# jseppanen/azalea

Hardware: AMD Instinct MI355X
Metric: mcts_sims_per_sec (higher is better)
Workload: dtype f16x3 (fp32 operands split hi+lo f16, fp32 accumulate)

## Files before the change

azalea_amd/csrc/azx_capi.cpp:

```cpp
#include <hip/hip_runtime.h>

#include <algorithm>
#include <cmath>
#include <cstdarg>
#include <cstdio>
#include <cstdlib>
#include <cstring>
#include <map>
#include <mutex>
#include <string>
#include <vector>

#include "../../include/azx.h"
#include "azx_dev.h"
#include "mcts_kernels.h"
#include "net.h"
#include "train.h"
#include "replay_kernels.h"
#include "ext_kernels.h"
#include "match_kernels.h"

#ifndef AZX_SRC_SHA
#define AZX_SRC_SHA "unknown"
#endif

static thread_local std::string g_err;

static int fail(int code, const char *fmt, ...) {
    char buf[1024];
    va_list ap;
    va_start(ap, fmt);
    vsnprintf(buf, sizeof buf, fmt, ap);
    va_end(ap);
    g_err = buf;
    return code;
}

#define HIPCHECK(expr)                                                                    \
    do {                                                                                  \
        hipError_t _e = (expr);                                                           \
        if (_e != hipSuccess)                                                             \
            return fail(AZX_EHIP, "%s failed: %s (%s:%d)", #expr, hipGetErrorString(_e),  \
                        __FILE__, __LINE__);                                              \
    } while (0)

struct azx_engine {
    azx_config cfg;
    DevEngine d;
    hipStream_t stream = nullptr;
    int reserved_cus = 0;
    std::mutex alloc_mu;
    int num_batches = 0;
    int selects_per_search = 0;
    std::vector<void *> allocs;
    int32_t *g_k = nullptr, *g_legal = nullptr, *g_nn = nullptr;
    float *g_cv = nullptr, *g_cw = nullptr, *g_cp = nullptr, *g_rv = nullptr, *g_rw = nullptr,
          *g_sv = nullptr;
    double *noise_dev = nullptr;
    size_t noise_cap = 0;
    float *prior_table_dev = nullptr;
    int32_t *moveids_dev = nullptr;
    int32_t *slots_dev = nullptr, *moves_dev = nullptr, *nmoves_dev = nullptr;
    size_t moves_cap = 0;
    bool ext_active = false;
    int ext_batches_done = 0;
    std::vector<int> ext_order;
    std::vector<std::vector<int>> ext_cells;
    azx_eval_fn ext_fn = nullptr;
    void *ext_user = nullptr;
    ExtBufs ext = {nullptr, nullptr, nullptr, nullptr, nullptr, nullptr, nullptr};
    int32_t ext_info[4] = {0, 0, AZX_EXT_NO_ERROR, 0};
    int32_t *ext_info_host = nullptr;
    std::vector<char> ext_dirty;
    bool ext_failed = false;
    bool play_ready = false;
    int64_t q_alloc = 0;
    int64_t q_rows_valid = 0;
    std::vector<void *> q_allocs;
    int32_t *export_board = nullptr;
    float *export_prob = nullptr;
    size_t export_cap = 0;
    ReplayRows ring = {nullptr, nullptr, nullptr, nullptr, nullptr};
    int64_t ring_cap = 0, ring_size = 0, ring_write = 0;
    long long *ring_idx = nullptr;
    int64_t ring_idx_cap = 0;
    int32_t *ring_maxk = nullptr;
    bool ring_mover_view = false;
    std::vector<void *> ring_allocs;
    long long *cidx_host[8] = {nullptr}, *cidx_dev[8] = {nullptr};
    hipEvent_t cidx_ev[8] = {nullptr};
    int64_t cidx_cap = 0;
    uint64_t cidx_next = 0;
    int32_t *cidx_maxk = nullptr;
    std::vector<hipEvent_t> ev_pool;
    std::vector<char> ev_tag;
    std::vector<int> ev_weight;
    std::vector<int> ev_group, ev_ref;
    int ev_groups = 0;
    size_t ev_used = 0;
    AzxNet *net = nullptr;
    bool force_generic = false;
    bool no_persistent = false;
    bool pipeline = true;
    bool stagger = true;
    hipStream_t stream_b = nullptr;
    std::vector<uint32_t> cu_mask;
    hipEvent_t ev_fork = nullptr, ev_join = nullptr, ev_stagger = nullptr;
    int32_t *stagger_ctr = nullptr;
    int64_t dbg_qcap = 0;
};

template <typename T>
static int dev_alloc(azx_engine *e, T **p, size_t count, bool zero = true) {
    void *q = nullptr;
    const size_t bytes = std::max<size_t>(count * sizeof(T), 16);
    hipError_t err = hipMalloc(&q, bytes);
    if (err != hipSuccess)
        return fail(AZX_ENOMEM, "hipMalloc(%zu bytes) failed: %s", bytes, hipGetErrorString(err));
    if (zero) {
        err = hipMemsetAsync(q, 0, bytes, e->stream);
        if (err != hipSuccess) return fail(AZX_EHIP, "hipMemset failed: %s", hipGetErrorString(err));
    }
    std::lock_guard<std::mutex> lock(e->alloc_mu);
    e->allocs.push_back(q);
    *p = reinterpret_cast<T *>(q);
    return AZX_OK;
}

struct DevGuard {
    int prev = -1;
    bool changed = false;
    explicit DevGuard(int dev) {
        if (hipGetDevice(&prev) == hipSuccess && prev != dev) changed = hipSetDevice(dev) == hipSuccess;
    }
    ~DevGuard() { if (changed) (void)hipSetDevice(prev); }
    DevGuard(const DevGuard &) = delete;
    DevGuard &operator=(const DevGuard &) = delete;
};
#define ENGINE_GUARD(e) DevGuard _dev_guard((e)->cfg.device)

#define TRY(expr)            \
    do {                     \
        int _rc = (expr);    \
        if (_rc) return _rc; \
    } while (0)

extern "C" const char *azx_last_error(void) { return g_err.c_str(); }
extern "C" int azx_version(void) { return 7; }

extern "C" int azx_create(const azx_config *cfg, azx_engine **out) {
    if (!cfg || !out) return fail(AZX_EINVAL, "null argument");
    int ndev = 0;
    if (hipGetDeviceCount(&ndev) != hipSuccess || ndev <= 0)
        return fail(AZX_ENODEV, "no HIP device visible: the engine has no CPU fallback");
    if (cfg->board_size < 2 || cfg->board_size > AZX_MAX_BOARD)
        return fail(AZX_EINVAL, "board_size %d outside [2, %d]", cfg->board_size, AZX_MAX_BOARD);
    if (cfg->n_games < 1) return fail(AZX_EINVAL, "n_games must be >= 1");
    if (cfg->search_batch_size < 1 || cfg->search_batch_size > AZX_MAX_BATCH)
        return fail(AZX_EINVAL, "search_batch_size %d outside [1, %d]", cfg->search_batch_size,
                    AZX_MAX_BATCH);
    if (cfg->simulations < 0) return fail(AZX_EINVAL, "simulations must be >= 0");
    if (cfg->evaluator < AZX_EVAL_RESNET || cfg->evaluator > AZX_EVAL_EXTERNAL)
        return fail(AZX_EINVAL, "unknown evaluator %d", cfg->evaluator);
    if (cfg->device < 0 || cfg->device >= ndev)
        return fail(AZX_EINVAL, "device %d not in [0, %d)", cfg->device, ndev);
    if (cfg->game_index_stride < 0 || cfg->game_index_offset < 0 ||
        cfg->game_index_offset >= std::max(1, cfg->game_index_stride))
        return fail(AZX_EINVAL, "game_index_offset %d outside [0, game_index_stride %d)", cfg->game_index_offset,
                    std::max(1, cfg->game_index_stride));
    DevGuard guard(cfg->device);
    { int cur = -1; if (hipGetDevice(&cur) != hipSuccess || cur != cfg->device) return fail(AZX_EHIP, "hipSetDevice(%d) failed", cfg->device); }
    if (azx_init_geometry(cfg->device)) return fail(AZX_EHIP, "uploading the board geometry tables failed");

    azx_engine *e = new azx_engine();
    e->cfg = *cfg;
    { const char *v = getenv("AZX_MCTS_GENERIC"); e->force_generic = v && atoi(v) != 0; }
    { const char *v = getenv("AZX_NO_PERSISTENT"); e->no_persistent = v && atoi(v) != 0; }
    { const char *v = getenv("AZX_PIPELINE"); e->pipeline = !(v && atoi(v) == 0); }
    { const char *v = getenv("AZX_PIPELINE_STAGGER"); e->stagger = !(v && atoi(v) == 0); }
    HIPCHECK(hipStreamCreateWithFlags(&e->stream, hipStreamNonBlocking));
    DevEngine &d = e->d;
    memset(&d, 0, sizeof d);
    d.N = cfg->board_size;
    d.ncells = d.N * d.N;
    d.G = cfg->n_games;
    d.bs = cfg->search_batch_size;
    d.slots = d.ncells <= 128 ? 2 : 3;
    d.c_puct = cfg->exploration_coef;
    d.evaluator = cfg->evaluator;
    d.flags = cfg->flags;
    d.seed = cfg->seed;
    d.uid_stride = std::max(1, cfg->game_index_stride);
    d.uid_offset = cfg->game_index_offset;
    d.slot_base = 0;
    d.pool_games = d.G;
    d.noise_alpha = (float)cfg->noise_alpha;
    d.noise_scale = 0.0;
    d.exploration_depth = cfg->exploration_depth;
    d.temperature = (float)cfg->temperature;
    e->num_batches = cfg->simulations / cfg->search_batch_size + 1;
    e->selects_per_search = e->num_batches * cfg->search_batch_size;
    d.selects_per_search = e->selects_per_search;
    int cap = cfg->nodes_per_game;
    if (cap <= 0) cap = 6 * (e->selects_per_search + 1) * d.ncells + 1024;
    d.cap = cap;

    const size_t G = d.G, bs = d.bs, E = G * bs;
    const size_t pstride = d.ncells + (d.ncells & 1);
    int rc = AZX_OK;
#define A(ptr, count) if (!rc) rc = dev_alloc(e, &ptr, (count))
    A(d.cells, G * d.slots * 64);
    A(d.ghdr, G);
    A(d.thdr, G);
    if (!rc) rc = dev_alloc(e, &d.arena[0], G * (size_t)cap, false);
    if (cfg->flags & AZX_FLAG_NO_COMPACT) d.arena[1] = d.arena[0];
    else if (!rc) rc = dev_alloc(e, &d.arena[1], G * (size_t)cap, false);
    A(d.leaf_node, E); A(d.leaf_len, E); A(d.leaf_eval, E); A(d.leaf_link, E); A(d.leaf_cells, E);
    A(d.leaf_mask, E * 4); A(d.path, E * pstride);
    A(d.ev_board, E * AZX_CELL_STRIDE); A(d.ev_src, E); A(d.ev_flip, E);
    A(d.ev_value, E); A(d.ev_prior, E * AZX_CELL_STRIDE); A(d.n_eval, 4);
    A(d.counters, G * CTR_COUNT); A(d.q_count, 2); A(d.stat_sums, G * 8);
    A(e->g_k, G); A(e->g_legal, G * d.ncells); A(e->g_nn, G);
    A(e->g_cv, G * d.ncells); A(e->g_cw, G * d.ncells); A(e->g_cp, G * d.ncells);
    A(e->g_rv, G); A(e->g_rw, G); A(e->g_sv, G);
    A(e->moveids_dev, G); A(e->slots_dev, G); A(e->nmoves_dev, G);
#undef A
    if (rc) { azx_destroy(e); return rc; }
    if (cfg->evaluator == AZX_EVAL_RESNET) {
        rc = azx_net_create(&e->net, d.N, cfg->num_blocks, cfg->base_chans, (int)E, e->stream);
        if (rc) { g_err = azx_net_error(); azx_destroy(e); return rc; }
    }
    {
        float *gt = nullptr;
        rc = dev_alloc(e, &gt, AZX_GAMMA_TAB_FLOATS);
        if (rc) { azx_destroy(e); return rc; }
        std::vector<float> tab(AZX_GAMMA_TAB_FLOATS, 0.0f);
        if (cfg->noise_alpha > 0.0) azx_gamma_table(cfg->noise_alpha, tab.data());
        if (hipMemcpyAsync(gt, tab.data(), tab.size() * sizeof(float), hipMemcpyHostToDevice, e->stream) != hipSuccess ||
            hipStreamSynchronize(e->stream) != hipSuccess) {
            azx_destroy(e);
            return fail(AZX_EHIP, "uploading the gamma sampler table failed");
        }
        e->d.gamma_tab = gt;
    }
    *out = e;
    {
        std::vector<float> tab(d.ncells + 1, 0.0f);
        for (int k = 1; k <= d.ncells; ++k) tab[k] = 1.0f / (float)k;
        rc = azx_set_prior_table(e, tab.data(), d.ncells + 1);
        if (rc) { azx_destroy(e); *out = nullptr; return rc; }
        e->d.prior_default = 1;
    }
    azx_launch_reset(d, nullptr, d.G, nullptr, nullptr, 0, 1, e->stream);
    HIPCHECK(hipStreamSynchronize(e->stream));
    return AZX_OK;
}

extern "C" void azx_destroy(azx_engine *e) {
    if (!e) return;
    ENGINE_GUARD(e);
    if (e->stream) (void)hipStreamSynchronize(e->stream);
    if (e->net) azx_net_destroy(e->net);
    for (void *p : e->allocs) (void)hipFree(p);
    for (void *p : e->q_allocs) (void)hipFree(p);
    for (void *p : e->ring_allocs) (void)hipFree(p);
    if (e->export_board) (void)hipFree(e->export_board);
    if (e->export_prob) (void)hipFree(e->export_prob);
    if (e->ext_info_host) (void)hipHostFree(e->ext_info_host);
    for (hipEvent_t ev : e->ev_pool) (void)hipEventDestroy(ev);
    if (e->ev_fork) (void)hipEventDestroy(e->ev_fork);
    if (e->ev_join) (void)hipEventDestroy(e->ev_join);
    if (e->ev_stagger) (void)hipEventDestroy(e->ev_stagger);
    if (e->stream_b) { (void)hipStreamSynchronize(e->stream_b); (void)hipStreamDestroy(e->stream_b); }
    for (int i = 0; i < 8; ++i) {
        if (e->cidx_ev[i]) { (void)hipEventSynchronize(e->cidx_ev[i]); (void)hipEventDestroy(e->cidx_ev[i]); }
        if (e->cidx_host[i]) (void)hipHostFree(e->cidx_host[i]);
        if (e->cidx_dev[i]) (void)hipFree(e->cidx_dev[i]);
    }
    if (e->stream) (void)hipStreamDestroy(e->stream);
    delete e;
}

extern "C" void *azx_stream(azx_engine *e) { return e ? (void *)e->stream : nullptr; }

extern "C" int azx_reserve_cus(azx_engine *e, int cus_per_xcd, int *reserved_out) {
    if (!e) return fail(AZX_EINVAL, "null engine");
    ENGINE_GUARD(e);
    hipDeviceProp_t prop;
    HIPCHECK(hipGetDeviceProperties(&prop, e->cfg.device));
    const int ncu = prop.multiProcessorCount, xcds = 8, ses = 4;
    if (cus_per_xcd < 0 || cus_per_xcd * xcds >= ncu)
        return fail(AZX_EINVAL, "cus_per_xcd %d outside [0, %d)", cus_per_xcd, ncu / xcds);
    if (cus_per_xcd > 0 && ncu % (xcds * ses))
        return fail(AZX_ESTATE, "CU reservation is laid out for 8 XCDs x 4 shader engines; this device has %d CUs", ncu);
    const int per = (cus_per_xcd + ses - 1) / ses * ses;
    const int words = (ncu + 31) / 32;
    std::vector<uint32_t> mask((size_t)words, 0u);
    for (int b = 0; b < ncu; ++b)
        if (b >= per * xcds) mask[b / 32] |= 1u << (b % 32);
    HIPCHECK(hipStreamSynchronize(e->stream));
    hipStream_t fresh = nullptr;
    if (per == 0) HIPCHECK(hipStreamCreateWithFlags(&fresh, hipStreamNonBlocking));
    else HIPCHECK(hipExtStreamCreateWithCUMask(&fresh, (uint32_t)words, mask.data()));
    hipStream_t old = e->stream;
    e->stream = fresh;
    if (e->net) azx_net_set_stream(e->net, fresh, per ? mask.data() : nullptr, per ? words : 0);
    (void)hipStreamDestroy(old);
    if (e->stream_b) {
        (void)hipStreamSynchronize(e->stream_b);
        (void)hipStreamDestroy(e->stream_b);
        e->stream_b = nullptr;
    }
    e->cu_mask.assign(mask.begin(), per ? mask.end() : mask.begin());
    e->reserved_cus = per * xcds;
    if (!e->cidx_maxk) TRY(dev_alloc(e, &e->cidx_maxk, 4));
    HIPCHECK(hipStreamSynchronize(e->stream));
    if (reserved_out) *reserved_out = e->reserved_cus;
    return AZX_OK;
}

static bool use_pipeline(const azx_engine *e) {
    return e->pipeline && e->d.evaluator == AZX_EVAL_RESNET && e->d.G % 2 == 0 && e->d.G >= 1024 &&
           azx_net_rows_splittable(e->net);
}

static DevEngine pool_view(const DevEngine &d, int base, int n, int32_t *n_eval) {
    DevEngine v = d;
    const size_t b = (size_t)base, bs = (size_t)d.bs, nc = (size_t)d.ncells, pstride = nc + (nc & 1);
    v.G = n;
    v.slot_base = d.slot_base + base;
    v.cells += b * d.slots * 64;
    v.ghdr += b;
    v.thdr += b;
    v.arena[0] += b * d.cap;
    v.arena[1] += b * d.cap;
    v.leaf_node += b * bs; v.leaf_len += b * bs; v.leaf_eval += b * bs; v.leaf_link += b * bs; v.leaf_cells += b * bs;
    v.leaf_mask += b * bs * 4;
    v.path += b * bs * pstride;
    v.ev_board += b * bs * AZX_CELL_STRIDE;
    v.ev_src += b * bs;
    v.ev_flip += b * bs;
    v.ev_value += b * bs;
    v.ev_prior += b * bs * AZX_CELL_STRIDE;
    v.n_eval = n_eval;
    if (v.noise) v.noise += b * d.n_select * d.noise_stride;
    v.counters += b * CTR_COUNT;
    v.stat_sums += b * 8;
    if (v.row_board) v.row_board += b * nc * AZX_CELL_STRIDE;
    if (v.row_prob) v.row_prob += b * nc * AZX_CELL_STRIDE;
    if (v.row_k) v.row_k += b * nc;
    if (v.row_meta) v.row_meta += b * nc * AZX_ROW_METRICS;
    return v;
}

static int pipeline_streams(azx_engine *e) {
    if (!e->stream_b) {
        if (e->cu_mask.empty()) HIPCHECK(hipStreamCreateWithFlags(&e->stream_b, hipStreamNonBlocking));
        else HIPCHECK(hipExtStreamCreateWithCUMask(&e->stream_b, (uint32_t)e->cu_mask.size(), e->cu_mask.data()));
    }
    if (!e->ev_fork) HIPCHECK(hipEventCreateWithFlags(&e->ev_fork, hipEventDisableTiming));
    if (!e->ev_join) HIPCHECK(hipEventCreateWithFlags(&e->ev_join, hipEventDisableTiming));
    if (!e->ev_stagger) HIPCHECK(hipEventCreateWithFlags(&e->ev_stagger, hipEventDisableTiming));
    if (!e->stagger_ctr) TRY(dev_alloc(e, &e->stagger_ctr, 4));
    return AZX_OK;
}

extern "C" int azx_kernel_info(azx_engine *e, char *buf, int cap) {
    if (!e || !buf || cap < 1) return fail(AZX_EINVAL, "null argument");
    const DevEngine &d = e->d;
    const int S = d.slots <= 2 ? 2 : 3;
    char tree[96], play[160];
    if (d.evaluator == AZX_EVAL_UNIFORM || d.evaluator == AZX_EVAL_UNIFORM_HASH) {
        DevEngine probe = d;
        probe.device_noise = 1;
        const bool fast = azx_mcts_fast_path(probe, MODE_BEGIN | MODE_INLINE, e->force_generic);
        snprintf(tree, sizeof tree, "k_mcts<%d,%s>", S, fast ? "FAST (throughput mode; generic with host noise)" : "generic");
        snprintf(play, sizeof play, "%s", fast && !e->no_persistent ? (S == 2 ? "k_play<2> (persistent)" : "k_play<3> (persistent)")
                                                                       : "k_mcts + k_choose + k_advance per move");
    } else {
        snprintf(tree, sizeof tree, "k_mcts<%d,generic> (BEGIN / APPLY|SELECT / APPLY phases)", S);
        snprintf(play, sizeof play, "%s", !use_pipeline(e) ? "phases + k_choose + k_advance per move, one stream"
                                          : e->stagger     ? "phases + k_choose + k_advance per move, two half-pools on two streams half an evaluation apart (any tower)"
                                                           : "phases + k_choose + k_advance per move, two half-pools on two streams");
    }
    std::string text = std::string("tree=") + tree + "; play=" + play + "; net=" +
                       (e->net ? azx_net_kernel_info(e->net) : "none") +
                       "; switches: AZX_MCTS_GENERIC=" + (e->force_generic ? "1" : "0") +
                       " AZX_NO_PERSISTENT=" + (e->no_persistent ? "1" : "0") +
                       " AZX_PIPELINE=" + (e->pipeline ? "1" : "0") +
                       " AZX_PIPELINE_STAGGER=" + (e->stagger ? "1" : "0") +
                       " reserved_cus=" + std::to_string(e->reserved_cus) +
                       "; src=" AZX_SRC_SHA;
    snprintf(buf, (size_t)cap, "%s", text.c_str());
    return (int)text.size();
}

extern "C" int azx_debug_stagger(azx_engine *e, int32_t *out4) {
    if (!e || !out4) return fail(AZX_EINVAL, "null argument");
    ENGINE_GUARD(e);
    memset(out4, 0, 4 * sizeof(int32_t));
    if (!e->stagger_ctr) return AZX_OK;
    HIPCHECK(hipMemcpyAsync(out4, e->stagger_ctr, 4 * sizeof(int32_t), hipMemcpyDeviceToHost, e->stream));
    HIPCHECK(hipStreamSynchronize(e->stream));
    return AZX_OK;
}

extern "C" int azx_debug_set_queue_cap(azx_engine *e, int64_t rows) {
    if (!e || rows < 0) return fail(AZX_EINVAL, "bad argument");
    e->dbg_qcap = rows;
    return AZX_OK;
}

static int check_net_range(azx_engine *e) {
    if (!e->net) return AZX_OK;
    int rc = azx_net_check_range(e->net, e->stream);
    if (rc) g_err = azx_net_error();
    return rc;
}

extern "C" int azx_debug_weights(azx_engine *e, int which, void *out, int64_t cap, int64_t *nbytes, char *name, int name_cap) {
    if (!e) return fail(AZX_EINVAL, "null engine");
    ENGINE_GUARD(e);
    if (!e->net) return fail(AZX_ESTATE, "engine was not created with AZX_EVAL_RESNET");
    int rc = azx_net_debug_weights(e->net, which, out, cap, nbytes, name, name_cap);
    if (rc) g_err = azx_net_error();
    return rc;
}

extern "C" int azx_set_weights(azx_engine *e, int n_tensors, const char *const *names,
                               const void *const *ptrs, const int64_t *counts, int on_device) {
    if (!e) return fail(AZX_EINVAL, "null engine");
    ENGINE_GUARD(e);
    if (!e->net) return fail(AZX_ESTATE, "engine was not created with AZX_EVAL_RESNET");
    int rc = azx_net_set_weights(e->net, n_tensors, names, ptrs, counts, on_device);
    if (rc) g_err = azx_net_error();
    return rc;
}

extern "C" int azx_set_prior_table(azx_engine *e, const float *prior_by_k, int count) {
    if (!e || !prior_by_k) return fail(AZX_EINVAL, "null argument");
    ENGINE_GUARD(e);
    if (count < e->d.ncells + 1) return fail(AZX_EINVAL, "prior table needs %d entries", e->d.ncells + 1);
    if (!e->prior_table_dev) TRY(dev_alloc(e, &e->prior_table_dev, (size_t)e->d.ncells + 1));
    HIPCHECK(hipMemcpyAsync(e->prior_table_dev, prior_by_k, sizeof(float) * (e->d.ncells + 1),
                            hipMemcpyHostToDevice, e->stream));
    HIPCHECK(hipStreamSynchronize(e->stream));
    e->d.prior_by_k = e->prior_table_dev;
    e->d.prior_default = 0;
    return AZX_OK;
}

extern "C" int azx_reset(azx_engine *e, const int32_t *slots, int n_slots, const int32_t *moves,
                         const int32_t *n_moves, int stride) {
    if (!e) return fail(AZX_EINVAL, "null engine");
    ENGINE_GUARD(e);
    DevEngine &d = e->d;
    if (!slots) n_slots = d.G;
    if (n_slots < 1 || n_slots > d.G) return fail(AZX_EINVAL, "n_slots %d outside [1, %d]", n_slots, d.G);
    if (slots) {
        for (int i = 0; i < n_slots; ++i)
            if (slots[i] < 0 || slots[i] >= d.G) return fail(AZX_EINVAL, "slot %d out of range", slots[i]);
        HIPCHECK(hipMemcpyAsync(e->slots_dev, slots, sizeof(int32_t) * n_slots, hipMemcpyHostToDevice, e->stream));
    }
    if (moves) {
        if (!n_moves || stride < 1) return fail(AZX_EINVAL, "moves given without n_moves/stride");
        const size_t need = (size_t)n_slots * stride;
        if (need > e->moves_cap) {
            TRY(dev_alloc(e, &e->moves_dev, need));
            e->moves_cap = need;
        }
        for (int i = 0; i < n_slots; ++i) {
            if (n_moves[i] < 0 || n_moves[i] > stride) return fail(AZX_EINVAL, "n_moves[%d] out of range", i);
            std::vector<char> used(d.ncells, 0);
            for (int p = 0; p < n_moves[i]; ++p) {
                const int mv = moves[(size_t)i * stride + p];
                if (mv < 1 || mv > d.ncells || used[mv - 1]) return fail(AZX_EINVAL, "illegal move %d", mv);
                used[mv - 1] = 1;
            }
        }
        HIPCHECK(hipMemcpyAsync(e->moves_dev, moves, sizeof(int32_t) * need, hipMemcpyHostToDevice, e->stream));
        HIPCHECK(hipMemcpyAsync(e->nmoves_dev, n_moves, sizeof(int32_t) * n_slots, hipMemcpyHostToDevice, e->stream));
    }
    azx_launch_reset(d, slots ? e->slots_dev : nullptr, n_slots, moves ? e->moves_dev : nullptr,
                     moves ? e->nmoves_dev : nullptr, stride, 1, e->stream);
    HIPCHECK(hipGetLastError());
    HIPCHECK(hipStreamSynchronize(e->stream));
    e->ext_active = false;
    if (e->ext_failed) {
        for (int i = 0; i < n_slots; ++i) e->ext_dirty[slots ? slots[i] : i] = 0;
        e->ext_failed = std::find(e->ext_dirty.begin(), e->ext_dirty.end(), 1) != e->ext_dirty.end();
    }
    return AZX_OK;
}

static void time_begin(azx_engine *e, char tag = 0, hipStream_t s = nullptr, int group = 0, int ref = -1) {
    if (e->ev_used + 2 > e->ev_pool.size()) {
        if (e->ev_pool.size() >= 1 << 16) return;
        hipEvent_t a, b;
        if (hipEventCreate(&a) != hipSuccess || hipEventCreate(&b) != hipSuccess) return;
        e->ev_pool.push_back(a);
        e->ev_pool.push_back(b);
    }
    const size_t n = e->ev_pool.size() / 2, i = e->ev_used / 2;
    if (e->ev_tag.size() < n) { e->ev_tag.resize(n, 0); e->ev_weight.resize(n, 1); e->ev_group.resize(n, 0); e->ev_ref.resize(n, -1); }
    e->ev_tag[i] = tag;
    e->ev_weight[i] = 1;
    e->ev_group[i] = ref >= 0 ? group : 0;
    e->ev_ref[i] = ref;
    (void)hipEventRecord(e->ev_pool[e->ev_used], s ? s : e->stream);
}
static void time_end(azx_engine *e, int weight = 1, hipStream_t s = nullptr) {
    if (e->ev_used + 2 > e->ev_pool.size()) return;
    (void)hipEventRecord(e->ev_pool[e->ev_used + 1], s ? s : e->stream);
    e->ev_weight[e->ev_used / 2] = weight;
    e->ev_used += 2;
}
static int time_mark(azx_engine *e, hipStream_t s) {
    time_begin(e, 2, s);
    if (e->ev_used + 2 > e->ev_pool.size()) return -1;
    const int ref = (int)e->ev_used;
    time_end(e, 1, s);
    return ref;
}
static void time_collect(azx_engine *e, azx_play_stats *st) {
    auto book = [&](char tag, int weight, double seconds, int launches) {
        if (tag == 1) { st->net_seconds += seconds; st->net_launches += launches; }
        else {
            st->mcts_seconds += seconds;
            st->mcts_launches += weight * launches;
            st->mcts_kernel_launches += launches;
        }
    };
    std::map<int, char> groups;
    std::map<std::pair<int, char>, std::vector<std::pair<float, float>>> spans;
    for (size_t i = 0; i + 1 < e->ev_used; i += 2) {
        const size_t k = i / 2;
        if (e->ev_tag[k] == 2) continue;
        float ms = 0.f;
        if (!e->ev_group[k]) {
            if (hipEventElapsedTime(&ms, e->ev_pool[i], e->ev_pool[i + 1]) == hipSuccess)
                book(e->ev_tag[k], e->ev_weight[k], ms * 1e-3, 1);
            continue;
        }
        float b = 0.f, en = 0.f;
// ... 59 lines not shown
    char buf[768];
    va_list ap;
    va_start(ap, fmt);
    vsnprintf(buf, sizeof buf, fmt, ap);
    va_end(ap);
    (void)hipStreamSynchronize(e->stream);
    const int32_t clear = AZX_EXT_NO_ERROR;
    (void)hipMemcpyAsync(e->ext.info + 2, &clear, sizeof clear, hipMemcpyHostToDevice, e->stream);
    (void)hipStreamSynchronize(e->stream);
    e->ext_info[2] = clear;
    e->ext_active = false;
    e->ev_used = 0;
    e->ev_groups = 0;
    e->ext_failed = true;
    std::fill(e->ext_dirty.begin(), e->ext_dirty.end(), 1);
    return fail(AZX_EEXTERNAL, "%s", buf);
}

static int ext_check_rows(azx_engine *e) {
    const int32_t w = e->ext_info[2];
    if (w == AZX_EXT_NO_ERROR) return AZX_OK;
    const int row = w >> 3, what = w & 7;
    return ext_fail(e, "external evaluator: row %d of its batch %s", row,
                    (what & 1) ? "has a value that is not finite"
                    : (what & 2) ? "has a negative (or NaN) prior probability"
                                 : "has prior probabilities whose sum is not 1 within 1e-4 (mcts.py:211-213)");
}

static int ext_info_enqueue(azx_engine *e, hipStream_t s) {
    HIPCHECK(hipMemcpyAsync(e->ext_info_host, e->ext.info, sizeof e->ext_info, hipMemcpyDeviceToHost, s));
    return AZX_OK;
}

static int ext_info_take(azx_engine *e) {
    memcpy(e->ext_info, e->ext_info_host, sizeof e->ext_info);
    return ext_check_rows(e);
}

static int ext_read_info(azx_engine *e) {
    TRY(ext_info_enqueue(e, e->stream));
    HIPCHECK(hipStreamSynchronize(e->stream));
    return ext_info_take(e);
}

static int ext_point_enqueue(azx_engine *e, bool timed) {
    if (timed) time_begin(e, 1);
    azx_launch_ext_order(e->d, e->ext, e->stream);
    HIPCHECK(hipGetLastError());
    return ext_info_enqueue(e, e->stream);
}

static int ext_point_finish(azx_engine *e, bool timed) {
    DevEngine &d = e->d;
    HIPCHECK(hipStreamSynchronize(e->stream));
    const int rc_info = ext_info_take(e);
    if (rc_info) return rc_info;
    const int n = e->ext_info[0], kmax = e->ext_info[1];
    if (n < 0 || n > d.G * d.bs) return ext_fail(e, "external evaluator: %d pending rows (internal error)", n);
    if (n > 0) {
        azx_launch_ext_export(d, e->ext, n, e->stream);
        HIPCHECK(hipGetLastError());
        const int rc = e->ext_fn(e->ext_user, n, kmax, e->ext.board, e->ext.legal, e->ext.value, e->ext.prior,
                                 (void *)e->stream);
        if (rc) return ext_fail(e, "external evaluator returned %d on a batch of %d rows", rc, n);
        azx_launch_ext_import(d, e->ext, n, e->stream);
        HIPCHECK(hipGetLastError());
    }
    if (timed) time_end(e);
    return AZX_OK;
}

struct ExtCursor {
    int points = 0;
    bool done = true;
    bool timed = false;
};

static int ext_search_begin(azx_engine *e, ExtCursor *c, bool timed) {
    c->points = 0;
    c->done = false;
    c->timed = timed;
    HIPCHECK(hipMemsetAsync(e->d.n_eval, 0, sizeof(int32_t), e->stream));
    if (timed) time_begin(e);
    azx_launch_mcts(e->d, MODE_BEGIN, e->num_batches, e->stream, e->force_generic);
    if (timed) time_end(e);
    return ext_point_enqueue(e, timed);
}

static int ext_search_resume(azx_engine *e, ExtCursor *c) {
    TRY(ext_point_finish(e, c->timed));
    if (c->points < e->num_batches) {
        HIPCHECK(hipMemsetAsync(e->d.n_eval, 0, sizeof(int32_t), e->stream));
        if (c->timed) time_begin(e);
        azx_launch_mcts(e->d, MODE_APPLY | MODE_SELECT, e->num_batches, e->stream, e->force_generic);
        if (c->timed) time_end(e);
        c->points += 1;
        return ext_point_enqueue(e, c->timed);
    }
    if (c->timed) time_begin(e);
    azx_launch_mcts(e->d, MODE_APPLY, e->num_batches, e->stream, e->force_generic);
    if (c->timed) time_end(e);
    c->done = true;
    return AZX_OK;
}

extern "C" int azx_set_external_evaluator(azx_engine *e, azx_eval_fn fn, void *user) {
    if (!e) return fail(AZX_EINVAL, "null engine");
    ENGINE_GUARD(e);
    if (e->d.evaluator != AZX_EVAL_EXTERNAL)
        return fail(AZX_EINVAL, "an external evaluator needs an AZX_EVAL_EXTERNAL engine (this one has evaluator %d)",
                    e->d.evaluator);
    if (fn && !e->ext.info) {
        const size_t E = (size_t)e->d.G * e->d.bs, nc = (size_t)e->d.ncells;
        ExtBufs x = {nullptr, nullptr, nullptr, nullptr, nullptr, nullptr, nullptr};
        int rc = AZX_OK;
        if (!rc) rc = dev_alloc(e, &x.src2ev, E);
        if (!rc) rc = dev_alloc(e, &x.row_ev, E);
        if (!rc) rc = dev_alloc(e, &x.info, 4);
        if (!rc) rc = dev_alloc(e, &x.board, E * nc);
        if (!rc) rc = dev_alloc(e, &x.legal, E * nc);
        if (!rc) rc = dev_alloc(e, &x.value, E);
        if (!rc) rc = dev_alloc(e, &x.prior, E * nc);
        if (rc) return rc;
        if (!e->ext_info_host &&
            hipHostMalloc((void **)&e->ext_info_host, sizeof e->ext_info, hipHostMallocDefault) != hipSuccess)
            return fail(AZX_ENOMEM, "hipHostMalloc of the evaluator's info words failed");
        const int32_t init[4] = {0, 0, AZX_EXT_NO_ERROR, 0};
        HIPCHECK(hipMemcpyAsync(x.info, init, sizeof init, hipMemcpyHostToDevice, e->stream));
        HIPCHECK(hipStreamSynchronize(e->stream));
        e->ext = x;
        e->ext_dirty.assign((size_t)e->d.G, 0);
    }
    e->ext_fn = fn;
    e->ext_user = fn ? user : nullptr;
    return AZX_OK;
}

static int enqueue_search(azx_engine *e, bool timed) {
    DevEngine &d = e->d;
    if (ext_registered(e)) {
        ExtCursor c;
        TRY(ext_search_begin(e, &c, timed));
        while (!c.done) TRY(ext_search_resume(e, &c));
        return AZX_OK;
    }
    if (d.evaluator == AZX_EVAL_UNIFORM || d.evaluator == AZX_EVAL_UNIFORM_HASH) {
        if (timed) time_begin(e);
        azx_launch_mcts(d, MODE_BEGIN | MODE_INLINE, e->num_batches, e->stream, e->force_generic);
        if (timed) time_end(e);
        return AZX_OK;
    }
    if (d.evaluator == AZX_EVAL_RESNET) {
        if (!azx_net_ready(e->net)) return fail(AZX_ESTATE, "azx_set_weights has not been called");
        HIPCHECK(hipMemsetAsync(d.n_eval, 0, sizeof(int32_t), e->stream));
        if (timed) time_begin(e);
        azx_launch_mcts(d, MODE_BEGIN, e->num_batches, e->stream, e->force_generic);
        if (timed) time_end(e);
        if (timed) time_begin(e, 1);
        azx_net_eval(e->net, d, e->stream);
        if (timed) time_end(e);
        for (int b = 0; b < e->num_batches; ++b) {
            HIPCHECK(hipMemsetAsync(d.n_eval, 0, sizeof(int32_t), e->stream));
            if (timed) time_begin(e);
            azx_launch_mcts(d, MODE_APPLY | MODE_SELECT, e->num_batches, e->stream, e->force_generic);
            if (timed) time_end(e);
            if (timed) time_begin(e, 1);
            azx_net_eval(e->net, d, e->stream);
            if (timed) time_end(e);
        }
        if (timed) time_begin(e);
        azx_launch_mcts(d, MODE_APPLY, e->num_batches, e->stream, e->force_generic);
        if (timed) time_end(e);
        return AZX_OK;
    }
    return fail(AZX_ESTATE, "evaluator %d has no device pipeline", d.evaluator);
}

extern "C" int azx_search(azx_engine *e, const double *noise, int n_select, int noise_stride,
                          double noise_scale) {
    if (!e) return fail(AZX_EINVAL, "null engine");
    ENGINE_GUARD(e);
    TRY(ext_refuse(e));
    if (e->d.evaluator == AZX_EVAL_EXTERNAL && !ext_registered(e))
        return fail(AZX_ESTATE, "AZX_EVAL_EXTERNAL: drive azx_search_begin/step instead");
    TRY(upload_noise(e, noise, n_select, noise_stride, noise_scale));
    TRY(enqueue_search(e, false));
    HIPCHECK(hipGetLastError());
    HIPCHECK(hipStreamSynchronize(e->stream));
    if (ext_registered(e)) return ext_read_info(e);
    return check_net_range(e);
}

static int read_pending(azx_engine *e, int *n_pending) {
    int32_t n = 0;
    HIPCHECK(hipMemcpyAsync(&n, e->d.n_eval, sizeof n, hipMemcpyDeviceToHost, e->stream));
    HIPCHECK(hipStreamSynchronize(e->stream));
    *n_pending = n;
    return e->d.evaluator == AZX_EVAL_RESNET ? check_net_range(e) : AZX_OK;
}

extern "C" int azx_search_begin(azx_engine *e, const double *noise, int n_select, int noise_stride,
                                double noise_scale, int *n_pending) {
    if (!e || !n_pending) return fail(AZX_EINVAL, "null argument");
    ENGINE_GUARD(e);
    TRY(ext_refuse(e));
    if (e->d.evaluator != AZX_EVAL_EXTERNAL && e->d.evaluator != AZX_EVAL_RESNET)
        return fail(AZX_ESTATE, "phase API needs AZX_EVAL_EXTERNAL (or RESNET)");
    TRY(upload_noise(e, noise, n_select, noise_stride, noise_scale));
    HIPCHECK(hipMemsetAsync(e->d.n_eval, 0, sizeof(int32_t), e->stream));
    if (e->d.evaluator == AZX_EVAL_RESNET && !azx_net_ready(e->net))
        return fail(AZX_ESTATE, "azx_set_weights has not been called");
    azx_launch_mcts(e->d, MODE_BEGIN, e->num_batches, e->stream, e->force_generic);
    if (e->d.evaluator == AZX_EVAL_RESNET) azx_net_eval(e->net, e->d, e->stream);
    HIPCHECK(hipGetLastError());
    e->ext_active = true;
    e->ext_batches_done = 0;
    return read_pending(e, n_pending);
}

extern "C" int azx_search_step(azx_engine *e, int *n_pending, int *done) {
    if (!e || !n_pending || !done) return fail(AZX_EINVAL, "null argument");
    ENGINE_GUARD(e);
    if (!e->ext_active) return fail(AZX_ESTATE, "azx_search_step without azx_search_begin");
    HIPCHECK(hipMemsetAsync(e->d.n_eval, 0, sizeof(int32_t), e->stream));
    if (e->ext_batches_done < e->num_batches) {
        azx_launch_mcts(e->d, MODE_APPLY | MODE_SELECT, e->num_batches, e->stream, e->force_generic);
        if (e->d.evaluator == AZX_EVAL_RESNET) azx_net_eval(e->net, e->d, e->stream);
        e->ext_batches_done += 1;
        *done = 0;
    } else {
        azx_launch_mcts(e->d, MODE_APPLY, e->num_batches, e->stream, e->force_generic);
        e->ext_active = false;
        *done = 1;
    }
    HIPCHECK(hipGetLastError());
    return read_pending(e, n_pending);
}

static int flip_cell(int cell, int N) {
    const int r = cell / N, c = cell % N;
    return (N - 1 - c) * N + (N - 1 - r);
}

extern "C" int azx_get_leaves(azx_engine *e, int cap, int32_t *boards, int32_t *legal_moves,
                              int32_t *slot, int32_t *k, int *n_out) {
    if (!e || !n_out) return fail(AZX_EINVAL, "null argument");
    ENGINE_GUARD(e);
    DevEngine &d = e->d;
    int n = 0;
    TRY(read_pending(e, &n));
    if (n > cap) return fail(AZX_EINVAL, "%d pending leaves, caller capacity %d", n, cap);
    *n_out = n;
    e->ext_order.clear();
    e->ext_cells.clear();
    if (n == 0) return AZX_OK;
    std::vector<uint8_t> hb((size_t)n * AZX_CELL_STRIDE);
    std::vector<int32_t> hsrc(n), hflip(n);
    HIPCHECK(hipMemcpyAsync(hb.data(), d.ev_board, hb.size(), hipMemcpyDeviceToHost, e->stream));
    HIPCHECK(hipMemcpyAsync(hsrc.data(), d.ev_src, sizeof(int32_t) * n, hipMemcpyDeviceToHost, e->stream));
    HIPCHECK(hipMemcpyAsync(hflip.data(), d.ev_flip, sizeof(int32_t) * n, hipMemcpyDeviceToHost, e->stream));
    const size_t E = (size_t)d.G * d.bs;
    std::vector<uint64_t> hmask(E * 4);
    HIPCHECK(hipMemcpyAsync(hmask.data(), d.leaf_mask, sizeof(uint64_t) * hmask.size(), hipMemcpyDeviceToHost, e->stream));
    HIPCHECK(hipStreamSynchronize(e->stream));
    std::vector<int> order(n);
    for (int i = 0; i < n; ++i) order[i] = i;
    std::sort(order.begin(), order.end(), [&](int a, int b) { return hsrc[a] < hsrc[b]; });
    e->ext_order = order;
    e->ext_cells.resize(n);
    for (int j = 0; j < n; ++j) {
        const int ev = order[j], src = hsrc[ev];
        std::vector<int> &cells = e->ext_cells[j];
        for (int c = 0; c < d.ncells; ++c)
            if ((hmask[(size_t)src * 4 + (c >> 6)] >> (c & 63)) & 1ull) cells.push_back(c);
        if (slot) slot[j] = src / d.bs;
        if (k) k[j] = (int)cells.size();
        if (boards)
            for (int c = 0; c < d.ncells; ++c)
                boards[(size_t)j * d.ncells + c] = hb[(size_t)ev * AZX_CELL_STRIDE + c];
        if (legal_moves) {
            for (int c = 0; c < d.ncells; ++c) legal_moves[(size_t)j * d.ncells + c] = 0;
            for (size_t i = 0; i < cells.size(); ++i)
                legal_moves[(size_t)j * d.ncells + i] =
                    (hflip[ev] ? flip_cell(cells[i], d.N) : cells[i]) + 1;
        }
    }
    return AZX_OK;
}

extern "C" int azx_put_evals(azx_engine *e, int n, const float *value, const float *prior) {
    if (!e || (n && (!value || !prior))) return fail(AZX_EINVAL, "null argument");
    ENGINE_GUARD(e);
    DevEngine &d = e->d;
    if (n != (int)e->ext_order.size())
        return fail(AZX_ESTATE, "azx_put_evals(%d) does not match %zu pending leaves", n, e->ext_order.size());
    if (n == 0) return AZX_OK;
    std::vector<float> hv(n), hp((size_t)n * AZX_CELL_STRIDE, 0.0f);
    for (int j = 0; j < n; ++j) {
        const int ev = e->ext_order[j];
        hv[ev] = value[j];
        const std::vector<int> &cells = e->ext_cells[j];
        for (size_t i = 0; i < cells.size(); ++i)
            hp[(size_t)ev * AZX_CELL_STRIDE + cells[i]] = prior[(size_t)j * d.ncells + i];
    }
    HIPCHECK(hipMemcpyAsync(d.ev_value, hv.data(), sizeof(float) * n, hipMemcpyHostToDevice, e->stream));
    HIPCHECK(hipMemcpyAsync(d.ev_prior, hp.data(), sizeof(float) * hp.size(), hipMemcpyHostToDevice, e->stream));
    HIPCHECK(hipStreamSynchronize(e->stream));
    return AZX_OK;
}

extern "C" int azx_get_evals(azx_engine *e, int cap, float *value, float *prior, int *n_out) {
    if (!e || !n_out) return fail(AZX_EINVAL, "null argument");
    ENGINE_GUARD(e);
    DevEngine &d = e->d;
    const int n = (int)e->ext_order.size();
    if (n > cap) return fail(AZX_EINVAL, "%d evaluations, caller capacity %d", n, cap);
    *n_out = n;
    if (n == 0) return AZX_OK;
    std::vector<float> hv(n), hp((size_t)n * AZX_CELL_STRIDE);
    HIPCHECK(hipMemcpyAsync(hv.data(), d.ev_value, sizeof(float) * n, hipMemcpyDeviceToHost, e->stream));
    HIPCHECK(hipMemcpyAsync(hp.data(), d.ev_prior, sizeof(float) * hp.size(), hipMemcpyDeviceToHost, e->stream));
    HIPCHECK(hipStreamSynchronize(e->stream));
    for (int j = 0; j < n; ++j) {
        const int ev = e->ext_order[j];
// ... 137 lines not shown
}

extern "C" int azx_forward(azx_engine *e, int B, int K, const int32_t *boards,
                           const int32_t *legal_moves, float *value, float *moves_logprob) {
    if (!e) return fail(AZX_EINVAL, "null engine");
    ENGINE_GUARD(e);
    if (!e->net) return fail(AZX_ESTATE, "engine was not created with AZX_EVAL_RESNET");
    int rc = azx_net_forward_host(e->net, B, K, boards, legal_moves, value, moves_logprob, e->stream);
    if (rc) g_err = azx_net_error();
    return rc ? rc : check_net_range(e);
}

extern "C" int azx_hex_replay(int device, int board_size, int n_games, const int32_t *moves,
                              const int32_t *length, int stride, int32_t *result_out,
                              int32_t *nlegal_out, uint64_t *empties_out, int32_t *final_board) {
    int ndev = 0;
    if (hipGetDeviceCount(&ndev) != hipSuccess || ndev <= 0)
        return fail(AZX_ENODEV, "no HIP device visible: the engine has no CPU fallback");
    if (board_size < 2 || board_size > AZX_MAX_BOARD) return fail(AZX_EINVAL, "bad board_size");
    if (n_games < 1 || stride < 1 || !moves || !length) return fail(AZX_EINVAL, "bad argument");
    DevGuard guard(device);
    if (azx_init_geometry(device)) return fail(AZX_EHIP, "uploading the board geometry tables failed");
    const int ncells = board_size * board_size;
    for (int g = 0; g < n_games; ++g) {
        if (length[g] < 0 || length[g] > stride) return fail(AZX_EINVAL, "length[%d] out of range", g);
        std::vector<char> used(ncells, 0);
        for (int p = 0; p < length[g]; ++p) {
            const int mv = moves[(size_t)g * stride + p];
            if (mv < 1 || mv > ncells || used[mv - 1]) return fail(AZX_EINVAL, "illegal move %d in game %d", mv, g);
            used[mv - 1] = 1;
        }
    }
    const size_t gs = (size_t)n_games * stride;
    int32_t *dm = nullptr, *dl = nullptr, *dr = nullptr, *dn = nullptr, *df = nullptr;
    uint64_t *de = nullptr;
    HIPCHECK(hipMalloc(&dm, sizeof(int32_t) * gs));
    HIPCHECK(hipMalloc(&dl, sizeof(int32_t) * n_games));
    HIPCHECK(hipMalloc(&dr, sizeof(int32_t) * gs));
    HIPCHECK(hipMalloc(&dn, sizeof(int32_t) * gs));
    HIPCHECK(hipMalloc(&de, sizeof(uint64_t) * gs * 4));
    HIPCHECK(hipMalloc(&df, sizeof(int32_t) * (size_t)n_games * ncells));
    HIPCHECK(hipMemset(dr, 0, sizeof(int32_t) * gs));
    HIPCHECK(hipMemset(dn, 0, sizeof(int32_t) * gs));
    HIPCHECK(hipMemset(de, 0, sizeof(uint64_t) * gs * 4));
    HIPCHECK(hipMemcpy(dm, moves, sizeof(int32_t) * gs, hipMemcpyHostToDevice));
    HIPCHECK(hipMemcpy(dl, length, sizeof(int32_t) * n_games, hipMemcpyHostToDevice));
    azx_launch_hex_replay(board_size, n_games, dm, dl, stride, dr, dn, de, df, nullptr);
    HIPCHECK(hipGetLastError());
    HIPCHECK(hipDeviceSynchronize());
    if (result_out) HIPCHECK(hipMemcpy(result_out, dr, sizeof(int32_t) * gs, hipMemcpyDeviceToHost));
    if (nlegal_out) HIPCHECK(hipMemcpy(nlegal_out, dn, sizeof(int32_t) * gs, hipMemcpyDeviceToHost));
    if (empties_out) HIPCHECK(hipMemcpy(empties_out, de, sizeof(uint64_t) * gs * 4, hipMemcpyDeviceToHost));
    if (final_board) HIPCHECK(hipMemcpy(final_board, df, sizeof(int32_t) * (size_t)n_games * ncells, hipMemcpyDeviceToHost));
    (void)hipFree(dm); (void)hipFree(dl); (void)hipFree(dr); (void)hipFree(dn); (void)hipFree(de); (void)hipFree(df);
    return AZX_OK;
}

extern "C" int azx_set_active(azx_engine *e, const int32_t *active) {
    if (!e || !active) return fail(AZX_EINVAL, "null argument");
    ENGINE_GUARD(e);
    DevEngine &d = e->d;
    std::vector<int32_t> a((size_t)d.G);
    for (int g = 0; g < d.G; ++g) a[g] = active[g] ? 1 : 0;
    HIPCHECK(hipMemcpy2DAsync(&d.ghdr[0].active, sizeof(GameHdr), a.data(), sizeof(int32_t), sizeof(int32_t),
                              (size_t)d.G, hipMemcpyHostToDevice, e->stream));
    HIPCHECK(hipStreamSynchronize(e->stream));
    return AZX_OK;
}

static int play_setup(azx_engine *e, int64_t q_rows, int ring) {
    DevEngine &d = e->d;
    e->q_rows_valid = 0;
    if (!e->play_ready) {
        const size_t rows = (size_t)d.G * d.ncells;
        TRY(dev_alloc(e, &d.row_board, rows * AZX_CELL_STRIDE));
        TRY(dev_alloc(e, &d.row_prob, rows * AZX_CELL_STRIDE));
        TRY(dev_alloc(e, &d.row_k, rows));
        TRY(dev_alloc(e, &d.row_meta, rows * AZX_ROW_METRICS));
        e->play_ready = true;
    }
    if (q_rows > e->q_alloc) {
        (void)hipStreamSynchronize(e->stream);
        for (void *p : e->q_allocs) (void)hipFree(p);
        e->q_allocs.clear();
        auto qa = [&](void **p, size_t bytes) -> int {
            hipError_t err = hipMalloc(p, bytes);
            if (err != hipSuccess) return fail(AZX_ENOMEM, "hipMalloc(%zu) failed: %s", bytes, hipGetErrorString(err));
            e->q_allocs.push_back(*p);
            return AZX_OK;
        };
        TRY(qa((void **)&d.q_board, (size_t)q_rows * AZX_CELL_STRIDE));
        TRY(qa((void **)&d.q_prob, (size_t)q_rows * AZX_CELL_STRIDE * sizeof(float)));
        TRY(qa((void **)&d.q_color, (size_t)q_rows * sizeof(int32_t)));
        TRY(qa((void **)&d.q_k, (size_t)q_rows * sizeof(int32_t)));
        TRY(qa((void **)&d.q_reward, (size_t)q_rows * sizeof(float)));
        TRY(qa((void **)&d.q_uid, (size_t)q_rows * sizeof(int64_t)));
        TRY(qa((void **)&d.q_meta, (size_t)q_rows * AZX_ROW_METRICS * sizeof(float)));
        e->q_alloc = q_rows;
    }
    d.q_cap = e->q_alloc;
    d.q_ring = ring;
    HIPCHECK(hipMemsetAsync(d.q_count, 0, sizeof(unsigned long long), e->stream));
    return AZX_OK;
}

struct CounterSnap {
    unsigned long long c[CTR_COUNT];
    double s[8];
};

static int snap_counters(azx_engine *e, CounterSnap *s) {
    const size_t G = e->d.G;
    std::vector<unsigned long long> hc(G * CTR_COUNT);
    std::vector<double> hs(G * 8);
    HIPCHECK(hipMemcpyAsync(hc.data(), e->d.counters, hc.size() * sizeof(unsigned long long), hipMemcpyDeviceToHost, e->stream));
    HIPCHECK(hipMemcpyAsync(hs.data(), e->d.stat_sums, hs.size() * sizeof(double), hipMemcpyDeviceToHost, e->stream));
    HIPCHECK(hipStreamSynchronize(e->stream));
    memset(s, 0, sizeof *s);
    for (size_t g = 0; g < G; ++g) {
        for (int j = 0; j < CTR_COUNT; ++j) s->c[j] += hc[g * CTR_COUNT + j];
        for (int j = 0; j < 8; ++j) s->s[j] += hs[g * 8 + j];
    }
    return AZX_OK;
}

static void fill_stats(const CounterSnap &a, const CounterSnap &b, azx_play_stats *st) {
    st->games = (int64_t)(b.c[CTR_GAMES] - a.c[CTR_GAMES]);
    st->game_errors = (int64_t)(b.c[CTR_ERRORS] - a.c[CTR_ERRORS]);
    st->plies = (int64_t)(b.c[CTR_PLIES] - a.c[CTR_PLIES]);
    st->selects = (int64_t)(b.c[CTR_SELECTS] - a.c[CTR_SELECTS]);
    st->evals = (int64_t)(b.c[CTR_EVALS] - a.c[CTR_EVALS]);
    st->sum_depth = (int64_t)(b.c[CTR_SUM_DEPTH] - a.c[CTR_SUM_DEPTH]);
    st->sum_k_interior = (int64_t)(b.c[CTR_SUM_K_INT] - a.c[CTR_SUM_K_INT]);
    st->sum_k_leaf = (int64_t)(b.c[CTR_SUM_K_LEAF] - a.c[CTR_SUM_K_LEAF]);
    st->sum_search_value = b.s[0] - a.s[0];
    st->sum_root_width = b.s[1] - a.s[1];
    st->sum_action_logprob = b.s[2] - a.s[2];
    st->sum_reward_last = b.s[3] - a.s[3];
    st->sum_game_length = b.s[4] - a.s[4];
}

static int enqueue_ply(azx_engine *e) {
    TRY(enqueue_search(e, true));
    azx_launch_choose(e->d, e->stream);
    azx_launch_advance(e->d, nullptr, 1, e->stream);
    return AZX_OK;
}

static int enqueue_plies_pipelined(azx_engine *e, int64_t plies) {
    TRY(pipeline_streams(e));
    if (!azx_net_ready(e->net)) return fail(AZX_ESTATE, "azx_set_weights has not been called");
    const DevEngine &d = e->d;
    const int half = d.G / 2, rows = half * d.bs;
    const DevEngine hv[2] = {pool_view(d, 0, half, d.n_eval), pool_view(d, half, half, d.n_eval + 1)};
    const hipStream_t hs[2] = {e->stream, e->stream_b};
    const int nb = e->num_batches;
    const int split = rows / 2 / AZX_NET_ROW_ALIGN * AZX_NET_ROW_ALIGN;
    const bool stagger = e->stagger && split > 0;
    const int ref = time_mark(e, hs[0]);
    for (int64_t p = 0; p < plies; ++p) {
        for (int ph = 0; ph <= nb; ++ph) {
            const int g_tree = ++e->ev_groups, g_net = ++e->ev_groups;
            for (int h = 0; h < 2; ++h) {
                HIPCHECK(hipMemsetAsync(hv[h].n_eval, 0, sizeof(int32_t), hs[h]));
                time_begin(e, 0, hs[h], g_tree, ref);
                azx_launch_mcts(hv[h], ph ? MODE_APPLY | MODE_SELECT : MODE_BEGIN, nb, hs[h], e->force_generic);
                time_end(e, 1, hs[h]);
                if (p == 0 && ph == 0 && h == 0) {
                    HIPCHECK(hipEventRecord(e->ev_fork, hs[0]));
                    HIPCHECK(hipStreamWaitEvent(hs[1], e->ev_fork, 0));
                }
                const bool cut = stagger && ph == 1;
                if (cut && h == 1) HIPCHECK(hipStreamWaitEvent(hs[1], e->ev_stagger, 0));
                time_begin(e, 1, hs[h], g_net, ref);
                azx_net_eval_rows(e->net, hv[h], h * rows, cut && h == 0 ? split : rows, hs[h]);
                time_end(e, 1, hs[h]);
                if (cut && h == 0) {
                    HIPCHECK(hipEventRecord(e->ev_stagger, hs[0]));
                    time_begin(e, 1, hs[h], g_net, ref);
                    azx_net_eval_rows_behind(e->net, hv[h], h * rows, split, rows, e->stagger_ctr, hs[h]);
                    time_end(e, 1, hs[h]);
                }
            }
        }
        const int g_tree = ++e->ev_groups;
        for (int h = 0; h < 2; ++h) {
            time_begin(e, 0, hs[h], g_tree, ref);
            azx_launch_mcts(hv[h], MODE_APPLY, nb, hs[h], e->force_generic);
            time_end(e, 1, hs[h]);
            azx_launch_choose(hv[h], hs[h]);
            azx_launch_advance(hv[h], nullptr, 1, hs[h]);
        }
    }
    HIPCHECK(hipEventRecord(e->ev_join, hs[1]));
    HIPCHECK(hipStreamWaitEvent(hs[0], e->ev_join, 0));
    return AZX_OK;
}

extern "C" int azx_play_steps(azx_engine *e, int64_t plies, azx_play_stats *stats) {
    if (!e || !stats) return fail(AZX_EINVAL, "null argument");
    ENGINE_GUARD(e);
    TRY(ext_refuse(e));
    if (e->d.evaluator == AZX_EVAL_EXTERNAL && !ext_registered(e))
        return fail(AZX_ESTATE, "play mode needs a device evaluator");
    memset(stats, 0, sizeof *stats);
    TRY(play_setup(e, std::max<int64_t>(e->q_alloc, 1 << 16), 1));
    TRY(upload_noise(e, nullptr, 0, 0, e->cfg.noise_scale));
    CounterSnap a, b;
    TRY(snap_counters(e, &a));
    hipEvent_t t0, t1;
    HIPCHECK(hipEventCreate(&t0));
    HIPCHECK(hipEventCreate(&t1));
    HIPCHECK(hipEventRecord(t0, e->stream));
    azx_launch_advance(e->d, nullptr, 2, e->stream);
    {
        const int PLAY_CHUNK = 256;
        int64_t p = 0;
        while (p < plies) {
            const int n = (int)std::min<int64_t>(PLAY_CHUNK, plies - p);
            time_begin(e);
            const bool ok = azx_launch_play(e->d, e->num_batches, n, e->stream, !e->force_generic && !e->no_persistent);
            if (!ok) break;
            time_end(e, n);
            p += n;
        }
        if (p < plies && use_pipeline(e)) TRY(enqueue_plies_pipelined(e, plies - p));
        else for (; p < plies; ++p) TRY(enqueue_ply(e));
    }
    HIPCHECK(hipEventRecord(t1, e->stream));
    HIPCHECK(hipGetLastError());
    HIPCHECK(hipStreamSynchronize(e->stream));
    float ms = 0.f;
    HIPCHECK(hipEventElapsedTime(&ms, t0, t1));
    (void)hipEventDestroy(t0);
    (void)hipEventDestroy(t1);
    TRY(snap_counters(e, &b));
    fill_stats(a, b, stats);
    stats->positions = (int64_t)(b.c[CTR_ROWS] - a.c[CTR_ROWS]);
    stats->seconds = ms * 1e-3;
    time_collect(e, stats);
    if (ext_registered(e)) return ext_read_info(e);
    return check_net_range(e);
}

static int play_until(azx_engine *e, int64_t min_positions, int64_t max_plies, azx_play_stats *stats,
                      unsigned long long *rows_out) {
    DevEngine &d = e->d;
    memset(stats, 0, sizeof *stats);
    const int64_t worst = min_positions + (int64_t)d.G * d.ncells;
    TRY(play_setup(e, worst, 0));
    if (e->dbg_qcap > 0)
        d.q_cap = std::max<int64_t>(1, std::min<int64_t>(d.q_cap, e->dbg_qcap));
    TRY(upload_noise(e, nullptr, 0, 0, e->cfg.noise_scale));
    CounterSnap a, b;
    TRY(snap_counters(e, &a));
    hipEvent_t t0, t1;
    HIPCHECK(hipEventCreate(&t0));
    HIPCHECK(hipEventCreate(&t1));
    HIPCHECK(hipEventRecord(t0, e->stream));
    azx_launch_advance(d, nullptr, 2, e->stream);
    unsigned long long rows = 0;
    for (int64_t p = 0; (max_plies <= 0 || p < max_plies) && (int64_t)rows < min_positions;) {
        const int64_t most = std::min<int64_t>(8, 2 * d.N - 1);
        const int chunk = (int)std::min<int64_t>(most, max_plies > 0 ? max_plies - p : most);
        time_begin(e);
        if (azx_launch_play(d, e->num_batches, chunk, e->stream, !e->force_generic && !e->no_persistent)) {
            time_end(e, chunk);
            p += chunk;
        } else {
            if (use_pipeline(e)) TRY(enqueue_plies_pipelined(e, 1));
            else TRY(enqueue_ply(e));
            p += 1;
        }
        HIPCHECK(hipMemcpyAsync(&rows, d.q_count, sizeof rows, hipMemcpyDeviceToHost, e->stream));
        HIPCHECK(hipStreamSynchronize(e->stream));
        if (e->dbg_qcap > 0 && (p & 7) == 0) {
            std::vector<GameHdr> hh((size_t)d.G);
            HIPCHECK(hipMemcpyAsync(hh.data(), d.ghdr, sizeof(GameHdr) * hh.size(), hipMemcpyDeviceToHost, e->stream));
            HIPCHECK(hipStreamSynchronize(e->stream));
            bool any = false;
            for (const GameHdr &h : hh) any = any || h.active;
            if (!any) break;
        }
    }
    HIPCHECK(hipEventRecord(t1, e->stream));
    HIPCHECK(hipStreamSynchronize(e->stream));
    float ms = 0.f;
    HIPCHECK(hipEventElapsedTime(&ms, t0, t1));
    (void)hipEventDestroy(t0);
    (void)hipEventDestroy(t1);
    TRY(snap_counters(e, &b));
    fill_stats(a, b, stats);
    stats->positions = (int64_t)rows;
    stats->seconds = ms * 1e-3;
    time_collect(e, stats);
    *rows_out = rows;
    if (ext_registered(e)) return ext_read_info(e);
    return check_net_range(e);
}

extern "C" int azx_play(azx_engine *e, int64_t min_positions, int64_t max_plies, int64_t cap,
                        int32_t *board, int32_t *color, int32_t *nlegal, float *moves_prob,
                        float *reward, int64_t *game_uid, azx_play_stats *stats) {
    if (!e || !stats) return fail(AZX_EINVAL, "null argument");
    ENGINE_GUARD(e);
    TRY(ext_refuse(e));
    if (e->d.evaluator == AZX_EVAL_EXTERNAL && !ext_registered(e))
        return fail(AZX_ESTATE, "play mode needs a device evaluator");
    DevEngine &d = e->d;
    const int64_t worst = min_positions + (int64_t)d.G * d.ncells;
    if (cap < worst)
        return fail(AZX_EINVAL, "cap %lld < min_positions + n_games*cells = %lld (whole games only)",
                    (long long)cap, (long long)worst);
    unsigned long long rows = 0;
    TRY(play_until(e, min_positions, max_plies, stats, &rows));
    e->q_rows_valid = (int64_t)rows;
    if (rows == 0) return AZX_OK;
    const size_t n = (size_t)rows;
    if (board || moves_prob) {
        const size_t need = n * d.ncells;
        if (need > e->export_cap) {
            (void)hipStreamSynchronize(e->stream);
            if (e->export_board) (void)hipFree(e->export_board);
            if (e->export_prob) (void)hipFree(e->export_prob);
            e->export_board = nullptr; e->export_prob = nullptr; e->export_cap = 0;
            if (hipMalloc((void **)&e->export_board, need * sizeof(int32_t)) != hipSuccess ||
                hipMalloc((void **)&e->export_prob, need * sizeof(float)) != hipSuccess)
                return fail(AZX_ENOMEM, "hipMalloc of the export staging (%zu rows) failed", n);
            e->export_cap = need;
        }
        azx_launch_rows_export(d.q_board, d.q_prob, (long long)n, d.ncells, e->export_board, e->export_prob, e->stream);
        HIPCHECK(hipGetLastError());
        if (board) HIPCHECK(hipMemcpyAsync(board, e->export_board, need * sizeof(int32_t), hipMemcpyDeviceToHost, e->stream));
        if (moves_prob) HIPCHECK(hipMemcpyAsync(moves_prob, e->export_prob, need * sizeof(float), hipMemcpyDeviceToHost, e->stream));
    }
    if (color) HIPCHECK(hipMemcpyAsync(color, d.q_color, n * sizeof(int32_t), hipMemcpyDeviceToHost, e->stream));
    if (nlegal) HIPCHECK(hipMemcpyAsync(nlegal, d.q_k, n * sizeof(int32_t), hipMemcpyDeviceToHost, e->stream));
    if (reward) HIPCHECK(hipMemcpyAsync(reward, d.q_reward, n * sizeof(float), hipMemcpyDeviceToHost, e->stream));
    if (game_uid) HIPCHECK(hipMemcpyAsync(game_uid, d.q_uid, n * sizeof(int64_t), hipMemcpyDeviceToHost, e->stream));
    HIPCHECK(hipStreamSynchronize(e->stream));
    return AZX_OK;
}

extern "C" int azx_play_device(azx_engine *e, int64_t min_positions, int64_t max_plies, int64_t *rows_out,
// ... 855 lines not shown
```

azalea_amd/csrc/azx_dev.h:

```cpp
#pragma once
#include <hip/hip_runtime.h>
#include <stdint.h>

#include "../../include/azx.h"

#define AZX_LINK_UNEVAL (-1)
#define AZX_LINK_TERM(fc) (-2 - (fc))
#define AZX_LABEL_NONE 0x3FFFFFu

struct alignas(16) Node {
    float nv;
    float tv;
    float pp;
    int32_t link;
};

struct alignas(64) TreeHdr {
    int32_t num_nodes;
    int32_t root_id;
    int32_t root_k;
    int32_t k0;
    int32_t arena;
    int32_t status;
    int32_t batches_left;
    int32_t pending;
    int32_t pending_root;
    int32_t select_count;
    float   search_value;
    int32_t slow_div;
    int32_t defer_compact;
    int32_t dropped;
    int32_t pad[2];
};

struct alignas(64) GameHdr {
    int32_t color;
    int32_t winner;
    int32_t ply;
    int32_t active;
    int64_t uid;
    int32_t move_id;
    int32_t n_rows;
    int32_t gen;
    int32_t ply0;
    int32_t parked;
    int32_t pad[5];
};

enum {
    CTR_SELECTS = 0, CTR_SUM_DEPTH, CTR_SUM_K_INT, CTR_SUM_K_LEAF, CTR_EVALS, CTR_TERM_EVALS,
    CTR_GAMES, CTR_ERRORS, CTR_PLIES, CTR_ROWS, CTR_COUNT = 16
};

struct DevEngine {
    int32_t N, ncells, G, bs, cap, slots;
    int32_t selects_per_search;
    float c_puct;
    int32_t evaluator, flags;
    uint32_t *cells;
    GameHdr *ghdr;
    Node *arena[2];
    TreeHdr *thdr;
    int32_t *leaf_node;
    int32_t *leaf_len;
    int32_t *leaf_eval;
    int32_t *leaf_link;
    int32_t *leaf_cells;
    uint64_t *leaf_mask;
    int32_t *path;
    uint8_t *ev_board;
    int32_t *ev_src;
    int32_t *ev_flip;
    float *ev_value;
    float *ev_prior;
    int32_t *n_eval;
    const double *noise;
    int32_t n_select, noise_stride;
    double noise_scale;
    float noise_alpha;
    const float *gamma_tab;
    int32_t device_noise;
    uint64_t seed;
    int32_t uid_stride, uid_offset;
    int32_t slot_base, pool_games;
    const float *prior_by_k;
    int32_t prior_default;
    unsigned long long *counters;
    int32_t exploration_depth;
    float temperature;
    uint8_t *row_board;
    float *row_prob;
    int32_t *row_k;
    float *row_meta;
    int64_t q_cap;
    int32_t q_ring;
    uint8_t *q_board;
    float *q_prob;
    int32_t *q_color, *q_k;
    float *q_reward;
    int64_t *q_uid;
    float *q_meta;
    unsigned long long *q_count;
    double *stat_sums;
};

#define AZX_DPP(old, v, ctrl, rmask) \
    __builtin_amdgcn_update_dpp((old), (v), (ctrl), (rmask), 0xf, false)

__device__ __forceinline__ float wave_sum(float v) {
    v += __int_as_float(AZX_DPP(0, __float_as_int(v), 0x111, 0xf));
    v += __int_as_float(AZX_DPP(0, __float_as_int(v), 0x112, 0xf));
    v += __int_as_float(AZX_DPP(0, __float_as_int(v), 0x114, 0xf));
    v += __int_as_float(AZX_DPP(0, __float_as_int(v), 0x118, 0xf));
    v += __int_as_float(AZX_DPP(0, __float_as_int(v), 0x142, 0xa));
    v += __int_as_float(AZX_DPP(0, __float_as_int(v), 0x143, 0xc));
    return __int_as_float(__builtin_amdgcn_readlane(__float_as_int(v), 63));
}
__device__ __forceinline__ int wave_sum_i(int v) {
    v += AZX_DPP(0, v, 0x111, 0xf);
    v += AZX_DPP(0, v, 0x112, 0xf);
    v += AZX_DPP(0, v, 0x114, 0xf);
    v += AZX_DPP(0, v, 0x118, 0xf);
    v += AZX_DPP(0, v, 0x142, 0xa);
    v += AZX_DPP(0, v, 0x143, 0xc);
    return __builtin_amdgcn_readlane(v, 63);
}
__device__ __forceinline__ uint32_t wave_max_u32(uint32_t v) {
#define AZX_DPPZ(v, ctrl, rmask) (uint32_t)__builtin_amdgcn_update_dpp(0, (int)(v), (ctrl), (rmask), 0xf, true)
    uint32_t t;
    t = AZX_DPPZ(v, 0x111, 0xf); v = t > v ? t : v;
    t = AZX_DPPZ(v, 0x112, 0xf); v = t > v ? t : v;
    t = AZX_DPPZ(v, 0x114, 0xf); v = t > v ? t : v;
    t = AZX_DPPZ(v, 0x118, 0xf); v = t > v ? t : v;
    t = AZX_DPPZ(v, 0x142, 0xa); v = t > v ? t : v;
    t = AZX_DPPZ(v, 0x143, 0xc); v = t > v ? t : v;
#undef AZX_DPPZ
    return (uint32_t)__builtin_amdgcn_readlane((int)v, 63);
}
__device__ __forceinline__ float wave_max(float v) {
    const int ninf = 0xff800000;
    v = fmaxf(v, __int_as_float(AZX_DPP(ninf, __float_as_int(v), 0x111, 0xf)));
    v = fmaxf(v, __int_as_float(AZX_DPP(ninf, __float_as_int(v), 0x112, 0xf)));
    v = fmaxf(v, __int_as_float(AZX_DPP(ninf, __float_as_int(v), 0x114, 0xf)));
    v = fmaxf(v, __int_as_float(AZX_DPP(ninf, __float_as_int(v), 0x118, 0xf)));
    v = fmaxf(v, __int_as_float(AZX_DPP(ninf, __float_as_int(v), 0x142, 0xa)));
    v = fmaxf(v, __int_as_float(AZX_DPP(ninf, __float_as_int(v), 0x143, 0xc)));
    return __int_as_float(__builtin_amdgcn_readlane(__float_as_int(v), 63));
}

#define AZX_GEO_CELLS 820
extern __constant__ uint64_t c_geo[AZX_GEO_CELLS * 4];
#define AZX_SQRT_TAB 4096
extern __constant__ float c_sqrt[AZX_SQRT_TAB];
__host__ __device__ inline int azx_geo_base(int N) {
    int b = 0;
    for (int n = 2; n < N; ++n) b += n * n;
    return b;
}

template <int SLOTS>
struct HexWave {
    uint32_t c[SLOTS];
    uint64_t occ[2][SLOTS];
    int color;
    int winner;
    int gbase;

    __device__ __forceinline__ void geom(int N, int lane) { (void)lane; gbase = azx_geo_base(N); }
    __device__ __forceinline__ void load(const uint32_t *p, int lane) {
#pragma unroll
        for (int s = 0; s < SLOTS; ++s) {
            c[s] = p[s * 64 + lane];
            occ[0][s] = __ballot((c[s] & 3u) == 1u);
            occ[1][s] = __ballot((c[s] & 3u) == 2u);
        }
    }
    __device__ __forceinline__ void store(uint32_t *p, int lane) const {
#pragma unroll
        for (int s = 0; s < SLOTS; ++s) p[s * 64 + lane] = c[s];
    }
    __device__ __forceinline__ void clear() {
#pragma unroll
        for (int s = 0; s < SLOTS; ++s) { c[s] = 0; occ[0][s] = 0ull; occ[1][s] = 0ull; }
        color = 1;
        winner = 0;
    }
    __device__ __forceinline__ uint64_t empties(int s, int lane, int ncells) const {
        (void)lane;
        const int nv = ncells - 64 * s;
        const uint64_t valid = nv >= 64 ? ~0ull : (nv <= 0 ? 0ull : ((1ull << nv) - 1ull));
        return ~(occ[0][s] | occ[1][s]) & valid;
    }
    __device__ __forceinline__ void step(int cell, int N, int lane) {
        (void)N;
        const int col = color;
        const uint64_t *g = c_geo + (size_t)(gbase + cell) * 4;
        uint32_t flags = (uint32_t)(g[3] >> (2 * (col - 1))) & 3u;
        uint64_t nb[SLOTS];
#pragma unroll
        for (int s = 0; s < SLOTS; ++s) {
            nb[s] = g[s] & (col == 1 ? occ[0][s] : occ[1][s]);
            uint64_t m = nb[s];
            while (m) {
                const int j = (int)__ffsll((long long)m) - 1;
                m &= m - 1;
                flags |= ((uint32_t)__builtin_amdgcn_readlane((int)c[s], j) >> 2) & 3u;
            }
        }
        const uint32_t nv = (uint32_t)col | (flags << 2) | ((uint32_t)cell << 8);
#pragma unroll
        for (int s = 0; s < SLOTS; ++s) {
            uint64_t m = nb[s];
            while (m) {
                const int j = (int)__ffsll((long long)m) - 1;
                m &= m - 1;
                const uint32_t lab = (uint32_t)__builtin_amdgcn_readlane((int)c[s], j) >> 8;
#pragma unroll
                for (int t = 0; t < SLOTS; ++t)
                    if ((int)(c[t] & 3u) == col && (c[t] >> 8) == lab) c[t] = nv;
            }
        }
        const uint64_t bit = 1ull << (cell & 63);
#pragma unroll
        for (int s = 0; s < SLOTS; ++s) {
            if (s * 64 + lane == cell) c[s] = nv;
            if (s == (cell >> 6)) {
                if (col == 1) occ[0][s] |= bit; else occ[1][s] |= bit;
            }
        }
        winner = (flags == 3u) ? col : 0;
        color = 3 - col;
    }
};
```

azalea_amd/csrc/mcts_kernels.h:

```cpp
#pragma once
#include <hip/hip_runtime.h>
#include <stddef.h>
#include <stdint.h>

#include "azx_dev.h"

#define MODE_BEGIN 1
#define MODE_APPLY 2
#define MODE_SELECT 4
#define MODE_INLINE 8

size_t azx_mcts_lds_bytes(int ncells, int bs);
void azx_launch_mcts(const DevEngine &E, int mode, int num_batches, hipStream_t st, bool force_generic);
bool azx_mcts_fast_path(const DevEngine &E, int mode, bool force_generic);
bool azx_launch_play(const DevEngine &E, int num_batches, int steps, hipStream_t st, bool allowed);
void azx_launch_reset(const DevEngine &E, const int32_t *slots, int n_slots, const int32_t *moves,
                      const int32_t *n_moves, int stride, int assign_uid, hipStream_t st);
void azx_launch_advance(const DevEngine &E, const int32_t *move_ids, int play_mode, hipStream_t st);
void azx_launch_gather_root(const DevEngine &E, int32_t *k_out, int32_t *legal, float *cv, float *cw,
                            float *cp, float *rv, float *rw, int32_t *nn, float *sv, hipStream_t st);
void azx_launch_choose(const DevEngine &E, hipStream_t st);
void azx_launch_hex_replay(int N, int n_games, const int32_t *moves, const int32_t *length, int stride,
                           int32_t *result_out, int32_t *nlegal_out, uint64_t *empties_out,
                           int32_t *final_board, hipStream_t st);
void azx_launch_arith(const float *a, const float *b, float *sq, float *dv, float *mul, int n,
                      hipStream_t st);
void azx_launch_divide_test(const float *num, const float *den, float *q, float *rt, int n, hipStream_t st);
void azx_launch_noise_test(float alpha, const float *tab, int k, int n_rows, uint32_t seed, float *out, hipStream_t st);
#define AZX_GAMMA_TAB_FLOATS 802
void azx_gamma_table(double alpha, float *tab);
int azx_init_geometry(int device);
```

azalea_amd/csrc/mcts_kernels.hip:

```cpp
#include <cmath>
#include <cstdlib>
#include <cstring>
#include <type_traits>

#include "azx_dev.h"
#include "mcts_kernels.h"

__constant__ uint64_t c_geo[AZX_GEO_CELLS * 4];
__constant__ float c_sqrt[AZX_SQRT_TAB];
__constant__ float c_invk[256];

int azx_init_geometry(int device) {
    static bool done[64] = {false};
    if (device >= 0 && device < 64 && done[device]) return 0;
    static uint64_t tab[AZX_GEO_CELLS * 4];
    memset(tab, 0, sizeof tab);
    for (int N = 2; N <= AZX_MAX_BOARD; ++N) {
        const int base = azx_geo_base(N);
        const int dr[6] = {-1, -1, 0, 0, 1, 1}, dc[6] = {0, 1, -1, 1, -1, 0};
        for (int r = 0; r < N; ++r)
            for (int c = 0; c < N; ++c) {
                uint64_t *g = tab + (size_t)(base + r * N + c) * 4;
                for (int d = 0; d < 6; ++d) {
                    const int rr = r + dr[d], cc = c + dc[d];
// ... 1000 lines not shown
                } else {
#pragma unroll
                    for (int s = 0; s < SLOTS; ++s) m_mask[s] = lmask[s];
                }
            }
            lds_sync();
            path_apply(L.path + i * pstride, depth, -1, slot1, 1.0f, 1.0f, false, false);
            T_MARK(3)
        }
        int nu = 0;
        if (FAST) {
            for (int i = 0; i < bs; ++i) {
                const int id = rl(m_node, i);
                const bool dup = __ballot(lane < i && m_node == id) != 0ull;
                const int len = rl(m_len, i), cells = rl(m_cells, i);
                bool term = false;
                if (!dup) {
                    term = (rl(m_tm, i) & 1) != 0;
                    const int k = rl(m_k, i);
                    if (term) c_term += 1; else c_evals += 1;
                    if (!expand(id, len, cells, rl(m_link, i), term, nullptr, k, nullptr,
                                (!term && k) ? inline_prior(k, len) : 0.0f))
                        break;
                    if (lane == nu) m_val = term ? -1.0f : 0.0f;
                    nu += 1;
                    root_nv += 1.0f;
                    if (term) root_tv += (len & 1) ? 1.0f : -1.0f;
                }
                T_MARK(4)
                const float dvn = dup ? -1.0f : 0.0f;
                auto tvd = [&](int d) -> float {
                    return term ? (((len - 1 - d) & 1) ? 0.0f : -2.0f) : -1.0f;
                };
                root_child_add(cells & 0xffff, dvn, tvd(0));
                const int32_t *pth = L.path + i * pstride;
                const int s1 = rl(m_slot1, i);
                for (int d = 1; d < len; ++d) {
                    const int slot = (d == 1 && s1 >= 0 && memo_ok) ? s1
                                                                    : cache_find(pth[d] & 0xffffff, false, 0.f, 0.f);
                    if (lane == slot) { c_nv += dvn; c_tv += tvd(d); }
                }
                T_MARK(5)
            }
            batches_left -= 1;
            wave_mem_sync();
            if (status == 0) search_value += np_sum_vals(nu);
            T_MARK(5)
            continue;
        }
        for (int i = 0; i < bs; ++i)
            path_apply(L.path + i * pstride, rl(m_len, i), rl(m_cells, i) & 0xffff, rl(m_slot1, i), -1.0f, -1.0f,
                       false, false);
        for (int i = 0; i < bs; ++i) {
            const int id = rl(m_node, i);
            const bool dup = __ballot(lane < i && m_node == id) != 0ull;
            if (!dup) {
                if (lane == nu) m_uidx = i;
                nu += 1;
            }
        }
        batches_left -= 1;
        T_MARK(4)

        if (inline_eval) {
            for (int u = 0; u < nu; ++u) {
                const int i = rl(m_uidx, u);
                const int tm = rl(m_tm, i);
                const bool terminal = (tm & 1) != 0;
                const int k = rl(m_k, i);
                float v = -1.0f;
                if (!terminal) {
                    v = (!FAST && E.evaluator == AZX_EVAL_UNIFORM_HASH)
                            ? hash_value(L.colors + i * AZX_CELL_STRIDE, tm >> 1) : 0.0f;
                    c_evals += 1;
                    if (!value_in_fast_range(v)) slow_div = true;
                } else {
                    c_term += 1;
                }
                const int lf_len = rl(m_len, i), lf_cells = rl(m_cells, i);
                if (!expand(rl(m_node, i), lf_len, lf_cells, rl(m_link, i), terminal, nullptr, k, nullptr,
                            (!terminal && k) ? inline_prior(k, lf_len) : 0.0f))
                    break;
                path_apply(L.path + i * pstride, lf_len, lf_cells & 0xffff, rl(m_slot1, i), 1.0f, v, true, true);
                if (lane == u) m_val = v;
            }
            wave_mem_sync();
            if (status == 0) search_value += np_sum_vals(nu);
            T_MARK(5)
        } else {
            int n_nt = 0;
            for (int u = 0; u < nu; ++u) n_nt += (rl(m_tm, rl(m_uidx, u)) & 1) ? 0 : 1;
            int e0 = 0;
            if (lane == 0 && n_nt) e0 = atomicAdd(E.n_eval, n_nt);
            e0 = __builtin_amdgcn_readfirstlane(e0);
            const size_t lb = (size_t)g * bs;
            int e = e0;
            for (int u = 0; u < nu; ++u) {
                const int i = rl(m_uidx, u);
                const int tm = rl(m_tm, i);
                const bool terminal = (tm & 1) != 0;
                const int len = rl(m_len, i);
                int32_t *pth = E.path + (lb + u) * (size_t)pstride;
                for (int d = lane; d < len; d += 64) pth[d] = L.path[i * pstride + d];
                if (lane == 0) {
                    E.leaf_node[lb + u] = rl(m_node, i);
                    E.leaf_len[lb + u] = len;
                    E.leaf_link[lb + u] = rl(m_link, i);
                    E.leaf_cells[lb + u] = rl(m_cells, i);
                    E.leaf_eval[lb + u] = terminal ? -1 : e;
#pragma unroll
                    for (int s = 0; s < SLOTS; ++s) E.leaf_mask[(lb + u) * 4 + s] = rl64(m_mask[s], i);
                }
                if (!terminal) {
                    emit_request(e, g * bs + u, L.colors + i * AZX_CELL_STRIDE, tm >> 1);
                    e += 1;
                    c_evals += 1;
                } else {
                    c_term += 1;
                }
            }
            pending = nu;
        }
    }

    T_FLUSH
    cache_flush();
    if (root_link >= 0) {
#pragma unroll
        for (int s = 0; s < SLOTS; ++s)
            if (rempty[s]) *reinterpret_cast<float4 *>(arena + root_link + s * 64 + lane) = rst[s];
    }
    if (lane == 0) {
        *reinterpret_cast<float2 *>(arena + root_id) = make_float2(root_nv, root_tv);
        th->num_nodes = num_nodes;
        th->status = status;
        th->batches_left = batches_left;
        th->pending = pending;
        th->pending_root = pending_root;
        th->select_count = select_count;
        th->search_value = search_value;
        if (!FAST) th->slow_div = slow_div ? 1 : 0;
    }
    static_assert(CTR_SELECTS == 0 && CTR_SUM_DEPTH == 1 && CTR_SUM_K_INT == 2 && CTR_SUM_K_LEAF == 3 &&
                  CTR_EVALS == 4 && CTR_TERM_EVALS == 5, "tally order");
    if (lane < 6) {
        const uint32_t add = lane == 0 ? c_selects : lane == 1 ? c_depth : lane == 2 ? c_kint
                           : lane == 3 ? c_kleaf : lane == 4 ? c_evals : c_term;
        if (add) E.counters[(size_t)g * CTR_COUNT + lane] += add;
    }
}

template <int SLOTS, bool FAST>
__global__ __launch_bounds__(64) AZX_MCTS_ATTR void k_mcts(DevEngine E, int mode_arg, int num_batches) {
    mcts_body<SLOTS, FAST>(E, mode_arg, num_batches);
}

template <int SLOTS>
__device__ __forceinline__ void tree_reset(const DevEngine &E, int g, TreeHdr *th, int k, int lane) {
    Node *arena = E.arena[th->arena] + (size_t)g * E.cap;
    if (lane == 0) {
        Node nd;
        nd.nv = 0.0f; nd.tv = 0.0f; nd.pp = 1.0f; nd.link = AZX_LINK_UNEVAL;
        arena[0] = nd;
        th->num_nodes = 1;
        th->root_id = 0;
        th->root_k = k;
        th->k0 = k;
        th->status = 0;
        th->batches_left = 0;
        th->pending = 0;
        th->pending_root = 0;
        th->select_count = 0;
        th->search_value = 0.0f;
        th->slow_div = 0;
        th->defer_compact = 0;
        th->dropped = 0;
    }
}

template <int SLOTS>
__global__ __launch_bounds__(64) void k_reset(DevEngine E, const int32_t *slots, int n_slots,
                                              const int32_t *moves, const int32_t *n_moves,
                                              int stride, int assign_uid) {
    const int lane = threadIdx.x;
    const int idx = blockIdx.x;
    if (idx >= n_slots) return;
    const int g = slots ? slots[idx] : idx;
    HexWave<SLOTS> h;
    h.clear();
    h.geom(E.N, lane);
    int ply = 0;
    if (moves) {
        const int nm = n_moves[idx];
        for (int p = 0; p < nm; ++p) {
            const int mv = moves[(size_t)idx * stride + p];
            h.step(mv - 1, E.N, lane);
            ply += 1;
        }
    }
    h.store(E.cells + (size_t)g * SLOTS * 64, lane);
    const Masks<SLOTS> mk = make_masks<SLOTS>(h, lane, E.ncells);
    GameHdr *gh = E.ghdr + g;
    TreeHdr *th = E.thdr + g;
    if (lane == 0) {
        gh->color = h.color;
        gh->winner = h.winner;
        gh->ply = ply;
        gh->active = 1;
        gh->move_id = -1;
        gh->n_rows = 0;
        gh->parked = 0;
        gh->ply0 = ply;
        if (assign_uid) { gh->uid = game_uid(E, g, gh->gen); gh->gen += 1; }
        th->arena = 0;
    }
    __builtin_amdgcn_s_waitcnt(0);
    tree_reset<SLOTS>(E, g, th, mk.k, lane);
}

template <int SLOTS>
__device__ __forceinline__ void advance_body(const DevEngine &E, int g, const int32_t *move_ids, int play_mode) {
    __shared__ int sh_old[64];
    const int lane = threadIdx.x;
    GameHdr *gh = E.ghdr + g;
    TreeHdr *th = E.thdr + g;
    const bool parked = gh->parked != 0;
    if (play_mode == 2 ? !parked : !gh->active) return;
    int status = th->status;
    const int mid = move_ids ? move_ids[g] : gh->move_id;
    if (!parked && mid < 0 && status == 0) return;

    HexWave<SLOTS> h;
    h.load(E.cells + (size_t)g * SLOTS * 64, lane);
    h.geom(E.N, lane);
    h.color = gh->color;
    h.winner = gh->winner;
    int ply = gh->ply;
    bool finished = parked, errored = !parked && status != 0;

    if (!errored && !parked) {
        const Masks<SLOTS> mk = make_masks<SLOTS>(h, lane, E.ncells);
        int cell = -1;
#pragma unroll
        for (int s = 0; s < SLOTS; ++s) {
            const bool empty = lane_bit(mk.m[s]);
            const int rk = mk.base[s] + rank_below(mk.m[s]);
            const uint64_t hit = __ballot(empty && rk == mid);
            if (hit) cell = s * 64 + (int)__ffsll((long long)hit) - 1;
        }
        if (cell < 0) return;
        h.step(cell, E.N, lane);
        ply += 1;
        h.store(E.cells + (size_t)g * SLOTS * 64, lane);
        const Masks<SLOTS> nmk = make_masks<SLOTS>(h, lane, E.ncells);
        finished = h.winner != 0;

        Node *src = E.arena[th->arena] + (size_t)g * E.cap;
        const int root_id = th->root_id;
        const int root_link = src[root_id].link;
        int child = -1, clink = AZX_LINK_UNEVAL;
        if (root_link >= 0) {
            child = root_link + mid;
            clink = src[child].link;
        }
        if (child < 0 || clink == AZX_LINK_UNEVAL) {
            tree_reset<SLOTS>(E, g, th, nmk.k, lane);
        } else if ((E.flags & AZX_FLAG_NO_COMPACT) ||
                   (long long)th->num_nodes + (long long)(E.selects_per_search + 1) * nmk.k <= (long long)E.cap) {
            if (lane == 0) { th->root_id = child; th->root_k = nmk.k; }
        } else {
            if (play_mode) {
                if (lane == 0) { th->root_id = child; th->root_k = nmk.k; th->defer_compact = 1; }
            } else {
                compact_tree(E, g, th, child, nmk.k, lane, sh_old);
            }
        }
        if (lane == 0) {
            gh->color = h.color;
            gh->winner = h.winner;
            gh->ply = ply;
            gh->move_id = -1;
            E.counters[(size_t)g * CTR_COUNT + CTR_PLIES] += 1ull;
        }
    }

    if (!play_mode || !(finished || errored)) return;

    const int rows = gh->n_rows;
    bool restart = true;
    if (finished) {
        const int result = h.winner == 2 ? 1 : 3;
        unsigned long long pos = 0;
        if (lane == 0) pos = atomicAdd(E.q_count, (unsigned long long)rows);
        pos = ((unsigned long long)__builtin_amdgcn_readfirstlane((int)(pos >> 32)) << 32) |
              (unsigned int)__builtin_amdgcn_readfirstlane((int)pos);
        if (!E.q_ring && pos + rows > (unsigned long long)E.q_cap) {
            if (lane == 0) {
                atomicAdd(E.q_count, (unsigned long long)(-(long long)rows));
                gh->active = 0;
                gh->parked = 1;
            }
            restart = false;
        } else {
            const size_t q0 = (size_t)(pos % (unsigned long long)E.q_cap);
            const int first = (int)min((unsigned long long)rows, (unsigned long long)E.q_cap - q0);
            auto copy16 = [&](void *dst, const void *src, int n16) {
// ... 280 lines not shown
#pragma unroll
            for (int s = 0; s < 4; ++s) empties_out[o * 4 + s] = (s < SLOTS && mk.k) ? mk.m[s < SLOTS ? s : 0] : 0ull;
        }
        h.step(moves[o] - 1, N, lane);
        if (lane == 0) result_out[o] = h.winner ? (h.winner == 2 ? 1 : 3) : 0;
    }
#pragma unroll
    for (int s = 0; s < SLOTS; ++s) {
        const int cell = s * 64 + lane;
        if (cell < ncells) final_board[(size_t)g * ncells + cell] = (int32_t)(h.c[s] & 3u);
    }
}

__global__ void k_arith(const float *a, const float *b, float *sq, float *dv, float *mul, int n) {
    const int i = blockIdx.x * blockDim.x + threadIdx.x;
    if (i < n) {
        sq[i] = sqrtf(a[i]);
        dv[i] = a[i] / (1.0f + b[i]);
        mul[i] = (0.75f * a[i]) * b[i] + a[i];
    }
}

__global__ void k_divide_test(const float *num, const float *den, float *q, float *rt, int n) {
    const int i = 2 * (blockIdx.x * blockDim.x + threadIdx.x);
    if (i + 1 < n) {
        const f2 a = {num[i], num[i + 1]}, d = {den[i], den[i + 1]};
        const f2 r = div2_unscaled(a, d);
        q[i] = r.x;
        q[i + 1] = r.y;
    } else if (i < n) {
        const f2 a = {num[i], num[i]}, d = {den[i], den[i]};
        q[i] = div2_unscaled(a, d).x;
    }
    for (int j = i; j < n && j < i + 2; ++j) {
        const int v = (int)den[j];
        rt[j] = (v >= 0 && v < AZX_SQRT_TAB) ? c_sqrt[v] : 0.0f;
    }
}

__global__ __launch_bounds__(64) void k_noise_test(float alpha, const float *tab, int k, int n_rows, uint32_t seed, float *out) {
    const int lane = threadIdx.x, row = blockIdx.x;
    if (row >= n_rows) return;
    uint64_t m[2];
    m[0] = k >= 64 ? ~0ull : ((1ull << k) - 1ull);
    m[1] = k > 64 ? ((1ull << (k - 64)) - 1ull) : 0ull;
    const GammaConst gc = gamma_const(alpha, tab);
    float nz[2];
    dirichlet_noise<2>(m, lane, mix32(seed ^ mix32((uint32_t)row + 0x632be5abu)), gc, 1.0f, nz);
    if (lane < k) out[(size_t)row * k + lane] = nz[0];
    if (64 + lane < k) out[(size_t)row * k + 64 + lane] = nz[1];
}

void azx_launch_noise_test(float alpha, const float *tab, int k, int n_rows, uint32_t seed, float *out, hipStream_t st) {
    hipLaunchKernelGGL(k_noise_test, dim3(n_rows), dim3(64), 0, st, alpha, tab, k, n_rows, seed, out);
}

namespace {
void ln_inc_gamma(double a, double x, double *lnP, double *lnQ) {
    const double lg = std::lgamma(a);
    if (x < a + 1.0) {
        double ap = a, sum = 1.0 / a, del = sum;
        for (int n = 0; n < 2000; ++n) {
            ap += 1.0;
            del *= x / ap;
            sum += del;
            if (std::fabs(del) < std::fabs(sum) * 1e-17) break;
        }
        *lnP = -x + a * std::log(x) + std::log(sum) - lg;
        const double P = std::exp(*lnP);
        *lnQ = P < 1.0 ? std::log1p(-P) : -1e300;
    } else {
        const double tiny = 1e-300;
        double b = x + 1.0 - a, c = 1.0 / tiny, d = 1.0 / b, h = d;
        for (int i = 1; i < 5000; ++i) {
            const double an = -i * (i - a);
            b += 2.0;
            d = an * d + b;
            if (std::fabs(d) < tiny) d = tiny;
            c = b + an / c;
            if (std::fabs(c) < tiny) c = tiny;
            d = 1.0 / d;
            const double del = d * c;
            h *= del;
            if (std::fabs(del - 1.0) < 1e-16) break;
        }
        *lnQ = -x + a * std::log(x) + std::log(h) - lg;
        const double Q = std::exp(*lnQ);
        *lnP = Q < 1.0 ? std::log1p(-Q) : -1e300;
    }
}
double ln_gamma_quantile_from_y(double a, double y) {
    const bool lower = y > 0.5;
    const double target = lower ? std::log1p(-y) : std::log(y);
    double lo = -800.0 / a - 50.0, hi = std::log(80.0);
    if (lower) {
        const double est = (target + std::lgamma(a + 1.0)) / a;
        lo = est - 2.0;
        hi = std::min(hi, est + 40.0);
    }
    for (int it = 0; it < 200; ++it) {
        const double mid = 0.5 * (lo + hi);
        double lp, lq;
        const double x = std::exp(mid);
        if (x <= 0.0) { lo = mid; continue; }
        ln_inc_gamma(a, x, &lp, &lq);
        const bool below = lower ? (lp < target) : (lq > target);
        if (below) lo = mid; else hi = mid;
    }
    return 0.5 * (lo + hi);
}
}

void azx_gamma_table(double alpha, float *tab) {
    const double ln2 = std::log(2.0);
    const double c0 = std::lgamma(alpha + 1.0) / ln2;
    for (int j = 0; j < AZX_GAMMA_TAB; ++j) {
        const int e = (j >> 5) - 25;
        const double y = std::ldexp(1.0 + (j & 31) / 32.0, e);
        double delta = 0.0;
        if (y < 1.0) {
            const double u = 1.0 - y;
            const double lx0 = (std::log2(u) + c0) / alpha;
            if (lx0 > -60.0) delta = ln_gamma_quantile_from_y(alpha, y) / ln2 - lx0;
        }
        tab[j] = (float)delta;
    }
    tab[AZX_GAMMA_TAB] = (float)c0;
}

#define DISPATCH_SLOTS(slots, CALL)                         \
    do {                                                    \
        if ((slots) <= 2) { CALL(2); }                      \
        else { CALL(3); }                                   \
    } while (0)

bool azx_mcts_fast_path(const DevEngine &E, int mode, bool force_generic) {
    return !force_generic && mode == (MODE_BEGIN | MODE_INLINE) && E.evaluator == AZX_EVAL_UNIFORM &&
           E.prior_default && (E.noise_scale == 0.0 || E.device_noise);
}

void azx_launch_mcts(const DevEngine &E, int mode, int num_batches, hipStream_t st, bool force_generic) {
    const size_t lds = azx_mcts_lds_bytes(E.ncells, E.bs);
    if (azx_mcts_fast_path(E, mode, force_generic)) {
#define CALL(S) hipLaunchKernelGGL((k_mcts<S, true>), dim3(E.G), dim3(64), lds, st, E, mode, num_batches)
        DISPATCH_SLOTS(E.slots, CALL);
#undef CALL
        return;
    }
#define CALL(S) hipLaunchKernelGGL((k_mcts<S, false>), dim3(E.G), dim3(64), lds, st, E, mode, num_batches)
    DISPATCH_SLOTS(E.slots, CALL);
#undef CALL
}

bool azx_launch_play(const DevEngine &E, int num_batches, int steps, hipStream_t st, bool allowed) {
    if (!allowed) return false;
    if (!(E.evaluator == AZX_EVAL_UNIFORM && E.prior_default && (E.noise_scale == 0.0 || E.device_noise))) return false;
    const size_t lds = azx_mcts_lds_bytes(E.ncells, E.bs);
#define CALL(S) hipLaunchKernelGGL((k_play<S>), dim3(E.G), dim3(64), lds, st, E, num_batches, steps)
    DISPATCH_SLOTS(E.slots, CALL);
#undef CALL
    return true;
}

void azx_launch_reset(const DevEngine &E, const int32_t *slots, int n_slots, const int32_t *moves,
                      const int32_t *n_moves, int stride, int assign_uid, hipStream_t st) {
#define CALL(S) hipLaunchKernelGGL((k_reset<S>), dim3(n_slots), dim3(64), 0, st, E, slots, n_slots, moves, n_moves, stride, assign_uid)
    DISPATCH_SLOTS(E.slots, CALL);
#undef CALL
}

void azx_launch_advance(const DevEngine &E, const int32_t *move_ids, int play_mode, hipStream_t st) {
#define CALL(S) hipLaunchKernelGGL((k_advance<S>), dim3(E.G), dim3(64), 0, st, E, move_ids, play_mode)
    DISPATCH_SLOTS(E.slots, CALL);
#undef CALL
}

void azx_launch_gather_root(const DevEngine &E, int32_t *k_out, int32_t *legal, float *cv, float *cw,
                            float *cp, float *rv, float *rw, int32_t *nn, float *sv, hipStream_t st) {
#define CALL(S) hipLaunchKernelGGL((k_gather_root<S>), dim3(E.G), dim3(64), 0, st, E, k_out, legal, cv, cw, cp, rv, rw, nn, sv)
    DISPATCH_SLOTS(E.slots, CALL);
#undef CALL
}

void azx_launch_choose(const DevEngine &E, hipStream_t st) {
#define CALL(S) hipLaunchKernelGGL((k_choose<S>), dim3(E.G), dim3(64), 0, st, E)
    DISPATCH_SLOTS(E.slots, CALL);
#undef CALL
}

void azx_launch_hex_replay(int N, int n_games, const int32_t *moves, const int32_t *length, int stride,
                           int32_t *result_out, int32_t *nlegal_out, uint64_t *empties_out,
                           int32_t *final_board, hipStream_t st) {
    const int slots = (N * N + 63) / 64;
#define CALL(S) hipLaunchKernelGGL((k_hex_replay<S>), dim3(n_games), dim3(64), 0, st, N, n_games, moves, length, stride, result_out, nlegal_out, empties_out, final_board)
    DISPATCH_SLOTS(slots, CALL);
#undef CALL
}

void azx_launch_divide_test(const float *num, const float *den, float *q, float *rt, int n, hipStream_t st) {
    hipLaunchKernelGGL(k_divide_test, dim3((n / 2 + 256) / 256), dim3(256), 0, st, num, den, q, rt, n);
}

void azx_launch_arith(const float *a, const float *b, float *sq, float *dv, float *mul, int n,
                      hipStream_t st) {
    hipLaunchKernelGGL(k_arith, dim3((n + 255) / 256), dim3(256), 0, st, a, b, sq, dv, mul, n);
}

#include "match_kernels.hip"
```

azalea_amd/csrc/net.h:

```cpp
#pragma once
#include <hip/hip_runtime.h>
#include <stdint.h>

#include "azx_dev.h"

struct AzxNet;

int azx_net_create(AzxNet **out, int N, int blocks, int chans, int max_evals, hipStream_t st);
void azx_net_destroy(AzxNet *net);
void azx_net_set_stream(AzxNet *net, hipStream_t st, const uint32_t *mask, int words);
const char *azx_net_error();
int azx_net_set_weights(AzxNet *net, int n, const char *const *names, const void *const *ptrs,
                        const int64_t *counts, int on_device);
bool azx_net_ready(const AzxNet *net);
int azx_net_check_range(AzxNet *net, hipStream_t st);
int azx_net_debug_weights(AzxNet *net, int which, void *out, int64_t cap, int64_t *nbytes, char *name, int name_cap);
const char *azx_net_kernel_info(const AzxNet *net);
void azx_net_eval(AzxNet *net, const DevEngine &d, hipStream_t st);
bool azx_net_rows_splittable(const AzxNet *net);
void azx_net_eval_rows(AzxNet *net, const DevEngine &d, int row0, int max_n, hipStream_t st);
constexpr int AZX_NET_ROW_ALIGN = 16;
void azx_net_eval_rows_behind(AzxNet *net, const DevEngine &d, int row0, int first, int max_n, int32_t *ctr, hipStream_t st);
int azx_net_forward_host(AzxNet *net, int B, int K, const int32_t *boards,
                         const int32_t *legal_moves, float *value, float *logprob, hipStream_t st);

int azx_net_wide_train_conv(int N, int C, const unsigned short *w16, const unsigned short *in, float *out32, int n_boards,
                            const float *unscale, float2 *stat, hipStream_t st);
int azx_net_wide_train_conv_bwd(int N, int C, const unsigned short *w16, const unsigned short *in, float *g_out, int n_boards,
                                const float *unscale, float2 *pgsum, const unsigned char *mask, const float *raw, const float *skip,
                                const double *sums, float invN, unsigned int *gmax, hipStream_t st);
```

azalea_amd/csrc/net_kernels.hip:

```cpp
#include "net_priv.h"

#ifndef AZX_NET_ABLATE
#define AZX_NET_ABLATE 0
#endif
#ifndef AZX_SAT_TRACK
#define AZX_SAT_TRACK 1
#endif

#include <cmath>
#include <cstdio>
#include <cstdlib>
#include <cstring>
#include <map>
#include <string>
#include <type_traits>
#include <vector>

typedef float f32x16 __attribute__((ext_vector_type(16)));

static thread_local std::string g_net_err;
const char *azx_net_error() { return g_net_err.c_str(); }

int azx_net_fail(int code, const char *msg) {
    g_net_err = msg;
// ... 916 lines not shown
    __shared__ unsigned char cells[(AZX_MAX_BOARD + 2) * (AZX_MAX_BOARD + 2) + 15];
    const int n_eval = n_eval_ptr ? *n_eval_ptr : n_eval_host;
    const int e = blockIdx.x;
    if (e >= n_eval) return;
    const int C = P.C, N = P.N, ncells = P.ncells, NT = C / 32, NH = N + 2;
    const int co_base = blockIdx.y * 128;
    const int tid = threadIdx.x, lane = tid & 63, wave = tid >> 6;
    const int wm = wave & 1, wn = wave >> 1;
    const int li = lane & 31, lh = lane >> 5;
    const size_t rowg = (size_t)C * 4;
    typedef _Float16 f16x4 __attribute__((ext_vector_type(4)));
    const uint8_t *bd = ev_board + (size_t)e * AZX_CELL_STRIDE;
    for (int i = tid; i < NH * NH; i += 256) {
        const int y = i / NH - 1, x = i - (y + 1) * NH - 1;
        cells[i] = (y >= 0 && y < N && x >= 0 && x < N) ? bd[y * N + x] : (uint8_t)3;
    }
    __syncthreads();
    uint32_t onehot[MW];
#pragma unroll
    for (int m = 0; m < MW; ++m) {
        onehot[m] = 0u;
        const int r = (MW * wm + m) * 32 + li;
        if (r < ncells) {
            const int ry = r / N, rx = r - ry * N;
            const unsigned char *c0 = cells + ry * NH + rx;
#pragma unroll
            for (int tap = 0; tap < 9; ++tap) {
                const uint32_t v = c0[(tap / 3) * NH + tap % 3];
                onehot[m] |= (v < 3u ? 1u : 0u) << (3 * tap + v);
            }
        }
    }
    f32x16 acc[MW][NW];
#pragma unroll
    for (int m = 0; m < MW; ++m)
#pragma unroll
        for (int n = 0; n < NW; ++n)
#pragma unroll
            for (int r = 0; r < 16; ++r) acc[m][n][r] = 0.0f;
    const uint4 *ws = reinterpret_cast<const uint4 *>(P.Ws);
    const int nt0 = co_base / 32 + 2 * wn;
#pragma unroll
    for (int kk = 0; kk < 2; ++kk) {
        f16x8 bfr[MW];
#pragma unroll
        for (int m = 0; m < MW; ++m) {
            const uint32_t byte = (onehot[m] >> (16 * kk + 8 * lh)) & 0xffu;
            uint4 q;
            q.x = ((byte >> 0) & 1u) * 0x3C00u | ((byte >> 1) & 1u) * 0x3C000000u;
            q.y = ((byte >> 2) & 1u) * 0x3C00u | ((byte >> 3) & 1u) * 0x3C000000u;
            q.z = ((byte >> 4) & 1u) * 0x3C00u | ((byte >> 5) & 1u) * 0x3C000000u;
            q.w = ((byte >> 6) & 1u) * 0x3C00u | ((byte >> 7) & 1u) * 0x3C000000u;
            bfr[m] = *reinterpret_cast<const f16x8 *>(&q);
        }
#pragma unroll
        for (int n = 0; n < NW; ++n) {
            const uint4 *pa = ws + ((size_t)(kk * NT + nt0 + n) * 2) * 64 + lane;
            const uint4 qh = pa[0], ql = pa[64];
            const f16x8 wh8 = *reinterpret_cast<const f16x8 *>(&qh);
            const f16x8 wl8 = *reinterpret_cast<const f16x8 *>(&ql);
#pragma unroll
            for (int m = 0; m < MW; ++m) {
                acc[m][n] = __builtin_amdgcn_mfma_f32_32x32x16_f16(wh8, bfr[m], acc[m][n], 0, 0, 0);
                acc[m][n] = __builtin_amdgcn_mfma_f32_32x32x16_f16(wl8, bfr[m], acc[m][n], 0, 0, 0);
            }
        }
    }
    unsigned char *gout = reinterpret_cast<unsigned char *>(out) + (size_t)e * ncells * rowg;
#pragma unroll
    for (int n = 0; n < NW; ++n) {
        const int cb0 = co_base + 64 * wn + 32 * n + 4 * lh;
#pragma unroll
        for (int g4 = 0; g4 < 4; ++g4) {
            const int cb = cb0 + 8 * g4;
            const float4 b4 = *reinterpret_cast<const float4 *>(P.stem_b + cb);
            const float bv[4] = {b4.x, b4.y, b4.z, b4.w};
#pragma unroll
            for (int m = 0; m < MW; ++m) {
                const int r = (MW * wm + m) * 32 + li;
                if (r < ncells) {
                    f16x4 h4, l4;
                    float vv[4];
#pragma unroll
                    for (int j = 0; j < 4; ++j) {
                        const float v = fmaxf(acc[m][n][4 * g4 + j] + bv[j], 0.0f);
                        vv[j] = v;
                        if (AZX_SAT_TRACK) satmax = fmaxf(satmax, v);
                        _Float16 hi, lo;
                        split_f16(v, hi, lo);
                        h4[j] = hi;
                        l4[j] = lo;
                    }
                    *reinterpret_cast<f16x4 *>(gout + (size_t)r * rowg + cb * 2) = h4;
                    *reinterpret_cast<f16x4 *>(gout + (size_t)r * rowg + (size_t)C * 2 + cb * 2) = l4;
                    if (out32)
                        *reinterpret_cast<float4 *>(out32 + ((size_t)e * ncells + r) * C + cb) =
                            make_float4(vv[0], vv[1], vv[2], vv[3]);
                }
            }
        }
    }
    if (satmax > 65504.0f) atomicOr(P.sat_flag, 1u);
}

__global__ void k_stem_generic(NetDev P, const uint8_t *ev_board, const int32_t *n_eval_ptr,
                               int n_eval_host, int max_n, float *out) {
    const int n_eval = min(n_eval_ptr ? *n_eval_ptr : n_eval_host, max_n);
    const int C = P.C, N = P.N, ncells = P.ncells;
    const size_t total = (size_t)n_eval * ncells * C;
    for (size_t idx = (size_t)blockIdx.x * blockDim.x + threadIdx.x; idx < total;
         idx += (size_t)gridDim.x * blockDim.x) {
        const int co = idx % C;
        const int pos = (idx / C) % ncells;
        const size_t e = idx / ((size_t)C * ncells);
        const uint8_t *bd = ev_board + e * AZX_CELL_STRIDE;
        const int y = pos / N, x = pos - y * N;
        float acc = P.stem_b[co];
        for (int tap = 0; tap < 9; ++tap) {
            const int yy = y + tap / 3 - 1, xx = x + tap % 3 - 1;
            if (yy >= 0 && yy < N && xx >= 0 && xx < N)
                acc += P.stemT[(tap * 3 + bd[yy * N + xx]) * C + co];
        }
        out[idx] = fmaxf(acc, 0.0f);
    }
}

__global__ void k_conv_generic(NetDev P, int layer, const float *in, const float *residual,
                               const int32_t *n_eval_ptr, int n_eval_host, int max_n, float *out) {
    const int n_eval = min(n_eval_ptr ? *n_eval_ptr : n_eval_host, max_n);
    const int C = P.C, N = P.N, ncells = P.ncells;
    const float *w = P.Wg + (size_t)layer * 9 * C * C;
    const size_t total = (size_t)n_eval * ncells * C;
    for (size_t idx = (size_t)blockIdx.x * blockDim.x + threadIdx.x; idx < total;
         idx += (size_t)gridDim.x * blockDim.x) {
        const int co = idx % C;
        const int pos = (idx / C) % ncells;
        const size_t e = idx / ((size_t)C * ncells);
        const int y = pos / N, x = pos - y * N;
        float acc = 0.0f;
        for (int tap = 0; tap < 9; ++tap) {
            const int yy = y + tap / 3 - 1, xx = x + tap % 3 - 1;
            if (yy < 0 || yy >= N || xx < 0 || xx >= N) continue;
            const float *ip = in + (e * ncells + yy * N + xx) * C;
            const float *wp = w + (size_t)tap * C * C + co;
            for (int ci = 0; ci < C; ++ci) acc += ip[ci] * wp[(size_t)ci * C];
        }
        float v = acc + P.bias[layer * C + co];
        if (residual) v += residual[idx];
        out[idx] = fmaxf(v, 0.0f);
    }
}

#define HM_MB 16
__global__ __launch_bounds__(256, 3) void k_heads_mfma(NetDev P, const float *__restrict__ hfeat,
                                                       const uint8_t *__restrict__ ev_board,
                                                       const int32_t *__restrict__ ev_flip,
                                                       const int32_t *__restrict__ n_eval_ptr, int n_eval_host,
                                                       float *__restrict__ logit_out, float *__restrict__ value_out,
                                                       float *__restrict__ prior_out) {
    extern __shared__ __align__(16) float hsm[];
    const int n_eval = n_eval_ptr ? *n_eval_ptr : n_eval_host;
    const int e0 = blockIdx.x * HM_MB;
    if (e0 >= n_eval) return;
    const int nb = min(HM_MB, n_eval - e0);
    const int tid = threadIdx.x, lane = tid & 63, wave = tid >> 6;
    const int li = lane & 15, lk = lane >> 4;
    const int N = P.N, ncells = P.ncells, LDA = P.hm_lda;
    const int KV = 2 * ncells, KP = 4 * ncells, KVp = (KV + 15) & ~15, KPp = (KP + 15) & ~15;
    const int QV = KVp / 16, QP = KPp / 16, nf = 6 * ncells;
    float *A = hsm;
    uint8_t cellv[HM_MB / 4][2];
    int flipv[HM_MB / 4];
#pragma unroll
    for (int bi = 0; bi < HM_MB / 4; ++bi) {
        const int b = wave + 4 * bi, e = e0 + (b < nb ? b : 0);
        cellv[bi][0] = ev_board[(size_t)e * AZX_CELL_STRIDE + lane];
        cellv[bi][1] = ev_board[(size_t)e * AZX_CELL_STRIDE + 64 + lane];
        flipv[bi] = ev_flip[e];
    }
    {
        const int nf2 = 3 * ncells, total = nb * nf2;
        const float2 *src = reinterpret_cast<const float2 *>(hfeat + (size_t)e0 * nf);
        constexpr int INFL = 24;
        for (int f0 = 0; f0 < total; f0 += 256 * INFL) {
            float2 v[INFL];
#pragma unroll
            for (int j = 0; j < INFL; ++j) {
                const int f = f0 + tid + 256 * j;
                v[j] = src[f < total ? f : total - 1];
            }
#pragma unroll
            for (int j = 0; j < INFL; ++j) {
                const int f = f0 + tid + 256 * j;
                if (f < total) {
                    const int b = f / nf2, i = 2 * (f - b * nf2);
                    *reinterpret_cast<float2 *>(A + (size_t)b * LDA + (i < KV ? i : KVp + (i - KV))) = v[j];
                }
            }
        }
        for (int b = wave; b < HM_MB; b += 4) {
            float *row = A + (size_t)b * LDA;
            if (b < nb) {
                if (lane < KVp - KV) row[KV + lane] = 0.0f;
                if (lane < KPp - KP) row[KVp + KP + lane] = 0.0f;
            } else {
                for (int i = lane; i < KVp + KPp; i += 64) row[i] = 0.0f;
            }
        }
    }
    __syncthreads();
    const int NTP = (ncells + 15) / 16;
    typedef float f32x4_ __attribute__((ext_vector_type(4)));
    f32x4_ accp[2] = {f32x4_{0.f, 0.f, 0.f, 0.f}, f32x4_{0.f, 0.f, 0.f, 0.f}};
    constexpr int AH = 6;
    {
        const int t0 = min(2 * wave, NTP - 1), t1 = min(2 * wave + 1, NTP - 1);
        const float4 *w0 = reinterpret_cast<const float4 *>(P.hmP) + (size_t)t0 * QP * 64 + lane;
        const float4 *w1 = reinterpret_cast<const float4 *>(P.hmP) + (size_t)t1 * QP * 64 + lane;
        const float *ap = A + (size_t)li * LDA + KVp + 4 * lk;
        float4 bq0[AH], bq1[AH];
#pragma unroll
        for (int u = 0; u < AH; ++u) { bq0[u] = w0[(size_t)min(u, QP - 1) * 64]; bq1[u] = w1[(size_t)min(u, QP - 1) * 64]; }
        if (2 * wave < NTP)
        for (int q0 = 0; q0 < QP; q0 += AH) {
#pragma unroll
            for (int u = 0; u < AH; ++u) {
                const int q = q0 + u;
                const float4 b0 = bq0[u], b1 = bq1[u];
                bq0[u] = w0[(size_t)min(q + AH, QP - 1) * 64];
                bq1[u] = w1[(size_t)min(q + AH, QP - 1) * 64];
                if (q < QP) {
                    const float4 a4 = *reinterpret_cast<const float4 *>(ap + 16 * q);
                    accp[0] = __builtin_amdgcn_mfma_f32_16x16x4f32(a4.x, b0.x, accp[0], 0, 0, 0);
                    accp[1] = __builtin_amdgcn_mfma_f32_16x16x4f32(a4.x, b1.x, accp[1], 0, 0, 0);
                    accp[0] = __builtin_amdgcn_mfma_f32_16x16x4f32(a4.y, b0.y, accp[0], 0, 0, 0);
                    accp[1] = __builtin_amdgcn_mfma_f32_16x16x4f32(a4.y, b1.y, accp[1], 0, 0, 0);
                    accp[0] = __builtin_amdgcn_mfma_f32_16x16x4f32(a4.z, b0.z, accp[0], 0, 0, 0);
                    accp[1] = __builtin_amdgcn_mfma_f32_16x16x4f32(a4.z, b1.z, accp[1], 0, 0, 0);
                    accp[0] = __builtin_amdgcn_mfma_f32_16x16x4f32(a4.w, b0.w, accp[0], 0, 0, 0);
                    accp[1] = __builtin_amdgcn_mfma_f32_16x16x4f32(a4.w, b1.w, accp[1], 0, 0, 0);
                }
            }
        }
    }
    f32x4_ accv = f32x4_{0.f, 0.f, 0.f, 0.f};
    {
        const float4 *wv = reinterpret_cast<const float4 *>(P.hmV) + (size_t)wave * QV * 64 + lane;
        const float *ap = A + (size_t)li * LDA + 4 * lk;
        float4 bq[AH];
#pragma unroll
        for (int u = 0; u < AH; ++u) bq[u] = wv[(size_t)min(u, QV - 1) * 64];
        for (int qb = 0; qb < QV; qb += AH) {
#pragma unroll
            for (int u = 0; u < AH; ++u) {
                const int q = qb + u;
                const float4 b4 = bq[u];
                bq[u] = wv[(size_t)min(q + AH, QV - 1) * 64];
                if (q < QV) {
                    const float4 a4 = *reinterpret_cast<const float4 *>(ap + 16 * q);
                    accv = __builtin_amdgcn_mfma_f32_16x16x4f32(a4.x, b4.x, accv, 0, 0, 0);
                    accv = __builtin_amdgcn_mfma_f32_16x16x4f32(a4.y, b4.y, accv, 0, 0, 0);
                    accv = __builtin_amdgcn_mfma_f32_16x16x4f32(a4.z, b4.z, accv, 0, 0, 0);
                    accv = __builtin_amdgcn_mfma_f32_16x16x4f32(a4.w, b4.w, accv, 0, 0, 0);
                }
            }
        }
    }
    __syncthreads();
    float (*lg)[AZX_CELL_STRIDE] = reinterpret_cast<float (*)[AZX_CELL_STRIDE]>(hsm);
    float (*h2)[64] = reinterpret_cast<float (*)[64]>(hsm + HM_MB * AZX_CELL_STRIDE);
#pragma unroll
    for (int tt = 0; tt < 2; ++tt) {
        const int j = 16 * (2 * wave + tt) + li;
        if (2 * wave + tt < NTP && j < ncells) {
            const float bias = P.mfcb[j];
#pragma unroll
            for (int r = 0; r < 4; ++r) {
                const int b = 4 * lk + r;
                const float logit = accp[tt][r] + bias;
                lg[b][j] = logit;
                if (b < nb) logit_out[(size_t)(e0 + b) * AZX_CELL_STRIDE + j] = logit;
            }
        }
    }
#pragma unroll
    for (int r = 0; r < 4; ++r) h2[4 * lk + r][16 * wave + li] = accv[r];
    __syncthreads();
    if (tid < nb) {
        float acc = 0.f;
        for (int i = 0; i < 64; ++i) acc += fmaxf(h2[tid][i] + P.fc2b[i], 0.f) * P.fc3w[i];
        value_out[e0 + tid] = tanhf(acc + P.fc3b[0]);
    }
    if (!prior_out) return;
#pragma unroll
    for (int bi = 0; bi < HM_MB / 4; ++bi) {
        const int b = wave + 4 * bi;
        if (b >= nb) break;
        const int e = e0 + b;
        float x[2];
        bool legal[2];
        float mx = -INFINITY;
#pragma unroll
        for (int s2 = 0; s2 < 2; ++s2) {
            const int cell = s2 * 64 + lane;
            legal[s2] = cell < ncells && cellv[bi][s2] == 0;
            x[s2] = legal[s2] ? lg[b][cell] : -INFINITY;
            mx = fmaxf(mx, x[s2]);
        }
        mx = wave_max(mx);
        float sum = 0.f;
#pragma unroll
        for (int s2 = 0; s2 < 2; ++s2) sum += legal[s2] ? expf(x[s2] - mx) : 0.f;
        const float lse = mx + logf(wave_sum(sum));
        const int flip = flipv[bi];
#pragma unroll
        for (int s2 = 0; s2 < 2; ++s2) {
            const int cell = s2 * 64 + lane;
            if (cell < ncells) {
                int oc = cell;
                if (flip) {
                    const int i = cell / N, j = cell - i * N;
                    oc = (N - 1 - j) * N + (N - 1 - i);
                }
                prior_out[(size_t)e * AZX_CELL_STRIDE + oc] = legal[s2] ? expf(x[s2] - lse) : 0.f;
            }
        }
    }
}

#ifndef HEADS_BPB
#define HEADS_BPB 8
#endif
#ifndef HEADS_KSPLIT
#define HEADS_KSPLIT 1
#endif
__global__ __launch_bounds__(192 * HEADS_KSPLIT) void k_heads(NetDev P, const float *__restrict__ act,
                                               const float *__restrict__ hfeat,
                                               const uint8_t *__restrict__ ev_board,
                                               const int32_t *__restrict__ ev_flip,
                                               const int32_t *__restrict__ n_eval_ptr,
                                               int n_eval_host, float *__restrict__ logit_out,
                                               float *__restrict__ value_out,
                                               float *__restrict__ prior_out) {
    extern __shared__ __align__(16) float hsm[];
    const int n_eval = n_eval_ptr ? *n_eval_ptr : n_eval_host;
    const int e0 = blockIdx.x * HEADS_BPB;
    if (e0 >= n_eval) return;
    const int nb = min(HEADS_BPB, n_eval - e0);
    const int tid = threadIdx.x;
    const int part = tid / 192, t = tid - 192 * part;
    const int C = P.C, N = P.N, ncells = P.ncells;
    typedef float (*rowsB)[HEADS_BPB];
    rowsB hv = reinterpret_cast<rowsB>(hsm);
    rowsB hp = reinterpret_cast<rowsB>(hsm + 2 * ncells * HEADS_BPB);
    rowsB h2 = reinterpret_cast<rowsB>(hsm + 6 * ncells * HEADS_BPB);
    float (*lg)[AZX_CELL_STRIDE] = reinterpret_cast<float (*)[AZX_CELL_STRIDE]>(hsm + (6 * ncells + 64) * HEADS_BPB);
    float *psum = hsm + (6 * ncells + 64) * HEADS_BPB + HEADS_BPB * AZX_CELL_STRIDE;

    if (hfeat != nullptr) {
        const int nf = 6 * ncells;
        constexpr int NTH = 192 * HEADS_KSPLIT;
        constexpr int NFT = (6 * AZX_MAX_CELLS + NTH - 1) / NTH;
#pragma unroll 2
        for (int b = 0; b < HEADS_BPB; ++b) {
            float v[NFT];
            const float *src = hfeat + (size_t)(e0 + (b < nb ? b : 0)) * nf;
#pragma unroll
            for (int j = 0; j < NFT; ++j) {
                const int f = tid + NTH * j;
                v[j] = src[f < nf ? f : nf - 1];
            }
#pragma unroll
            for (int j = 0; j < NFT; ++j) {
                const int f = tid + NTH * j;
                if (f < nf) {
                    const float x = b < nb ? v[j] : 0.0f;
                    if (f < 2 * ncells) hv[f][b] = x; else hp[f - 2 * ncells][b] = x;
                }
            }
        }
    } else if (tid < ncells) {
        for (int b = 0; b < HEADS_BPB; ++b) {
            float v0 = 0.f, v1 = 0.f, p0 = 0.f, p1 = 0.f, p2 = 0.f, p3 = 0.f;
            if (b < nb) {
                const float4 *a = reinterpret_cast<const float4 *>(act + ((size_t)(e0 + b) * ncells + tid) * C);
                for (int c4 = 0; c4 < C / 4; ++c4) {
                    const float4 x = a[c4];
                    const float xs[4] = {x.x, x.y, x.z, x.w};
#pragma unroll
                    for (int j = 0; j < 4; ++j) {
                        const int c = 4 * c4 + j;
                        v0 += xs[j] * P.wv[c];
                        v1 += xs[j] * P.wv[C + c];
                        p0 += xs[j] * P.wp[c];
                        p1 += xs[j] * P.wp[C + c];
                        p2 += xs[j] * P.wp[2 * C + c];
                        p3 += xs[j] * P.wp[3 * C + c];
                    }
                }
                for (int c = (C / 4) * 4; c < C; ++c) {
                    const float x = act[((size_t)(e0 + b) * ncells + tid) * C + c];
                    v0 += x * P.wv[c]; v1 += x * P.wv[C + c];
                    p0 += x * P.wp[c]; p1 += x * P.wp[C + c]; p2 += x * P.wp[2 * C + c]; p3 += x * P.wp[3 * C + c];
                }
            }
            hv[tid][b] = fmaxf(v0 + P.bv[0], 0.f);
            hv[ncells + tid][b] = fmaxf(v1 + P.bv[1], 0.f);
            hp[tid][b] = fmaxf(p0 + P.bp[0], 0.f);
            hp[ncells + tid][b] = fmaxf(p1 + P.bp[1], 0.f);
            hp[2 * ncells + tid][b] = fmaxf(p2 + P.bp[2], 0.f);
            hp[3 * ncells + tid][b] = fmaxf(p3 + P.bp[3], 0.f);
        }
    }
    __syncthreads();
    float acc2[HEADS_BPB], accm[HEADS_BPB];
#pragma unroll
    for (int b = 0; b < HEADS_BPB; ++b) { acc2[b] = 0.f; accm[b] = 0.f; }
    if (t < 64) {
        const int i0 = (2 * ncells * part) / HEADS_KSPLIT, i1 = (2 * ncells * (part + 1)) / HEADS_KSPLIT;
#pragma unroll 8
        for (int i = i0; i < i1; ++i) {
            const float w = P.fc2T[i * 64 + t];
#pragma unroll
            for (int b4 = 0; b4 < HEADS_BPB / 4; ++b4) {
                const float4 x = *reinterpret_cast<const float4 *>(&hv[i][4 * b4]);
                acc2[4 * b4] += x.x * w; acc2[4 * b4 + 1] += x.y * w; acc2[4 * b4 + 2] += x.z * w; acc2[4 * b4 + 3] += x.w * w;
            }
        }
    }
    if (t < ncells) {
        const int i0 = (4 * ncells * part) / HEADS_KSPLIT, i1 = (4 * ncells * (part + 1)) / HEADS_KSPLIT;
#pragma unroll 8
        for (int i = i0; i < i1; ++i) {
            const float w = P.mfcT[(size_t)i * AZX_CELL_STRIDE + t];
#pragma unroll
            for (int b4 = 0; b4 < HEADS_BPB / 4; ++b4) {
                const float4 x = *reinterpret_cast<const float4 *>(&hp[i][4 * b4]);
                accm[4 * b4] += x.x * w; accm[4 * b4 + 1] += x.y * w; accm[4 * b4 + 2] += x.z * w; accm[4 * b4 + 3] += x.w * w;
            }
        }
    }
    if (HEADS_KSPLIT > 1) {
        if (part > 0) {
            float *ps = psum + (size_t)(part - 1) * (64 + 192) * HEADS_BPB;
#pragma unroll
            for (int b = 0; b < HEADS_BPB; ++b) {
                if (t < 64) ps[b * 64 + t] = acc2[b];
                if (t < ncells) ps[64 * HEADS_BPB + b * 192 + t] = accm[b];
            }
        }
        __syncthreads();
        if (part == 0) {
            for (int pp = 0; pp < HEADS_KSPLIT - 1; ++pp) {
                const float *ps = psum + (size_t)pp * (64 + 192) * HEADS_BPB;
#pragma unroll
                for (int b = 0; b < HEADS_BPB; ++b) {
                    if (t < 64) acc2[b] += ps[b * 64 + t];
                    if (t < ncells) accm[b] += ps[64 * HEADS_BPB + b * 192 + t];
                }
            }
        }
    }
    if (part == 0 && t < 64) {
#pragma unroll
        for (int b = 0; b < HEADS_BPB; ++b) h2[t][b] = fmaxf(acc2[b] + P.fc2b[t], 0.f);
    }
    if (part == 0 && t < ncells) {
        const float bias = P.mfcb[t];
#pragma unroll
        for (int b = 0; b < HEADS_BPB; ++b) {
            const float logit = accm[b] + bias;
            lg[b][t] = logit;
            if (b < nb) logit_out[(size_t)(e0 + b) * AZX_CELL_STRIDE + t] = logit;
        }
    }
    __syncthreads();
    if (tid < nb) {
        float acc = 0.f;
        for (int i = 0; i < 64; ++i) acc += h2[i][tid] * P.fc3w[i];
        value_out[e0 + tid] = tanhf(acc + P.fc3b[0]);
    }
    if (!prior_out) return;
    const int lane = tid & 63, wave = tid >> 6;
    for (int b = wave; b < nb; b += 3 * HEADS_KSPLIT) {
        const int e = e0 + b;
        float x[3];
        bool legal[3];
        float mx = -INFINITY;
#pragma unroll
        for (int s = 0; s < 3; ++s) {
            const int cell = s * 64 + lane;
            legal[s] = cell < ncells && ev_board[(size_t)e * AZX_CELL_STRIDE + cell] == 0;
            x[s] = legal[s] ? lg[b][cell] : -INFINITY;
            mx = fmaxf(mx, x[s]);
        }
        mx = wave_max(mx);
        float sum = 0.f;
#pragma unroll
        for (int s = 0; s < 3; ++s) sum += legal[s] ? expf(x[s] - mx) : 0.f;
        const float lse = mx + logf(wave_sum(sum));
        const int flip = ev_flip[e];
#pragma unroll
        for (int s = 0; s < 3; ++s) {
            const int cell = s * 64 + lane;
            if (cell < ncells) {
                int oc = cell;
                if (flip) {
                    const int i = cell / N, j = cell - i * N;
                    oc = (N - 1 - j) * N + (N - 1 - i);
                }
                prior_out[(size_t)e * AZX_CELL_STRIDE + oc] = legal[s] ? expf(x[s] - lse) : 0.f;
            }
        }
    }
}



static int raise_lds_limits() {
    const int cap = 160 * 1024;
    const void *fns[] = {(const void *)k_tower_f16x3_s16, (const void *)k_conv_wide_f16x3_s16,
                         (const void *)k_tower_mfma<64, 4, 2, 1, 2>, (const void *)k_tower_mfma<64, 6, 1, 2, 2>,
                         (const void *)k_tower_mfma<32, 6, 2, 2, 1>, (const void *)k_heads_mfma, (const void *)k_heads};
    for (const void *f : fns)
        if (hipFuncSetAttribute(f, hipFuncAttributeMaxDynamicSharedMemorySize, cap) != hipSuccess)
            return nfail(AZX_EHIP, "net: raising a tower kernel's dynamic LDS limit failed");
    return AZX_OK;
}

int azx_net_create(AzxNet **out, int N, int blocks, int chans, int max_evals, hipStream_t st) {
    if (N < 2 || N > AZX_MAX_BOARD) return nfail(AZX_EINVAL, "net: board size out of range");
    if (blocks < 0 || chans < 1) return nfail(AZX_EINVAL, "net: bad num_blocks/base_chans");
    if (int rc = raise_lds_limits()) return rc;
    AzxNet *net = new AzxNet();
    memset(&net->d, 0, sizeof net->d);
    net->d.N = N;
    net->d.ncells = N * N;
    net->d.C = chans;
    net->d.blocks = blocks;
    net->d.layers = 2 * blocks;
    net->max_evals = max_evals;
    net->stream = st;
    const int ncells = N * N;
    const char *force = getenv("AZX_TOWER");
    const bool want_fp32 = force && !strcmp(force, "fp32");
    if (chans == 64 && ncells <= 121 && blocks >= 1 && !want_fp32) net->tower_variant = 4;
    else if (chans == 64 && ncells <= 128) net->tower_variant = 1;
    else if (chans == 64 && ncells <= 192) net->tower_variant = 2;
    else if (chans == 32 && ncells <= 192) net->tower_variant = 3;
    else if (chans % 128 == 0 && ncells <= 192 && !want_fp32) net->tower_variant = 5;
    net->use_mfma = net->tower_variant != 0;
    { const char *v = getenv("AZX_WIDE_STREAMS"); net->opt_wsplit = std::min(4, std::max(1, v ? atoi(v) : 2)); }
    { const char *v = getenv("AZX_HEADS"); net->opt_heads_mfma = !(v && !strcmp(v, "valu")); }
    { const char *v = getenv("AZX_PACK"); net->pack_on_host = v && !strcmp(v, "host"); }
    {
        char b[260];
        const char *tower = "k_stem_generic + k_conv_generic (VALU)";
        if (net->tower_variant == 4) tower = "k_tower_f16x3_s16";
        else if (net->tower_variant == 5) tower = "k_stem_wide_f16x3 + k_conv_wide_f16x3_s16 per layer";
        else if (net->tower_variant == 1) tower = "k_tower_mfma<64,4,2,1,2> (fp32 MFMA)";
        else if (net->tower_variant == 2) tower = "k_tower_mfma<64,6,1,2,2> (fp32 MFMA)";
        else if (net->tower_variant == 3) tower = "k_tower_mfma<32,6,2,2,1> (fp32 MFMA)";
        const bool hm = net->tower_variant == 4 && net->opt_heads_mfma && ncells <= 128;
        snprintf(b, sizeof b, "%s + %s (%dx%d on %dx%d; AZX_TOWER=%s AZX_WIDE_STREAMS=%d AZX_HEADS=%s AZX_PACK=%s)",
                 tower, hm ? "k_heads_mfma" : "k_heads", blocks, chans, N, N, want_fp32 ? "fp32" : "default",
                 net->opt_wsplit, net->opt_heads_mfma ? "mfma" : "valu", net->pack_on_host ? "host" : "device");
        net->info = b;
    }
    const size_t E = max_evals;
    net->act = nalloc<float>(net, E * ncells * chans);
    net->logit = nalloc<float>(net, E * AZX_CELL_STRIDE);
    if (net->tower_variant == 4) net->hfeat = nalloc<float>(net, E * 6 * ncells);
    net->hb_board = nalloc<uint8_t>(net, E * AZX_CELL_STRIDE);
    net->hb_flip = nalloc<int32_t>(net, E);
    net->hb_value = nalloc<float>(net, E);
    if (!net->use_mfma) {
        net->act2 = nalloc<float>(net, E * ncells * chans);
        net->act3 = nalloc<float>(net, E * ncells * chans);
    }
    if (net->tower_variant == 5) {
        net->wideX = nalloc<unsigned short>(net, E * ncells * chans * 2);
        net->wideY = nalloc<unsigned short>(net, E * ncells * chans * 2);
    }
    if (!net->act || !net->logit || !net->hb_board || !net->hb_flip || !net->hb_value ||
        (!net->use_mfma && (!net->act2 || !net->act3)) || (net->tower_variant == 5 && (!net->wideX || !net->wideY))) {
        azx_net_destroy(net);
        return nfail(AZX_ENOMEM, "net: hipMalloc failed");
    }
    const int bpb = net->tower_variant == 2 ? 1 : 2;
    net->lds_bytes = (size_t)bpb * 2 * (ncells + 1) * (chans + 4) * sizeof(float);
    if (net->tower_variant == 4) net->lds_bytes = (size_t)F16X3_BPB * 128 * 272 + 2 * 272;
    if (net->tower_variant == 5) net->lds_bytes = (size_t)(ncells + 2) * WIDE_ROWB;
    net->d.sat_flag = nalloc<uint32_t>(net, 4);
    if (!net->d.sat_flag || hipDeviceSynchronize() != hipSuccess) {
        azx_net_destroy(net);
        return nfail(AZX_ENOMEM, "net: hipMalloc failed");
    }
    *out = net;
    return AZX_OK;
}

void azx_net_set_stream(AzxNet *net, hipStream_t st, const uint32_t *mask, int words) {
    if (!net) return;
    for (int i = 0; i < 3; ++i) {
        if (net->stream2[i]) { (void)hipStreamSynchronize(net->stream2[i]); (void)hipStreamDestroy(net->stream2[i]); }
        if (net->ev_join[i]) (void)hipEventDestroy(net->ev_join[i]);
        net->stream2[i] = nullptr;
        net->ev_join[i] = nullptr;
    }
    if (net->ev_fork) (void)hipEventDestroy(net->ev_fork);
    net->ev_fork = nullptr;
    net->streams_ok = false;
    net->cu_mask.assign(mask, mask + (mask ? words : 0));
    net->stream = st;
}

void azx_net_destroy(AzxNet *net) {
    if (net) {
        for (int i = 0; i < 3; ++i) {
            if (net->stream2[i]) { (void)hipStreamSynchronize(net->stream2[i]); (void)hipStreamDestroy(net->stream2[i]); }
            if (net->ev_join[i]) (void)hipEventDestroy(net->ev_join[i]);
            net->stream2[i] = nullptr;
            net->ev_join[i] = nullptr;
        }
        if (net->ev_fork) (void)hipEventDestroy(net->ev_fork);
        net->ev_fork = nullptr;
    }
#ifdef AZX_NET_STAMP
    {
        unsigned long long h[10] = {0};
        if (hipMemcpyFromSymbol(h, HIP_SYMBOL(g_wide_stamp), sizeof h) == hipSuccess && h[7]) {
            static const char *nm[6] = {"prologue (bias + residual, setup)", "barrier after staging", "k-loops (MFMA)", "epilogue (stores acknowledged)",
                                        "barrier before staging (skew)", "staging: requests, round trips, LDS writes"};
            unsigned long long tot = 0;
            for (int r = 0; r < 6; ++r) tot += h[r];
            fprintf(stderr, "k_conv_wide_f16x3_s16 stamps over %llu waves: %.0f cycles/wave, shader clock %.0f MHz during the kernel\n",
                    h[7], (double)tot / h[7], h[8] ? 100.0 * (double)tot / (double)h[8] : 0.0);
            for (int r = 0; r < 6; ++r)
                fprintf(stderr, "  %-44s %6.1f%%  %9.0f cycles/wave\n", nm[r], 100.0 * h[r] / tot, (double)h[r] / h[7]);
            unsigned long long z[10] = {0};
            (void)hipMemcpyToSymbol(HIP_SYMBOL(g_wide_stamp), z, sizeof z);
        }
    }
    {
        unsigned long long h[10] = {0};
        if (hipMemcpyFromSymbol(h, HIP_SYMBOL(g_tower_stamp), sizeof h) == hipSuccess && h[7]) {
            static const char *nm[7] = {"stem", "residual load/setup", "k-loop (MFMA)", "barrier after k-loop",
                                        "epilogue", "barrier after epilogue", "output store"};
            unsigned long long tot = 0;
            for (int r = 0; r < 7; ++r) tot += h[r];
            fprintf(stderr, "k_tower_f16x3_s16 stamps over %llu blocks: %.0f cycles/block, shader clock %.0f MHz during the kernel\n",
                    h[7], (double)tot / h[7], h[8] ? 100.0 * (double)tot / (double)h[8] : 0.0);
            for (int r = 0; r < 7; ++r)
                fprintf(stderr, "  %-24s %6.1f%%  %9.0f cycles/block\n", nm[r], 100.0 * h[r] / tot, (double)h[r] / h[7]);
            {
                std::vector<unsigned long long> tr(3 * 32768);
                (void)hipMemcpyFromSymbol(tr.data(), HIP_SYMBOL(g_tower_trace), tr.size() * sizeof(unsigned long long));
                std::map<unsigned long long, std::vector<std::pair<unsigned long long, unsigned long long>>> cu;
                unsigned long long t0 = ~0ull, t1 = 0;
                size_t nblk = 0;
                for (int b = 0; b < 32768; ++b)
                    if (tr[3 * b + 2]) {
                        cu[tr[3 * b]].push_back({tr[3 * b + 1], tr[3 * b + 2]});
                        t0 = std::min(t0, tr[3 * b + 1]);
                        t1 = std::max(t1, tr[3 * b + 2]);
                        ++nblk;
                    }
                double busy = 0, mn = 1e30, mx = 0, lastend_min = 1e30, lastend_max = 0;
                size_t cmin = 1 << 30, cmax = 0;
                for (auto &kv : cu) {
                    double b = 0, le = 0;
                    for (auto &iv : kv.second) { b += (double)(iv.second - iv.first); le = std::max(le, (double)(iv.second - t0)); }
                    busy += b; mn = std::min(mn, b); mx = std::max(mx, b);
                    cmin = std::min(cmin, kv.second.size()); cmax = std::max(cmax, kv.second.size());
                    lastend_min = std::min(lastend_min, le); lastend_max = std::max(lastend_max, le);
                }
                fprintf(stderr, "  last launch: %zu blocks on %zu CUs, span %.1f us, blocks/CU %zu..%zu, mean resident blocks/CU %.2f, "
                        "per-CU block-time %.0f..%.0f us, CU finish %.0f..%.0f us\n", nblk, cu.size(), (t1 - t0) / 100.0, cmin, cmax,
                        busy / ((double)(t1 - t0) * cu.size()), mn / 100.0, mx / 100.0, lastend_min / 100.0, lastend_max / 100.0);
            }
            int nb = -1;
            (void)hipOccupancyMaxActiveBlocksPerMultiprocessor(&nb, (const void *)k_tower_f16x3_s16, F16X3_BPB * 128, net->lds_bytes);
            hipFuncAttributes fa;
            memset(&fa, 0, sizeof fa);
            (void)hipFuncGetAttributes(&fa, (const void *)k_tower_f16x3_s16);
            fprintf(stderr, "  runtime occupancy: %d blocks/CU (dynamic LDS %zu B, static %zu B, %d VGPRs, max threads %d)\n", nb,
                    net->lds_bytes, (size_t)fa.sharedSizeBytes, fa.numRegs, fa.maxThreadsPerBlock);
        }
    }
#endif
    if (!net) return;
    for (void *p : net->allocs) (void)hipFree(p);
    if (net->raw_tab_host) (void)hipHostFree((void *)net->raw_tab_host);
    if (net->wmax_host) (void)hipHostFree((void *)net->wmax_host);
    delete net;
}

bool azx_net_ready(const AzxNet *net) { return net && net->ready; }


static void run_net(AzxNet *net, const uint8_t *boards, const int32_t *flip, const int32_t *n_eval_ptr,
                    int n_host, int max_n, float *logit, float *value, float *prior, hipStream_t st, size_t row0 = 0) {
    const NetDev &d = net->d;
    if (max_n <= 0) return;
    const size_t act_rows = row0 * d.ncells * d.C;
    float *const act = net->act + act_rows;
    float *const act2 = net->act2 ? net->act2 + act_rows : nullptr;
    float *const act3 = net->act3 ? net->act3 + act_rows : nullptr;
    float *const hfeat_rows = net->hfeat ? net->hfeat + row0 * 6 * d.ncells : nullptr;
    const float *hfeat = nullptr;
    if (net->use_mfma) {
        const size_t lds = net->lds_bytes;
        if (net->tower_variant == 4) {
            const dim3 grid((max_n + F16X3_BPB - 1) / F16X3_BPB), block(F16X3_BPB * 128);
            hipLaunchKernelGGL(k_tower_f16x3_s16, grid, block, lds, st, d, boards, n_eval_ptr, n_host, (float *)nullptr, hfeat_rows);
            hfeat = hfeat_rows;
        } else if (net->tower_variant == 5) {
            const dim3 grid(max_n, d.C / 128), block(256);
            hipLaunchKernelGGL(k_stem_wide_f16x3, grid, block, 0, st, d, boards, net->wideX,
                               d.blocks == 0 ? net->act : (float *)nullptr, n_eval_ptr, n_host);
            const int wsplit = net->opt_wsplit;
            {
                int parts = wsplit;
                if (parts > 1 && !net->ev_fork) {
                    bool ok = hipEventCreateWithFlags(&net->ev_fork, hipEventDisableTiming) == hipSuccess;
                    for (int i = 0; i < 3 && ok; ++i)
                        ok = (net->cu_mask.empty() ? hipStreamCreateWithFlags(&net->stream2[i], hipStreamNonBlocking)
                                                   : hipExtStreamCreateWithCUMask(&net->stream2[i], (uint32_t)net->cu_mask.size(), net->cu_mask.data())) == hipSuccess &&
                             hipEventCreateWithFlags(&net->ev_join[i], hipEventDisableTiming) == hipSuccess;
                    net->streams_ok = ok;
                }
                if (parts > 1 && !net->streams_ok) parts = 1;
                const int per = (((max_n + parts - 1) / parts + 7) / 8) * 8;
                if (per >= max_n) parts = 1;
                if (parts > 1 && hipEventRecord(net->ev_fork, st) != hipSuccess) parts = 1;
                for (int part = 1; part < parts; ++part)
                    if (hipStreamWaitEvent(net->stream2[part - 1], net->ev_fork, 0) != hipSuccess) { parts = 1; break; }
                const int per_ok = parts > 1 ? per : max_n;
                for (int part = 0; part < parts; ++part) {
                    hipStream_t s = part ? net->stream2[part - 1] : st;
                    const int e0 = part * per_ok, e1 = std::min(max_n, e0 + per_ok);
                    if (e1 <= e0) continue;
                    const dim3 g(8 * (d.C / 128), (e1 - e0 + 7) / 8);
                    for (int b = 0; b < d.blocks; ++b) {
                        hipLaunchKernelGGL(k_conv_wide_f16x3_s16, g, block, lds, s, d, 2 * b, (const unsigned short *)net->wideX, net->wideY,
                                           (const unsigned short *)nullptr, (float *)nullptr, n_eval_ptr, n_host, e0, e1);
                        hipLaunchKernelGGL(k_conv_wide_f16x3_s16, g, block, lds, s, d, 2 * b + 1, (const unsigned short *)net->wideY, net->wideX,
                                           (const unsigned short *)net->wideX, b == d.blocks - 1 ? net->act : (float *)nullptr, n_eval_ptr, n_host, e0, e1);
                    }
                    if (part) {
                        if (hipEventRecord(net->ev_join[part - 1], s) != hipSuccess ||
                            hipStreamWaitEvent(st, net->ev_join[part - 1], 0) != hipSuccess)
                            (void)hipStreamSynchronize(s);
                    }
                }
            }
        } else if (net->tower_variant == 1) {
            hipLaunchKernelGGL((k_tower_mfma<64, 4, 2, 1, 2>), dim3((max_n + 1) / 2), dim3(256), lds, st, d, boards, n_eval_ptr, n_host, act);
        } else if (net->tower_variant == 2) {
            hipLaunchKernelGGL((k_tower_mfma<64, 6, 1, 2, 2>), dim3(max_n), dim3(256), lds, st, d, boards, n_eval_ptr, n_host, act);
        } else {
            hipLaunchKernelGGL((k_tower_mfma<32, 6, 2, 2, 1>), dim3((max_n + 1) / 2), dim3(256), lds, st, d, boards, n_eval_ptr, n_host, act);
        }
    } else {
        const int grid = 2048;
        hipLaunchKernelGGL(k_stem_generic, dim3(grid), dim3(256), 0, st, d, boards, n_eval_ptr, n_host, max_n, act);
        float *x = act, *y = act2, *z = act3;
        for (int b = 0; b < d.blocks; ++b) {
            hipLaunchKernelGGL(k_conv_generic, dim3(grid), dim3(256), 0, st, d, 2 * b, x, (const float *)nullptr, n_eval_ptr, n_host, max_n, y);
            hipLaunchKernelGGL(k_conv_generic, dim3(grid), dim3(256), 0, st, d, 2 * b + 1, y, x, n_eval_ptr, n_host, max_n, z);
            std::swap(x, z);
        }
        if (x != act)
            (void)hipMemcpyAsync(act, x, (size_t)max_n * d.ncells * d.C * sizeof(float), hipMemcpyDeviceToDevice, st);
    }
    if (hfeat != nullptr && net->opt_heads_mfma && d.ncells <= 128) {
        const size_t hl = std::max((size_t)HM_MB * d.hm_lda, (size_t)HM_MB * AZX_CELL_STRIDE + (size_t)HM_MB * 64) * sizeof(float);
        hipLaunchKernelGGL(k_heads_mfma, dim3((max_n + HM_MB - 1) / HM_MB), dim3(256), hl, st, d, hfeat, boards, flip, n_eval_ptr, n_host, logit, value, prior);
    } else {
        const size_t hl = ((size_t)(6 * d.ncells + 64) * HEADS_BPB + (size_t)HEADS_BPB * AZX_CELL_STRIDE +
                           (size_t)(HEADS_KSPLIT - 1) * (64 + 192) * HEADS_BPB) * sizeof(float);
        hipLaunchKernelGGL(k_heads, dim3((max_n + HEADS_BPB - 1) / HEADS_BPB), dim3(192 * HEADS_KSPLIT), hl, st, d, act, hfeat, boards, flip, n_eval_ptr, n_host, logit, value, prior);
    }
}

const char *azx_net_kernel_info(const AzxNet *net) { return net->info.c_str(); }

int azx_net_check_range(AzxNet *net, hipStream_t st) {
    if (!net || !net->d.sat_flag) return AZX_OK;
    uint32_t flag = 0;
    if (hipMemcpyAsync(&flag, net->d.sat_flag, sizeof flag, hipMemcpyDeviceToHost, st) != hipSuccess ||
        hipStreamSynchronize(st) != hipSuccess)
        return nfail(AZX_EHIP, "net: reading the activation range flag failed");
    if (!flag) return AZX_OK;
    (void)hipMemsetAsync(net->d.sat_flag, 0, sizeof flag, st);
    return nfail(AZX_ERANGE, "net: an activation of the residual tower exceeded the f16 range (65504) of the split-f16 "
                             "kernels -- the evaluations of this call are not valid (AZX_TOWER=fp32 runs the fp32 MFMA tower)");
}

void azx_net_eval(AzxNet *net, const DevEngine &e, hipStream_t st) {
    run_net(net, e.ev_board, e.ev_flip, e.n_eval, 0, net->max_evals, net->logit, e.ev_value, e.ev_prior, st);
}

bool azx_net_rows_splittable(const AzxNet *net) { return net && !(net->use_mfma && net->tower_variant == 5); }

void azx_net_eval_rows(AzxNet *net, const DevEngine &e, int row0, int max_n, hipStream_t st) {
    run_net(net, e.ev_board, e.ev_flip, e.n_eval, 0, max_n, net->logit + (size_t)row0 * AZX_CELL_STRIDE, e.ev_value,
            e.ev_prior, st, (size_t)row0);
}

__global__ void k_rows_behind(const int32_t *__restrict__ n_eval_ptr, int first, int32_t *__restrict__ ctr) {
    if (threadIdx.x != 0 || blockIdx.x != 0) return;
    const int n = *n_eval_ptr;
    const int rest = n > first ? n - first : 0;
    ctr[0] = rest;
    ctr[1] = n;
    ctr[2] = ctr[2] + 1;
    ctr[3] = ctr[3] + (rest == 0 ? 1 : 0);
}

static_assert(AZX_NET_ROW_ALIGN % HM_MB == 0 && AZX_NET_ROW_ALIGN % HEADS_BPB == 0 && AZX_NET_ROW_ALIGN % F16X3_BPB == 0 &&
              AZX_NET_ROW_ALIGN % 2 == 0, "AZX_NET_ROW_ALIGN: whole blocks of k_tower_f16x3_s16, k_tower_mfma (1 or 2 boards), k_heads_mfma, k_heads");
void azx_net_eval_rows_behind(AzxNet *net, const DevEngine &e, int row0, int first, int max_n, int32_t *ctr, hipStream_t st) {
    if (first <= 0 || first >= max_n) return;
    hipLaunchKernelGGL(k_rows_behind, dim3(1), dim3(64), 0, st, (const int32_t *)e.n_eval, first, ctr);
    const size_t f = (size_t)first;
    run_net(net, e.ev_board + f * AZX_CELL_STRIDE, e.ev_flip + f, ctr, 0, max_n - first,
            net->logit + ((size_t)row0 + f) * AZX_CELL_STRIDE, e.ev_value + f, e.ev_prior + f * AZX_CELL_STRIDE, st,
            (size_t)row0 + f);
}

int azx_net_forward_host(AzxNet *net, int B, int K, const int32_t *boards, const int32_t *legal_moves,
                         float *value, float *logprob, hipStream_t st) {
    if (!net->ready) return nfail(AZX_ESTATE, "net: azx_set_weights has not been called");
    if (B < 0 || K < 0 || (B && (!boards || !legal_moves || !value || !logprob)))
        return nfail(AZX_EINVAL, "net: bad forward arguments");
    const NetDev &d = net->d;
    const int ncells = d.ncells;
    std::vector<uint8_t> hb((size_t)net->max_evals * AZX_CELL_STRIDE);
    std::vector<float> hl((size_t)net->max_evals * AZX_CELL_STRIDE), hv(net->max_evals);
    for (int b0 = 0; b0 < B; b0 += net->max_evals) {
        const int nb = std::min(net->max_evals, B - b0);
        std::fill(hb.begin(), hb.end(), 0);
        for (int i = 0; i < nb; ++i)
            for (int c = 0; c < ncells; ++c) {
                const int32_t v = boards[(size_t)(b0 + i) * ncells + c];
                if (v < 0 || v > 2) return nfail(AZX_EINVAL, "net: board values must be 0/1/2");
                hb[(size_t)i * AZX_CELL_STRIDE + c] = (uint8_t)v;
            }
        if (hipMemcpyAsync(net->hb_board, hb.data(), (size_t)nb * AZX_CELL_STRIDE, hipMemcpyHostToDevice, st) != hipSuccess)
            return nfail(AZX_EHIP, "net: H2D copy failed");
        run_net(net, net->hb_board, net->hb_flip, nullptr, nb, nb, net->logit, net->hb_value, nullptr, st);
        if (hipGetLastError() != hipSuccess) return nfail(AZX_EHIP, "net: kernel launch failed");
        if (hipMemcpyAsync(hl.data(), net->logit, (size_t)nb * AZX_CELL_STRIDE * sizeof(float), hipMemcpyDeviceToHost, st) != hipSuccess ||
            hipMemcpyAsync(hv.data(), net->hb_value, (size_t)nb * sizeof(float), hipMemcpyDeviceToHost, st) != hipSuccess ||
            hipStreamSynchronize(st) != hipSuccess)
            return nfail(AZX_EHIP, "net: D2H copy failed");
        for (int i = 0; i < nb; ++i) {
            value[b0 + i] = hv[i];
            const int32_t *lm = legal_moves + (size_t)(b0 + i) * K;
            float *lp = logprob + (size_t)(b0 + i) * K;
            float mx = -INFINITY;
            for (int j = 0; j < K; ++j) {
                if (lm[j] < 0 || lm[j] > ncells) return nfail(AZX_EINVAL, "net: legal move out of range");
                const int tile = lm[j] > 0 ? lm[j] - 1 : 0;
                lp[j] = lm[j] == 0 ? -99.0f : hl[(size_t)i * AZX_CELL_STRIDE + tile];
                mx = std::max(mx, lp[j]);
            }
            double sum = 0.0;
            for (int j = 0; j < K; ++j) sum += std::exp((double)lp[j] - (double)mx);
            const float lse = (float)((double)mx + std::log(sum));
            for (int j = 0; j < K; ++j) lp[j] = lp[j] - lse;
        }
    }
    return AZX_OK;
}
```

azalea_amd/csrc/net_priv.h:

```cpp
#pragma once
#include <hip/hip_runtime.h>
#include <stdint.h>

#include <algorithm>
#include <string>
#include <vector>

#include "net.h"

struct NetDev {
    int N, ncells, C, blocks, layers;
    const float *stemT;
    const float *stem_b;
    const unsigned short *Ws;
    const unsigned short *Ws16, *Wh16;
    const unsigned short *Whd16;
    const float *hbias16;
    const float *Wp;
    const float *Wg;
    const float *bias;
    const float *wv, *bv;
    const float *wp, *bp;
    const float *fc2T, *fc2b;
    const float *fc3w, *fc3b;
    const float *mfcT, *mfcb;
    const float *hmP, *hmV;
    int hm_lda;
    uint32_t *sat_flag;
};

#ifndef AZX_LO_BITS
#define AZX_LO_BITS 10
#endif
#define LO_MASK ((0xFFFFu << (10 - AZX_LO_BITS)) & 0xFFFFu)
#define LO_RND (AZX_LO_BITS < 10 ? (1u << (9 - AZX_LO_BITS)) : 0u)
static inline unsigned short lo_round_bits(unsigned short bits) {
    return (unsigned short)((bits + LO_RND) & LO_MASK);
}

struct AzxNet {
    NetDev d;
    int max_evals = 0;
    bool ready = false;
    bool use_mfma = false;
    hipStream_t stream = nullptr;
    std::vector<void *> allocs;
    float *act = nullptr, *act2 = nullptr, *act3 = nullptr;
    unsigned short *wideX = nullptr, *wideY = nullptr;
    float *logit = nullptr;
    float *hfeat = nullptr;
    uint8_t *hb_board = nullptr;
    int32_t *hb_flip = nullptr;
    float *hb_value = nullptr;
    size_t lds_bytes = 0;
    int tower_variant = 0;
    hipStream_t stream2[3] = {nullptr, nullptr, nullptr};
    std::vector<uint32_t> cu_mask;
    hipEvent_t ev_fork = nullptr, ev_join[3] = {nullptr, nullptr, nullptr};
    bool streams_ok = false;
    int opt_wsplit = 2;
    bool opt_heads_mfma = true;
    std::string info;
    bool pack_on_host = false;
    bool packed_once = false;
    const float **raw_tab = nullptr;
    const float **raw_tab_host = nullptr;
    int raw_slots = 0;
    float *raw_arena = nullptr;
    size_t raw_arena_floats = 0;
    double *fold = nullptr;
    uint32_t *wmax = nullptr;
    uint32_t *wmax_host = nullptr;
    struct PackBuf { std::string name; void *ptr; size_t bytes; };
    std::vector<PackBuf> packs;
};

int azx_net_fail(int code, const char *msg);

template <typename T>
static T *nalloc(AzxNet *net, size_t count) {
    void *p = nullptr;
    if (hipMalloc(&p, std::max<size_t>(count * sizeof(T), 16)) != hipSuccess) return nullptr;
    (void)hipMemset(p, 0, std::max<size_t>(count * sizeof(T), 16));
    net->allocs.push_back(p);
    return reinterpret_cast<T *>(p);
}
```

azalea_amd/engine.py:

```python
import ctypes as C

import numpy as np

from . import _lib
from ._lib import (EVAL_EXTERNAL, EVAL_RESNET, EVAL_UNIFORM, EVAL_UNIFORM_HASH,
                   FLAG_NO_COMPACT, AzxError, Config, MatchStats, PlayStats, check)


def _p(a, ctype):
    return None if a is None else a.ctypes.data_as(C.POINTER(ctype))


class _DeviceArray:

    def __init__(self, ptr, shape, typestr):
        self.__cuda_array_interface__ = {"shape": tuple(shape), "typestr": typestr, "data": (int(ptr), False),
                                         "version": 2, "strides": None}


class Engine:
    def __init__(self, board_size=11, n_games=1, simulations=400, search_batch_size=10,
                 exploration_coef=0.5, exploration_depth=15, noise_alpha=0.03, noise_scale=0.25,
                 temperature=1.0, evaluator=EVAL_UNIFORM, num_blocks=6, base_chans=64,
                 nodes_per_game=0, flags=0, device=0, seed=0xBAD5EED5,
# ... 171 lines not shown
        check(self.L.azx_get_leaves(self.h, cap, _p(boards, C.c_int32), _p(lm, C.c_int32),
                                    _p(slot, C.c_int32), _p(k, C.c_int32), C.byref(n)))
        n = n.value
        return boards[:n], lm[:n], slot[:n], k[:n]

    def put_evals(self, value, prior):
        v = np.ascontiguousarray(value, np.float32)
        p = np.zeros((len(v), self.cells), np.float32)
        pr = np.asarray(prior, np.float32)
        if len(v):
            p[:, :pr.shape[1]] = pr
        check(self.L.azx_put_evals(self.h, len(v), _p(v, C.c_float), _p(p, C.c_float)))

    def get_evals(self):
        cap = self.G * self.bs
        v = np.zeros(cap, np.float32)
        p = np.zeros((cap, self.cells), np.float32)
        n = C.c_int(0)
        check(self.L.azx_get_evals(self.h, cap, _p(v, C.c_float), _p(p, C.c_float), C.byref(n)))
        return v[:n.value], p[:n.value]

    def search_recorded(self, noise=None, noise_scale=0.0):
        tape = []
        n = self.search_begin(noise, noise_scale)
        while True:
            if n:
                b, lm, slot, k = self.get_leaves()
                v, p = self.get_evals()
                for i in range(len(k)):
                    tape.append((int(slot[i]), int(k[i]), np.float32(v[i]), p[i, :k[i]].copy()))
            n, done = self.search_step()
            if done:
                break
        return tape

    def search_external(self, evaluate, noise=None, noise_scale=0.0):
        n = self.search_begin(noise, noise_scale)
        while True:
            if n:
                b, lm, slot, k = self.get_leaves()
                v, p = evaluate(b, lm, slot, k)
                self.put_evals(v, p)
            n, done = self.search_step()
            if done:
                break

    def get_root(self):
        G, Cn = self.G, self.cells
        out = dict(k=np.zeros(G, np.int32), legal_moves=np.zeros((G, Cn), np.int32),
                   child_visits=np.zeros((G, Cn), np.float32),
                   child_value=np.zeros((G, Cn), np.float32),
                   child_prior=np.zeros((G, Cn), np.float32), root_visits=np.zeros(G, np.float32),
                   root_value=np.zeros(G, np.float32), num_nodes=np.zeros(G, np.int32),
                   search_value=np.zeros(G, np.float32))
        check(self.L.azx_get_root(
            self.h, _p(out["k"], C.c_int32), _p(out["legal_moves"], C.c_int32),
            _p(out["child_visits"], C.c_float), _p(out["child_value"], C.c_float),
            _p(out["child_prior"], C.c_float), _p(out["root_visits"], C.c_float),
            _p(out["root_value"], C.c_float), _p(out["num_nodes"], C.c_int32),
            _p(out["search_value"], C.c_float)))
        return out

    def get_status(self):
        st = np.zeros(self.G, np.int32)
        check(self.L.azx_get_status(self.h, _p(st, C.c_int32)))
        return st

    def get_tree_nodes(self):
        nn = np.zeros(self.G, np.int32)
        check(self.L.azx_get_tree_nodes(self.h, _p(nn, C.c_int32)))
        return nn

    def get_games(self):
        G = self.G
        board = np.zeros((G, self.n, self.n), np.int32)
        color, result, ply = (np.zeros(G, np.int32) for _ in range(3))
        check(self.L.azx_get_games(self.h, _p(board, C.c_int32), _p(color, C.c_int32),
                                   _p(result, C.c_int32), _p(ply, C.c_int32)))
        return dict(board=board, color=color, result=result, ply=ply)

    def advance(self, move_ids):
        m = np.ascontiguousarray(move_ids, np.int32)
        assert m.shape == (self.G,)
        check(self.L.azx_advance(self.h, _p(m, C.c_int32)))

    def tree_dump(self, slot=0, cap=None):
        if cap is None:
            cap = int(self.get_root()["num_nodes"][slot]) + 8
        arrs = dict(parent=np.zeros(cap, np.int32), first_child=np.zeros(cap, np.int32),
                    num_children=np.zeros(cap, np.int32), num_visits=np.zeros(cap, np.float32),
                    total_value=np.zeros(cap, np.float32), prior_prob=np.zeros(cap, np.float32))
        nn, rid = C.c_int32(0), C.c_int32(0)
        check(self.L.azx_tree_dump(
            self.h, slot, cap, _p(arrs["parent"], C.c_int32), _p(arrs["first_child"], C.c_int32),
            _p(arrs["num_children"], C.c_int32), _p(arrs["num_visits"], C.c_float),
            _p(arrs["total_value"], C.c_float), _p(arrs["prior_prob"], C.c_float),
            C.byref(nn), C.byref(rid)))
        out = {k: v[:nn.value].copy() for k, v in arrs.items()}
        out["num_nodes"], out["root_id"] = nn.value, rid.value
        return out

    def forward(self, boards, legal_moves):
        b = np.ascontiguousarray(boards, np.int32)
        lm = np.ascontiguousarray(legal_moves, np.int32)
        B, K = lm.shape
        value = np.zeros(B, np.float32)
        logprob = np.zeros((B, K), np.float32)
        check(self.L.azx_forward(self.h, B, K, _p(b, C.c_int32), _p(lm, C.c_int32),
                                 _p(value, C.c_float), _p(logprob, C.c_float)))
        return value, logprob

    def play(self, min_positions, max_plies=0):
        cap = int(min_positions) + self.G * self.cells
        board = np.zeros((cap, self.n, self.n), np.int32)
        color = np.zeros(cap, np.int32)
        nlegal = np.zeros(cap, np.int32)
        prob = np.zeros((cap, self.cells), np.float32)
        reward = np.zeros(cap, np.float32)
        uid = np.zeros(cap, np.int64)
        st = PlayStats()
        self._check(self.L.azx_play(self.h, int(min_positions), int(max_plies), cap,
                              _p(board, C.c_int32), _p(color, C.c_int32), _p(nlegal, C.c_int32),
                              _p(prob, C.c_float), _p(reward, C.c_float), _p(uid, C.c_int64),
                              C.byref(st)))
        n = st.positions
        self._last_rows = int(n)
        return dict(board=board[:n], color=color[:n], nlegal=nlegal[:n], moves_prob=prob[:n],
                    reward=reward[:n], game_uid=uid[:n]), st.as_dict()

    ROW_METRIC_COLUMNS = (("search_value", 0), ("search_root_width", 1), ("action_logprob", 2),
                          ("search_root_visits", 4), ("search_tree_nodes", 5), ("search_root_children", 6))

    def game_metric_sums(self, rows=None):
        m = self.play_row_metrics(rows)
        names = [k for k, _ in self.ROW_METRIC_COLUMNS]
        if len(m) == 0:
            return dict.fromkeys(names, 0.0)
        starts = np.flatnonzero(m[:, 3] > 0.5)
        if len(starts) == 0 or starts[0] != 0:
            starts = np.r_[0, starts]
        cols = [c for _, c in self.ROW_METRIC_COLUMNS]
        sums = np.add.reduceat(m[:, cols].astype(np.float64), starts, axis=0)
        lens = np.diff(np.r_[starts, len(m)])
        return dict(zip(names, (sums / lens[:, None]).sum(0).tolist()))

    def play_row_metrics(self, rows=None):
        cap = int(rows) if rows is not None else self._last_rows
        m = np.zeros((max(1, cap), _lib.ROW_METRICS), np.float32)
        n = C.c_int64(0)
        check(self.L.azx_play_row_metrics(self.h, max(1, cap), _p(m, C.c_float), C.byref(n)))
        return m[:n.value]

    def kernel_info(self):
        buf = C.create_string_buffer(1024)
        n = self.L.azx_kernel_info(self.h, buf, len(buf))
        if n < 0:
            check(n)
        return buf.value.decode()

    def debug_set_queue_cap(self, rows):
        check(self.L.azx_debug_set_queue_cap(self.h, int(rows)))

    def debug_stagger(self):
        out = np.zeros(4, np.int32)
        check(self.L.azx_debug_stagger(self.h, _p(out, C.c_int32)))
        return dict(zip(("rows_behind", "rows_queued", "starts", "empty"), out.tolist()))

    def play_device(self, min_positions, max_plies=0):
        st = PlayStats()
        rows = C.c_int64(0)
        self._check(self.L.azx_play_device(self.h, int(min_positions), int(max_plies), C.byref(rows), C.byref(st)))
        self._last_rows = int(rows.value)
        return rows.value, st.as_dict()

    def rows_pack(self, first, n, records_ptr):
        check(self.L.azx_rows_pack(self.h, int(first), int(n), C.c_void_p(int(records_ptr))))

    def replay_put_records(self, n, records_ptr):
        check(self.L.azx_replay_put_records(self.h, int(n), C.c_void_p(int(records_ptr))))

    def replay_put_records_async(self, n, records_ptr, stream):
        check(self.L.azx_replay_put_records_async(self.h, int(n), C.c_void_p(int(records_ptr)), C.c_void_p(int(stream))))

    def reserve_cus(self, cus_per_xcd):
        out = C.c_int(0)
        check(self.L.azx_reserve_cus(self.h, int(cus_per_xcd), C.byref(out)))
        return out.value

    @property
    def record_bytes(self):
        return _lib.record_bytes(self.cells)

    def debug_counters(self):
        out = np.zeros(16, np.uint64)
        check(self.L.azx_debug_counters(self.h, _p(out, C.c_uint64)))
        return out

    def replay_create(self, capacity):
        check(self.L.azx_replay_create(self.h, int(capacity)))

    def replay_state(self):
        v = [C.c_int64(0) for _ in range(3)]
        check(self.L.azx_replay_state(self.h, *(C.byref(x) for x in v)))
        return dict(capacity=v[0].value, size=v[1].value, write_idx=v[2].value)

    def replay_set_state(self, size, write_idx):
        check(self.L.azx_replay_set_state(self.h, int(size), int(write_idx)))

    def replay_put(self, board, color, nlegal, moves_prob, reward):
        P = len(reward)
        cells = self.n * self.n
        board = np.ascontiguousarray(board, np.int32).reshape(P, cells)
        prob = np.ascontiguousarray(moves_prob, np.float32).reshape(P, cells)
        color = np.ascontiguousarray(color, np.int32)
        nlegal = np.ascontiguousarray(nlegal, np.int32)
        reward = np.ascontiguousarray(reward, np.float32)
        check(self.L.azx_replay_put(self.h, P, _p(board, C.c_int32), _p(color, C.c_int32),
                                    _p(nlegal, C.c_int32), _p(prob, C.c_float), _p(reward, C.c_float)))

    def replay_fill(self, min_positions, max_plies=0):
        st = PlayStats()
        rows = C.c_int64(0)
        self._check(self.L.azx_replay_fill(self.h, int(min_positions), int(max_plies), C.byref(rows), C.byref(st)))
        self._last_rows = int(rows.value)
        return rows.value, st.as_dict()

    def replay_collate(self, indices, out):
        idx = np.ascontiguousarray(indices, np.int64)
        mk = C.c_int32(0)
        check(self.L.azx_replay_collate(self.h, len(idx), _p(idx, C.c_int64),
                                        *(C.c_void_p(int(out[k])) for k in
                                          ("color", "legal_moves", "result", "board", "moves_prob", "reward")),
                                        C.byref(mk)))
        return mk.value

    def replay_set_mover_view(self, on: bool):
        check(self.L.azx_replay_set_mover_view(self.h, 1 if on else 0))

    def replay_collate_async(self, indices, out, stream):
        idx = np.ascontiguousarray(indices, np.int64)
        check(self.L.azx_replay_collate_async(self.h, len(idx), _p(idx, C.c_int64),
                                              *(C.c_void_p(int(out[k])) for k in
                                                ("color", "legal_moves", "result", "board", "moves_prob", "reward")),
                                              C.c_void_p(int(stream))))

    def debug_choose(self):
        mid = np.zeros(self.G, np.int32)
        prob = np.zeros((self.G, self.cells), np.float32)
        check(self.L.azx_debug_choose(self.h, _p(mid, C.c_int32), _p(prob, C.c_float)))
        return mid, prob

    def debug_counters_raw(self):
        out = np.zeros((self.G, 16), np.uint64)
        check(self.L.azx_debug_counters_raw(self.h, _p(out, C.c_uint64), self.G))
        return out

    def play_steps(self, plies):
        st = PlayStats()
        self._check(self.L.azx_play_steps(self.h, int(plies), C.byref(st)))
        return st.as_dict()


class Match:

    def __init__(self, engine_a, engine_b):
        self.L = _lib.lib()
        self.a, self.b = engine_a, engine_b
        self.cells = engine_a.cells
        self.h = C.c_void_p()
        check(self.L.azx_match_create(engine_a.h, engine_b.h, C.byref(self.h)))

    def close(self):
        if getattr(self, "h", None) is not None and self.h:
            self.L.azx_match_destroy(self.h)
            self.h = None

    def __del__(self):
        try:
            self.close()
        except Exception:
            pass

    def play(self, n_games, first_game=0, moves=False):
        n = int(n_games)
        outcome = np.zeros(n, np.int8)
        length = np.zeros(n, np.int16)
        mv = np.zeros((n, self.cells), np.int16) if moves else None
        st = MatchStats()
        self.a._ext_exc = self.b._ext_exc = None
        rc = self.L.azx_match_play(self.h, int(first_game), n, _p(outcome, C.c_int8), _p(length, C.c_int16),
                                   _p(mv, C.c_int16), C.byref(st))
        exc = self.a._ext_exc if self.a._ext_exc is not None else self.b._ext_exc
        self.a._ext_exc = self.b._ext_exc = None
        if rc != 0 and exc is not None:
            try:
                check(rc)
            except AzxError as err:
                raise exc from err
        check(rc)
        out = dict(outcome=outcome, length=length, stats=st.as_dict())
        if moves:
            out["moves"] = mv
        return out


class Tournament:

# ... 109 lines not shown
```

Baseline: 5.272 million.

## Alternate n_eval counters cleared in-kernel and add chunked-LDS heads MFMA kernel

```diff
diff --git a/azalea_amd/csrc/azx_capi.cpp b/azalea_amd/csrc/azx_capi.cpp
--- a/azalea_amd/csrc/azx_capi.cpp
+++ b/azalea_amd/csrc/azx_capi.cpp
@@ -103,6 +103,7 @@
     bool no_persistent = false;
     bool pipeline = true;
     bool stagger = true;
+    bool neval_memset = false;
     hipStream_t stream_b = nullptr;
     std::vector<uint32_t> cu_mask;
     hipEvent_t ev_fork = nullptr, ev_join = nullptr, ev_stagger = nullptr;
@@ -178,6 +179,7 @@
     { const char *v = getenv("AZX_NO_PERSISTENT"); e->no_persistent = v && atoi(v) != 0; }
     { const char *v = getenv("AZX_PIPELINE"); e->pipeline = !(v && atoi(v) == 0); }
     { const char *v = getenv("AZX_PIPELINE_STAGGER"); e->stagger = !(v && atoi(v) == 0); }
+    { const char *v = getenv("AZX_NEVAL_RESET"); e->neval_memset = v && !strcmp(v, "memset"); }
     HIPCHECK(hipStreamCreateWithFlags(&e->stream, hipStreamNonBlocking));
     DevEngine &d = e->d;
     memset(&d, 0, sizeof d);
@@ -353,6 +355,20 @@
     return v;
 }
 
+static void neval_views(const azx_engine *e, const DevEngine &base, int h, DevEngine v[3]) {
+    v[0] = v[1] = v[2] = base;
+    v[0].n_eval = v[2].n_eval = e->d.n_eval + h;
+    v[1].n_eval = e->neval_memset ? v[0].n_eval : e->d.n_eval + 2 + h;
+    v[0].n_eval_clear = e->neval_memset ? nullptr : v[1].n_eval;
+    v[1].n_eval_clear = e->neval_memset ? nullptr : v[0].n_eval;
+    v[2].n_eval_clear = nullptr;
+}
+
+static int neval_begin(azx_engine *e) {
+    if (!e->neval_memset) HIPCHECK(hipMemsetAsync(e->d.n_eval, 0, 4 * sizeof(int32_t), e->stream));
+    return AZX_OK;
+}
+
 static int pipeline_streams(azx_engine *e) {
     if (!e->stream_b) {
         if (e->cu_mask.empty()) HIPCHECK(hipStreamCreateWithFlags(&e->stream_b, hipStreamNonBlocking));
@@ -383,13 +399,20 @@
                                           : e->stagger     ? "phases + k_choose + k_advance per move, two half-pools on two streams half an evaluation apart (any tower)"
                                                            : "phases + k_choose + k_advance per move, two half-pools on two streams");
     }
+    int hole_v = 0;
+    size_t hole_l = 0;
+    azx_net_hole(e->net, &hole_v, &hole_l);
+    ENGINE_GUARD(e);
+    const std::string tree_fp = azx_mcts_footprint(d, hole_v, hole_l);
     std::string text = std::string("tree=") + tree + "; play=" + play + "; net=" +
                        (e->net ? azx_net_kernel_info(e->net) : "none") +
                        "; switches: AZX_MCTS_GENERIC=" + (e->force_generic ? "1" : "0") +
                        " AZX_NO_PERSISTENT=" + (e->no_persistent ? "1" : "0") +
                        " AZX_PIPELINE=" + (e->pipeline ? "1" : "0") +
                        " AZX_PIPELINE_STAGGER=" + (e->stagger ? "1" : "0") +
+                       " AZX_NEVAL_RESET=" + (e->neval_memset ? "memset" : "alternate") +
                        " reserved_cus=" + std::to_string(e->reserved_cus) +
+                       "; " + tree_fp +
                        "; src=" AZX_SRC_SHA;
     snprintf(buf, (size_t)cap, "%s", text.c_str());
     return (int)text.size();
@@ -755,24 +778,21 @@
     }
     if (d.evaluator == AZX_EVAL_RESNET) {
         if (!azx_net_ready(e->net)) return fail(AZX_ESTATE, "azx_set_weights has not been called");
-        HIPCHECK(hipMemsetAsync(d.n_eval, 0, sizeof(int32_t), e->stream));
-        if (timed) time_begin(e);
-        azx_launch_mcts(d, MODE_BEGIN, e->num_batches, e->stream, e->force_generic);
-        if (timed) time_end(e);
-        if (timed) time_begin(e, 1);
-        azx_net_eval(e->net, d, e->stream);
-        if (timed) time_end(e);
-        for (int b = 0; b < e->num_batches; ++b) {
-            HIPCHECK(hipMemsetAsync(d.n_eval, 0, sizeof(int32_t), e->stream));
+        DevEngine v[3];
+        neval_views(e, d, 0, v);
+        TRY(neval_begin(e));
+        for (int ph = 0; ph <= e->num_batches; ++ph) {
+            const DevEngine &dv = v[ph & 1];
+            if (e->neval_memset) HIPCHECK(hipMemsetAsync(dv.n_eval, 0, sizeof(int32_t), e->stream));
             if (timed) time_begin(e);
-            azx_launch_mcts(d, MODE_APPLY | MODE_SELECT, e->num_batches, e->stream, e->force_generic);
+            azx_launch_mcts(dv, ph ? MODE_APPLY | MODE_SELECT : MODE_BEGIN, e->num_batches, e->stream, e->force_generic);
             if (timed) time_end(e);
             if (timed) time_begin(e, 1);
-            azx_net_eval(e->net, d, e->stream);
+            azx_net_eval(e->net, dv, e->stream);
             if (timed) time_end(e);
         }
         if (timed) time_begin(e);
-        azx_launch_mcts(d, MODE_APPLY, e->num_batches, e->stream, e->force_generic);
+        azx_launch_mcts(v[2], MODE_APPLY, e->num_batches, e->stream, e->force_generic);
         if (timed) time_end(e);
         return AZX_OK;
     }
@@ -1216,19 +1236,23 @@
     if (!azx_net_ready(e->net)) return fail(AZX_ESTATE, "azx_set_weights has not been called");
     const DevEngine &d = e->d;
     const int half = d.G / 2, rows = half * d.bs;
-    const DevEngine hv[2] = {pool_view(d, 0, half, d.n_eval), pool_view(d, half, half, d.n_eval + 1)};
+    DevEngine hv[2][3];
+    for (int h = 0; h < 2; ++h) neval_views(e, pool_view(d, h * half, half, d.n_eval + h), h, hv[h]);
+    TRY(neval_begin(e));
+    int64_t phase = 0;
     const hipStream_t hs[2] = {e->stream, e->stream_b};
     const int nb = e->num_batches;
     const int split = rows / 2 / AZX_NET_ROW_ALIGN * AZX_NET_ROW_ALIGN;
     const bool stagger = e->stagger && split > 0;
     const int ref = time_mark(e, hs[0]);
     for (int64_t p = 0; p < plies; ++p) {
-        for (int ph = 0; ph <= nb; ++ph) {
+        for (int ph = 0; ph <= nb; ++ph, ++phase) {
             const int g_tree = ++e->ev_groups, g_net = ++e->ev_groups;
             for (int h = 0; h < 2; ++h) {
-                HIPCHECK(hipMemsetAsync(hv[h].n_eval, 0, sizeof(int32_t), hs[h]));
+                const DevEngine &v = hv[h][phase & 1];
+                if (e->neval_memset) HIPCHECK(hipMemsetAsync(v.n_eval, 0, sizeof(int32_t), hs[h]));
                 time_begin(e, 0, hs[h], g_tree, ref);
-                azx_launch_mcts(hv[h], ph ? MODE_APPLY | MODE_SELECT : MODE_BEGIN, nb, hs[h], e->force_generic);
+                azx_launch_mcts(v, ph ? MODE_APPLY | MODE_SELECT : MODE_BEGIN, nb, hs[h], e->force_generic);
                 time_end(e, 1, hs[h]);
                 if (p == 0 && ph == 0 && h == 0) {
                     HIPCHECK(hipEventRecord(e->ev_fork, hs[0]));
@@ -1237,12 +1261,12 @@
                 const bool cut = stagger && ph == 1;
                 if (cut && h == 1) HIPCHECK(hipStreamWaitEvent(hs[1], e->ev_stagger, 0));
                 time_begin(e, 1, hs[h], g_net, ref);
-                azx_net_eval_rows(e->net, hv[h], h * rows, cut && h == 0 ? split : rows, hs[h]);
+                azx_net_eval_rows(e->net, v, h * rows, cut && h == 0 ? split : rows, hs[h]);
                 time_end(e, 1, hs[h]);
                 if (cut && h == 0) {
                     HIPCHECK(hipEventRecord(e->ev_stagger, hs[0]));
                     time_begin(e, 1, hs[h], g_net, ref);
-                    azx_net_eval_rows_behind(e->net, hv[h], h * rows, split, rows, e->stagger_ctr, hs[h]);
+                    azx_net_eval_rows_behind(e->net, v, h * rows, split, rows, e->stagger_ctr, hs[h]);
                     time_end(e, 1, hs[h]);
                 }
             }
@@ -1250,10 +1274,10 @@
         const int g_tree = ++e->ev_groups;
         for (int h = 0; h < 2; ++h) {
             time_begin(e, 0, hs[h], g_tree, ref);
-            azx_launch_mcts(hv[h], MODE_APPLY, nb, hs[h], e->force_generic);
+            azx_launch_mcts(hv[h][2], MODE_APPLY, nb, hs[h], e->force_generic);
             time_end(e, 1, hs[h]);
-            azx_launch_choose(hv[h], hs[h]);
-            azx_launch_advance(hv[h], nullptr, 1, hs[h]);
+            azx_launch_choose(hv[h][2], hs[h]);
+            azx_launch_advance(hv[h][2], nullptr, 1, hs[h]);
         }
     }
     HIPCHECK(hipEventRecord(e->ev_join, hs[1]));
diff --git a/azalea_amd/csrc/azx_dev.h b/azalea_amd/csrc/azx_dev.h
--- a/azalea_amd/csrc/azx_dev.h
+++ b/azalea_amd/csrc/azx_dev.h
@@ -74,6 +74,7 @@
     float *ev_value;
     float *ev_prior;
     int32_t *n_eval;
+    int32_t *n_eval_clear;
     const double *noise;
     int32_t n_select, noise_stride;
     double noise_scale;
@@ -104,6 +105,27 @@
     double *stat_sums;
 };
 
+#include <cstdio>
+#include <string>
+static inline std::string azx_footprint_text(const char *name, const void *fn, int threads, size_t dyn_lds,
+                                             int hole_vgprs, size_t hole_lds) {
+    hipFuncAttributes fa = {};
+    int alone = -1;
+    if (hipFuncGetAttributes(&fa, fn) != hipSuccess) { (void)hipGetLastError(); return std::string(name) + ": no attributes"; }
+    if (hipOccupancyMaxActiveBlocksPerMultiprocessor(&alone, fn, threads, dyn_lds) != hipSuccess) { (void)hipGetLastError(); alone = -1; }
+    const int regs = (fa.numRegs + 7) / 8 * 8, waves = (threads + 63) / 64;
+    const size_t lds = fa.sharedSizeBytes + dyn_lds;
+    char b[256];
+    int n = snprintf(b, sizeof b, "%s: vgprs=%d lds=%zu scratch=%zu blocks_per_cu=%d", name, fa.numRegs, lds,
+                     (size_t)fa.localSizeBytes, alone);
+    if (hole_vgprs > 0 && regs > 0) {
+        const int by_regs = 4 * (hole_vgprs / regs) / waves;
+        const int by_lds = lds ? (int)(hole_lds / lds) : by_regs;
+        snprintf(b + n, sizeof b - (size_t)n, " blocks_per_hole=%d (vgprs %d, lds %d)", by_regs < by_lds ? by_regs : by_lds, by_regs, by_lds);
+    }
+    return b;
+}
+
 #define AZX_DPP(old, v, ctrl, rmask) \
     __builtin_amdgcn_update_dpp((old), (v), (ctrl), (rmask), 0xf, false)
 
diff --git a/azalea_amd/csrc/mcts_kernels.h b/azalea_amd/csrc/mcts_kernels.h
--- a/azalea_amd/csrc/mcts_kernels.h
+++ b/azalea_amd/csrc/mcts_kernels.h
@@ -12,6 +12,7 @@
 
 size_t azx_mcts_lds_bytes(int ncells, int bs);
 void azx_launch_mcts(const DevEngine &E, int mode, int num_batches, hipStream_t st, bool force_generic);
+std::string azx_mcts_footprint(const DevEngine &E, int hole_vgprs, size_t hole_lds);
 bool azx_mcts_fast_path(const DevEngine &E, int mode, bool force_generic);
 bool azx_launch_play(const DevEngine &E, int num_batches, int steps, hipStream_t st, bool allowed);
 void azx_launch_reset(const DevEngine &E, const int32_t *slots, int n_slots, const int32_t *moves,
diff --git a/azalea_amd/csrc/mcts_kernels.hip b/azalea_amd/csrc/mcts_kernels.hip
--- a/azalea_amd/csrc/mcts_kernels.hip
+++ b/azalea_amd/csrc/mcts_kernels.hip
@@ -1176,6 +1176,7 @@
 
 template <int SLOTS, bool FAST>
 __global__ __launch_bounds__(64) AZX_MCTS_ATTR void k_mcts(DevEngine E, int mode_arg, int num_batches) {
+    if (!FAST && E.n_eval_clear && blockIdx.x == 0 && threadIdx.x == 0) *E.n_eval_clear = 0;
     mcts_body<SLOTS, FAST>(E, mode_arg, num_batches);
 }
 
@@ -1762,6 +1763,12 @@
 #undef CALL
 }
 
+std::string azx_mcts_footprint(const DevEngine &E, int hole_vgprs, size_t hole_lds) {
+    const size_t lds = azx_mcts_lds_bytes(E.ncells, E.bs);
+    if (E.slots <= 2) return azx_footprint_text("k_mcts<2,false>", (const void *)k_mcts<2, false>, 64, lds, hole_vgprs, hole_lds);
+    return azx_footprint_text("k_mcts<3,false>", (const void *)k_mcts<3, false>, 64, lds, hole_vgprs, hole_lds);
+}
+
 bool azx_launch_play(const DevEngine &E, int num_batches, int steps, hipStream_t st, bool allowed) {
     if (!allowed) return false;
     if (!(E.evaluator == AZX_EVAL_UNIFORM && E.prior_default && (E.noise_scale == 0.0 || E.device_noise))) return false;
diff --git a/azalea_amd/csrc/net.h b/azalea_amd/csrc/net.h
--- a/azalea_amd/csrc/net.h
+++ b/azalea_amd/csrc/net.h
@@ -16,6 +16,7 @@
 int azx_net_check_range(AzxNet *net, hipStream_t st);
 int azx_net_debug_weights(AzxNet *net, int which, void *out, int64_t cap, int64_t *nbytes, char *name, int name_cap);
 const char *azx_net_kernel_info(const AzxNet *net);
+void azx_net_hole(const AzxNet *net, int *vgprs, size_t *lds);
 void azx_net_eval(AzxNet *net, const DevEngine &d, hipStream_t st);
 bool azx_net_rows_splittable(const AzxNet *net);
 void azx_net_eval_rows(AzxNet *net, const DevEngine &d, int row0, int max_n, hipStream_t st);
diff --git a/azalea_amd/csrc/net_kernels.hip b/azalea_amd/csrc/net_kernels.hip
--- a/azalea_amd/csrc/net_kernels.hip
+++ b/azalea_amd/csrc/net_kernels.hip
@@ -1092,7 +1092,7 @@
 }
 
 #define HM_MB 16
-__global__ __launch_bounds__(256, 3) void k_heads_mfma(NetDev P, const float *__restrict__ hfeat,
+__global__ __launch_bounds__(256, 3) void k_heads_mfma_r8(NetDev P, const float *__restrict__ hfeat,
                                                        const uint8_t *__restrict__ ev_board,
                                                        const int32_t *__restrict__ ev_flip,
                                                        const int32_t *__restrict__ n_eval_ptr, int n_eval_host,
@@ -1190,6 +1190,208 @@
         float4 bq[AH];
 #pragma unroll
         for (int u = 0; u < AH; ++u) bq[u] = wv[(size_t)min(u, QV - 1) * 64];
+        for (int qb = 0; qb < QV; qb += AH) {
+#pragma unroll
+            for (int u = 0; u < AH; ++u) {
+                const int q = qb + u;
+                const float4 b4 = bq[u];
+                bq[u] = wv[(size_t)min(q + AH, QV - 1) * 64];
+                if (q < QV) {
+                    const float4 a4 = *reinterpret_cast<const float4 *>(ap + 16 * q);
+                    accv = __builtin_amdgcn_mfma_f32_16x16x4f32(a4.x, b4.x, accv, 0, 0, 0);
+                    accv = __builtin_amdgcn_mfma_f32_16x16x4f32(a4.y, b4.y, accv, 0, 0, 0);
+                    accv = __builtin_amdgcn_mfma_f32_16x16x4f32(a4.z, b4.z, accv, 0, 0, 0);
+                    accv = __builtin_amdgcn_mfma_f32_16x16x4f32(a4.w, b4.w, accv, 0, 0, 0);
+                }
+            }
+        }
+    }
+    __syncthreads();
+    float (*lg)[AZX_CELL_STRIDE] = reinterpret_cast<float (*)[AZX_CELL_STRIDE]>(hsm);
+    float (*h2)[64] = reinterpret_cast<float (*)[64]>(hsm + HM_MB * AZX_CELL_STRIDE);
+#pragma unroll
+    for (int tt = 0; tt < 2; ++tt) {
+        const int j = 16 * (2 * wave + tt) + li;
+        if (2 * wave + tt < NTP && j < ncells) {
+            const float bias = P.mfcb[j];
+#pragma unroll
+            for (int r = 0; r < 4; ++r) {
+                const int b = 4 * lk + r;
+                const float logit = accp[tt][r] + bias;
+                lg[b][j] = logit;
+                if (b < nb) logit_out[(size_t)(e0 + b) * AZX_CELL_STRIDE + j] = logit;
+            }
+        }
+    }
+#pragma unroll
+    for (int r = 0; r < 4; ++r) h2[4 * lk + r][16 * wave + li] = accv[r];
+    __syncthreads();
+    if (tid < nb) {
+        float acc = 0.f;
+        for (int i = 0; i < 64; ++i) acc += fmaxf(h2[tid][i] + P.fc2b[i], 0.f) * P.fc3w[i];
+        value_out[e0 + tid] = tanhf(acc + P.fc3b[0]);
+    }
+    if (!prior_out) return;
+#pragma unroll
+    for (int bi = 0; bi < HM_MB / 4; ++bi) {
+        const int b = wave + 4 * bi;
+        if (b >= nb) break;
+        const int e = e0 + b;
+        float x[2];
+        bool legal[2];
+        float mx = -INFINITY;
+#pragma unroll
+        for (int s2 = 0; s2 < 2; ++s2) {
+            const int cell = s2 * 64 + lane;
+            legal[s2] = cell < ncells && cellv[bi][s2] == 0;
+            x[s2] = legal[s2] ? lg[b][cell] : -INFINITY;
+            mx = fmaxf(mx, x[s2]);
+        }
+        mx = wave_max(mx);
+        float sum = 0.f;
+#pragma unroll
+        for (int s2 = 0; s2 < 2; ++s2) sum += legal[s2] ? expf(x[s2] - mx) : 0.f;
+        const float lse = mx + logf(wave_sum(sum));
+        const int flip = flipv[bi];
+#pragma unroll
+        for (int s2 = 0; s2 < 2; ++s2) {
+            const int cell = s2 * 64 + lane;
+            if (cell < ncells) {
+                int oc = cell;
+                if (flip) {
+                    const int i = cell / N, j = cell - i * N;
+                    oc = (N - 1 - j) * N + (N - 1 - i);
+                }
+                prior_out[(size_t)e * AZX_CELL_STRIDE + oc] = legal[s2] ? expf(x[s2] - lse) : 0.f;
+            }
+        }
+    }
+}
+
+
+#define HM_CQ 18
+#define HM_CK (16 * HM_CQ)
+#define HM_LDC 324
+#define HM_LDS_BYTES (2 * HM_MB * HM_LDC * sizeof(float))
+static_assert(HM_LDC >= HM_CK && HM_LDC % 64 == 4, "chunk stride");
+static_assert(HM_MB * HM_LDC >= HM_MB * AZX_CELL_STRIDE + HM_MB * 64, "the logits and fc2 sums reuse the first chunk buffer");
+static_assert(HM_MB * HM_CK / 2 % 256 == 0, "a chunk is a whole number of float2 per thread");
+__global__ __launch_bounds__(256, 4) void k_heads_mfma(NetDev P, const float *__restrict__ hfeat,
+                                                       const uint8_t *__restrict__ ev_board,
+                                                       const int32_t *__restrict__ ev_flip,
+                                                       const int32_t *__restrict__ n_eval_ptr, int n_eval_host,
+                                                       float *__restrict__ logit_out, float *__restrict__ value_out,
+                                                       float *__restrict__ prior_out) {
+    extern __shared__ __align__(16) float hsm[];
+    const int n_eval = n_eval_ptr ? *n_eval_ptr : n_eval_host;
+    const int e0 = blockIdx.x * HM_MB;
+    if (e0 >= n_eval) return;
+    const int nb = min(HM_MB, n_eval - e0);
+    const int tid = threadIdx.x, lane = tid & 63, wave = tid >> 6;
+    const int li = lane & 15, lk = lane >> 4;
+    const int N = P.N, ncells = P.ncells;
+    const int KV = 2 * ncells, KP = 4 * ncells, KVp = (KV + 15) & ~15, KPp = (KP + 15) & ~15;
+    const int QV = KVp / 16, QP = KPp / 16, nf = 6 * ncells;
+    const int NCP = (QP + HM_CQ - 1) / HM_CQ;
+    constexpr int SF = HM_MB * HM_CK / 2 / 256;
+    float2 sv[SF];
+    const float *src0 = hfeat + (size_t)e0 * nf;
+    auto chunk_cols = [&](int c, int &col0, int &cw) {
+        col0 = c < NCP ? KV + c * HM_CK : 0;
+        cw = c < NCP ? min(HM_CK, KP - c * HM_CK) : KV;
+    };
+    auto chunk_load = [&](int c) {
+        int col0, cw;
+        chunk_cols(c, col0, cw);
+        const int hw = cw >> 1, total = nb * hw;
+#pragma unroll
+        for (int j = 0; j < SF; ++j) {
+            const int f = min(tid + 256 * j, total - 1), b = f / hw, i = f - b * hw;
+            sv[j] = *reinterpret_cast<const float2 *>(src0 + (size_t)b * nf + col0 + 2 * i);
+        }
+    };
+    auto chunk_store = [&](int c) {
+        int col0, cw;
+        chunk_cols(c, col0, cw);
+        const int hw = cw >> 1, total = nb * hw, cwp = (cw + 15) & ~15;
+        float *T = hsm + (size_t)(c & 1) * HM_MB * HM_LDC;
+#pragma unroll
+        for (int j = 0; j < SF; ++j) {
+            const int f = tid + 256 * j;
+            if (f < total) {
+                const int b = f / hw, i = f - b * hw;
+                *reinterpret_cast<float2 *>(T + (size_t)b * HM_LDC + 2 * i) = sv[j];
+            }
+        }
+        for (int b = wave; b < HM_MB; b += 4) {
+            float *row = T + (size_t)b * HM_LDC;
+            if (b < nb) {
+                if (lane < cwp - cw) row[cw + lane] = 0.0f;
+            } else {
+                for (int i = lane; i < cwp; i += 64) row[i] = 0.0f;
+            }
+        }
+    };
+    chunk_load(0);
+    const int NTP = (ncells + 15) / 16;
+    typedef float f32x4_ __attribute__((ext_vector_type(4)));
+    f32x4_ accp[2] = {f32x4_{0.f, 0.f, 0.f, 0.f}, f32x4_{0.f, 0.f, 0.f, 0.f}};
+    constexpr int AH = 6;
+    static_assert(HM_CQ % AH == 0, "a chunk is a whole number of pipeline rounds");
+    {
+        const int t0 = min(2 * wave, NTP - 1), t1 = min(2 * wave + 1, NTP - 1);
+        const float4 *w0 = reinterpret_cast<const float4 *>(P.hmP) + (size_t)t0 * QP * 64 + lane;
+        const float4 *w1 = reinterpret_cast<const float4 *>(P.hmP) + (size_t)t1 * QP * 64 + lane;
+        float4 bq0[AH], bq1[AH];
+#pragma unroll
+        for (int u = 0; u < AH; ++u) { bq0[u] = w0[(size_t)min(u, QP - 1) * 64]; bq1[u] = w1[(size_t)min(u, QP - 1) * 64]; }
+        for (int c = 0; c < NCP; ++c) {
+            chunk_store(c);
+            __syncthreads();
+            chunk_load(c + 1);
+            const float *ap = hsm + (size_t)(c & 1) * HM_MB * HM_LDC + (size_t)li * HM_LDC + 4 * lk;
+            const int qe = min(QP, (c + 1) * HM_CQ);
+            if (2 * wave < NTP)
+            for (int q0 = c * HM_CQ; q0 < qe; q0 += AH) {
+#pragma unroll
+                for (int u = 0; u < AH; ++u) {
+                    const int q = q0 + u;
+                    const float4 b0 = bq0[u], b1 = bq1[u];
+                    bq0[u] = w0[(size_t)min(q + AH, QP - 1) * 64];
+                    bq1[u] = w1[(size_t)min(q + AH, QP - 1) * 64];
+                    if (q < QP) {
+                        const float4 a4 = *reinterpret_cast<const float4 *>(ap + 16 * (q - c * HM_CQ));
+                        accp[0] = __builtin_amdgcn_mfma_f32_16x16x4f32(a4.x, b0.x, accp[0], 0, 0, 0);
+                        accp[1] = __builtin_amdgcn_mfma_f32_16x16x4f32(a4.x, b1.x, accp[1], 0, 0, 0);
+                        accp[0] = __builtin_amdgcn_mfma_f32_16x16x4f32(a4.y, b0.y, accp[0], 0, 0, 0);
+                        accp[1] = __builtin_amdgcn_mfma_f32_16x16x4f32(a4.y, b1.y, accp[1], 0, 0, 0);
+                        accp[0] = __builtin_amdgcn_mfma_f32_16x16x4f32(a4.z, b0.z, accp[0], 0, 0, 0);
+                        accp[1] = __builtin_amdgcn_mfma_f32_16x16x4f32(a4.z, b1.z, accp[1], 0, 0, 0);
+                        accp[0] = __builtin_amdgcn_mfma_f32_16x16x4f32(a4.w, b0.w, accp[0], 0, 0, 0);
+                        accp[1] = __builtin_amdgcn_mfma_f32_16x16x4f32(a4.w, b1.w, accp[1], 0, 0, 0);
+                    }
+                }
+            }
+        }
+    }
+    uint8_t cellv[HM_MB / 4][2];
+    int flipv[HM_MB / 4];
+#pragma unroll
+    for (int bi = 0; bi < HM_MB / 4; ++bi) {
+        const int b = wave + 4 * bi, e = e0 + (b < nb ? b : 0);
+        cellv[bi][0] = ev_board[(size_t)e * AZX_CELL_STRIDE + lane];
+        cellv[bi][1] = ev_board[(size_t)e * AZX_CELL_STRIDE + 64 + lane];
+        flipv[bi] = ev_flip[e];
+    }
+    f32x4_ accv = f32x4_{0.f, 0.f, 0.f, 0.f};
+    {
+        const float4 *wv = reinterpret_cast<const float4 *>(P.hmV) + (size_t)wave * QV * 64 + lane;
+        float4 bq[AH];
+#pragma unroll
+        for (int u = 0; u < AH; ++u) bq[u] = wv[(size_t)min(u, QV - 1) * 64];
+        chunk_store(NCP);
+        __syncthreads();
+        const float *ap = hsm + (size_t)(NCP & 1) * HM_MB * HM_LDC + (size_t)li * HM_LDC + 4 * lk;
         for (int qb = 0; qb < QV; qb += AH) {
 #pragma unroll
             for (int u = 0; u < AH; ++u) {
@@ -1461,7 +1663,8 @@
     const int cap = 160 * 1024;
     const void *fns[] = {(const void *)k_tower_f16x3_s16, (const void *)k_conv_wide_f16x3_s16,
                          (const void *)k_tower_mfma<64, 4, 2, 1, 2>, (const void *)k_tower_mfma<64, 6, 1, 2, 2>,
-                         (const void *)k_tower_mfma<32, 6, 2, 2, 1>, (const void *)k_heads_mfma, (const void *)k_heads};
+                         (const void *)k_tower_mfma<32, 6, 2, 2, 1>, (const void *)k_heads_mfma, (const void *)k_heads_mfma_r8,
+                         (const void *)k_heads};
     for (const void *f : fns)
         if (hipFuncSetAttribute(f, hipFuncAttributeMaxDynamicSharedMemorySize, cap) != hipSuccess)
             return nfail(AZX_EHIP, "net: raising a tower kernel's dynamic LDS limit failed");
@@ -1492,9 +1695,10 @@
     net->use_mfma = net->tower_variant != 0;
     { const char *v = getenv("AZX_WIDE_STREAMS"); net->opt_wsplit = std::min(4, std::max(1, v ? atoi(v) : 2)); }
     { const char *v = getenv("AZX_HEADS"); net->opt_heads_mfma = !(v && !strcmp(v, "valu")); }
+    { const char *v = getenv("AZX_HEADS_LAYOUT"); net->opt_heads_r8 = v && !strcmp(v, "r8"); }
     { const char *v = getenv("AZX_PACK"); net->pack_on_host = v && !strcmp(v, "host"); }
     {
-        char b[260];
+        char b[320];
         const char *tower = "k_stem_generic + k_conv_generic (VALU)";
         if (net->tower_variant == 4) tower = "k_tower_f16x3_s16";
         else if (net->tower_variant == 5) tower = "k_stem_wide_f16x3 + k_conv_wide_f16x3_s16 per layer";
@@ -1502,9 +1706,10 @@
         else if (net->tower_variant == 2) tower = "k_tower_mfma<64,6,1,2,2> (fp32 MFMA)";
         else if (net->tower_variant == 3) tower = "k_tower_mfma<32,6,2,2,1> (fp32 MFMA)";
         const bool hm = net->tower_variant == 4 && net->opt_heads_mfma && ncells <= 128;
-        snprintf(b, sizeof b, "%s + %s (%dx%d on %dx%d; AZX_TOWER=%s AZX_WIDE_STREAMS=%d AZX_HEADS=%s AZX_PACK=%s)",
-                 tower, hm ? "k_heads_mfma" : "k_heads", blocks, chans, N, N, want_fp32 ? "fp32" : "default",
-                 net->opt_wsplit, net->opt_heads_mfma ? "mfma" : "valu", net->pack_on_host ? "host" : "device");
+        snprintf(b, sizeof b, "%s + %s (%dx%d on %dx%d; AZX_TOWER=%s AZX_WIDE_STREAMS=%d AZX_HEADS=%s AZX_HEADS_LAYOUT=%s AZX_PACK=%s)",
+                 tower, hm ? (net->opt_heads_r8 ? "k_heads_mfma_r8" : "k_heads_mfma") : "k_heads", blocks, chans, N, N,
+                 want_fp32 ? "fp32" : "default", net->opt_wsplit, net->opt_heads_mfma ? "mfma" : "valu",
+                 net->opt_heads_r8 ? "r8" : "chunked", net->pack_on_host ? "host" : "device");
         net->info = b;
     }
     const size_t E = max_evals;
@@ -1531,6 +1736,21 @@
     net->lds_bytes = (size_t)bpb * 2 * (ncells + 1) * (chans + 4) * sizeof(float);
     if (net->tower_variant == 4) net->lds_bytes = (size_t)F16X3_BPB * 128 * 272 + 2 * 272;
     if (net->tower_variant == 5) net->lds_bytes = (size_t)(ncells + 2) * WIDE_ROWB;
+    if (net->tower_variant == 4) {
+        hipFuncAttributes fa = {};
+        if (hipFuncGetAttributes(&fa, (const void *)k_tower_f16x3_s16) != hipSuccess) (void)hipGetLastError();
+        const int hole_v = 512 - (fa.numRegs + 7) / 8 * 8;
+        const size_t hole_l = (size_t)160 * 1024 - net->lds_bytes - fa.sharedSizeBytes;
+        net->info += "; footprint: " + azx_footprint_text("k_tower_f16x3_s16", (const void *)k_tower_f16x3_s16, F16X3_BPB * 128, net->lds_bytes, 0, 0);
+        net->info += " hole_vgprs=" + std::to_string(hole_v) + " hole_lds=" + std::to_string(hole_l);
+        if (net->opt_heads_mfma && ncells <= 128) {
+            const size_t hl = std::max((size_t)HM_MB * azx_hm_lda(ncells), (size_t)HM_MB * AZX_CELL_STRIDE + (size_t)HM_MB * 64) * sizeof(float);
+            net->info += "; " + (net->opt_heads_r8 ? azx_footprint_text("k_heads_mfma_r8", (const void *)k_heads_mfma_r8, 256, hl, hole_v, hole_l)
+                                                   : azx_footprint_text("k_heads_mfma", (const void *)k_heads_mfma, 256, HM_LDS_BYTES, hole_v, hole_l));
+        }
+        net->hole_vgprs = hole_v;
+        net->hole_lds = hole_l;
+    }
     net->d.sat_flag = nalloc<uint32_t>(net, 4);
     if (!net->d.sat_flag || hipDeviceSynchronize() != hipSuccess) {
         azx_net_destroy(net);
@@ -1716,7 +1936,10 @@
     }
     if (hfeat != nullptr && net->opt_heads_mfma && d.ncells <= 128) {
         const size_t hl = std::max((size_t)HM_MB * d.hm_lda, (size_t)HM_MB * AZX_CELL_STRIDE + (size_t)HM_MB * 64) * sizeof(float);
-        hipLaunchKernelGGL(k_heads_mfma, dim3((max_n + HM_MB - 1) / HM_MB), dim3(256), hl, st, d, hfeat, boards, flip, n_eval_ptr, n_host, logit, value, prior);
+        if (net->opt_heads_r8)
+            hipLaunchKernelGGL(k_heads_mfma_r8, dim3((max_n + HM_MB - 1) / HM_MB), dim3(256), hl, st, d, hfeat, boards, flip, n_eval_ptr, n_host, logit, value, prior);
+        else
+            hipLaunchKernelGGL(k_heads_mfma, dim3((max_n + HM_MB - 1) / HM_MB), dim3(256), HM_LDS_BYTES, st, d, hfeat, boards, flip, n_eval_ptr, n_host, logit, value, prior);
     } else {
         const size_t hl = ((size_t)(6 * d.ncells + 64) * HEADS_BPB + (size_t)HEADS_BPB * AZX_CELL_STRIDE +
                            (size_t)(HEADS_KSPLIT - 1) * (64 + 192) * HEADS_BPB) * sizeof(float);
@@ -1725,6 +1948,7 @@
 }
 
 const char *azx_net_kernel_info(const AzxNet *net) { return net->info.c_str(); }
+void azx_net_hole(const AzxNet *net, int *vgprs, size_t *lds) { *vgprs = net ? net->hole_vgprs : 0; *lds = net ? net->hole_lds : 0; }
 
 int azx_net_check_range(AzxNet *net, hipStream_t st) {
     if (!net || !net->d.sat_flag) return AZX_OK;
diff --git a/azalea_amd/csrc/net_priv.h b/azalea_amd/csrc/net_priv.h
--- a/azalea_amd/csrc/net_priv.h
+++ b/azalea_amd/csrc/net_priv.h
@@ -38,6 +38,11 @@
     return (unsigned short)((bits + LO_RND) & LO_MASK);
 }
 
+static inline int azx_hm_lda(int ncells) {
+    const int KVp = (2 * ncells + 15) & ~15, KPp = (4 * ncells + 15) & ~15;
+    return ((KVp + KPp - 4 + 63) / 64) * 64 + 4;
+}
+
 struct AzxNet {
     NetDev d;
     int max_evals = 0;
@@ -54,12 +59,15 @@
     float *hb_value = nullptr;
     size_t lds_bytes = 0;
     int tower_variant = 0;
+    int hole_vgprs = 0;
+    size_t hole_lds = 0;
     hipStream_t stream2[3] = {nullptr, nullptr, nullptr};
     std::vector<uint32_t> cu_mask;
     hipEvent_t ev_fork = nullptr, ev_join[3] = {nullptr, nullptr, nullptr};
     bool streams_ok = false;
     int opt_wsplit = 2;
     bool opt_heads_mfma = true;
+    bool opt_heads_r8 = false;
     std::string info;
     bool pack_on_host = false;
     bool packed_once = false;
diff --git a/azalea_amd/engine.py b/azalea_amd/engine.py
--- a/azalea_amd/engine.py
+++ b/azalea_amd/engine.py
@@ -347,7 +347,7 @@
         return m[:n.value]
 
     def kernel_info(self):
-        buf = C.create_string_buffer(1024)
+        buf = C.create_string_buffer(4096)
         n = self.L.azx_kernel_info(self.h, buf, len(buf))
         if n < 0:
             check(n)
```

Measured after the change: 5.313 million, median of 2. Within noise of the previous version (+0.8%).
